# elun15/Graph-Convolutional-Network-for-Multi-Camera-Vehicle-Tracking

Measured on AMD Instinct MI355X. Metric: MPN forward edges/sec (+ achieved roofline fraction of the dominant kernel), higher is better.
Workload: dtype f32; 1 GPU; s02: AIC19-S02 ground-truth topology, cams 124/90/99/137: N=450 E=150454, L=3, Cs=1, eval forward; N=450, E=150454, parallelism=1 GPU

## Files before the change

### graph-convolutional-network-for-multi-camera-vehicle-tracking_amd/_lib.py

```python
from __future__ import annotations

import ctypes as C
import os

MAX_ENC_LAYERS = 8
NODE_DIM, EDGE_DIM, MAX_CLASSES = 32, 4, 4
AGG = {"sum": 0, "mean": 1, "max": 2}

(PH_BEGIN, PH_EDGE_ENC, PH_NODE_ENC, PH_NODE_H0, PH_ROUND_PROJ, PH_ROUND_A, PH_ROUND_B, PH_ROUND_STAT,
 PH_ROUND_C, PH_END, PH_NODE_COMBINE) = range(11)

E_ARG, E_WORKSPACE, E_HIP, E_ROWS = -1, -2, -3, -4

_f32p = C.c_void_p


class Layer(C.Structure):
    _fields_ = [("weight", _f32p), ("bias", _f32p), ("gamma", _f32p), ("beta", _f32p),
                ("in_dim", C.c_int32), ("out_dim", C.c_int32)]


class Model(C.Structure):
    _fields_ = [("struct_bytes", C.c_uint32), ("n_enc_layers", C.c_int32), ("enc_node", Layer * MAX_ENC_LAYERS), ("enc_edge", Layer * 2),
                ("upd_edge", Layer), ("upd_node", Layer), ("cls", Layer),
                ("agg", C.c_int32), ("num_enc_steps", C.c_int32), ("num_class_steps", C.c_int32),
                ("reattach_nodes", C.c_int32), ("reattach_edges", C.c_int32),
                ("dropout_enc", C.c_float), ("dropout_upd_edge", C.c_float), ("dropout_upd_node", C.c_float)]

    def __init__(self, *args, **kw):
        super().__init__(*args, **kw)
        self.struct_bytes = C.sizeof(type(self))


class Call(C.Structure):
    _fields_ = [("struct_bytes", C.c_uint32), ("x", C.c_void_p), ("x_row_stride", C.c_int64), ("row", C.c_void_p), ("col", C.c_void_p),
                ("idx_stride", C.c_int64), ("edge_attr", C.c_void_p), ("n_nodes", C.c_int64), ("n_edges", C.c_int64),
                ("n_edges_total", C.c_int64), ("node_lo", C.c_int64), ("node_hi", C.c_int64),
                ("logits", C.c_void_p), ("h_out", C.c_void_p), ("workspace", C.c_void_p),
                ("workspace_bytes", C.c_size_t), ("training", C.c_int32), ("flags", C.c_int32),
                ("seed", C.c_uint64), ("stream", C.c_void_p), ("row_lo", C.c_int64), ("row_hi", C.c_int64),
                ("weight_cache", C.c_void_p), ("weight_cache_bytes", C.c_size_t)]

    def __init__(self, *args, **kw):
        super().__init__(*args, **kw)
        self.struct_bytes = C.sizeof(type(self))


class WsLayout(C.Structure):
    _fields_ = [("total_bytes", C.c_size_t), ("zero_bytes", C.c_size_t), ("flags_off", C.c_size_t),
                ("stat_attr_off", C.c_size_t), ("stat_enc2_off", C.c_size_t), ("stat_enc_layer_off", C.c_size_t * MAX_ENC_LAYERS),
                ("stat_round_off", C.c_size_t), ("deg_off", C.c_size_t), ("seg_off", C.c_size_t),
                ("h0_off", C.c_size_t), ("h_acc_off", C.c_size_t * 2), ("deg_global_off", C.c_size_t),
                ("P_off", C.c_size_t)]


class Plan(C.Structure):
    _fields_ = [("enc_kernel", C.c_int32 * MAX_ENC_LAYERS), ("enc_split_k", C.c_int32 * MAX_ENC_LAYERS),
                ("edges_per_thread", C.c_int32), ("lazy_edges", C.c_int32), ("pass_c", C.c_int32),
                ("avg_degree", C.c_double), ("pass_a_col_blocks", C.c_int32), ("layer0_panels", C.c_int32),
                ("enc2_passenger", C.c_int32), ("node_stat_folded", C.c_int32)]


(GEMM_GENERIC, GEMM_INLOOP_64, GEMM_INLOOP_128, GEMM_PRESPLIT_256, GEMM_STAGED_128, GEMM_ROWS_16, GEMM_FEW_L0,
 GEMM_FEW_WAVE) = range(8)
PASS_C_WALK, PASS_C_MFMA_SORTED, PASS_C_MFMA_ANY = range(3)

STAT_REPLICAS, ATTR_STRIDE, ENC2_STRIDE, Z1_STRIDE, M_STRIDE, Z2_STRIDE = 16, 16, 16, 16, 16, 64
ROUND_BLOCK = STAT_REPLICAS * (Z1_STRIDE + M_STRIDE + Z2_STRIDE)
F_DETERMINISTIC, F_GLOBAL_DEG, F_FORK, F_SEED_ON_DEVICE = 1, 4, 2, 16
EDGE_W_ONE, EDGE_W_GIVEN, EDGE_W_BALANCED = range(3)
EDGE_LOSS_RECORD = 4
CLUSTER_SCORES, CLUSTER_COUNTS, EDGE_PRF = 9, 7, 5
CLUSTER_SCORES_MAX_N = 1048576
POOL_INFO = 4

LIB_PATH = os.environ.get("MTMC_MPN_LIB") or os.path.join(os.path.dirname(os.path.abspath(__file__)), "csrc", "libmtmc_mpn.so")
EXPORTS = ["mtmc_mpn_abi_version", "mtmc_mpn_last_error", "mtmc_mpn_workspace_bytes", "mtmc_mpn_workspace_layout",
           "mtmc_mpn_forward", "mtmc_mpn_run_phase", "mtmc_mpn_run_phases", "mtmc_mpn_plan_call", "mtmc_scatter_add", "mtmc_scatter_add_i64", "mtmc_scatter_mean", "mtmc_scatter_max",
           "mtmc_mlp_layer_forward", "mtmc_mpn_train_workspace_bytes", "mtmc_mpn_backward", "mtmc_graph_workspace_bytes",
           "mtmc_build_graph", "mtmc_postprocess_workspace_bytes", "mtmc_postprocess",
           "mtmc_cross_entropy_forward", "mtmc_cross_entropy_backward",
           "mtmc_cross_entropy_steps_forward", "mtmc_cross_entropy_steps_backward", "mtmc_mpn_backward_steps", "mtmc_mpn_backward_flat", "mtmc_mpn_grad_layout", "mtmc_linear_raw", "mtmc_edge_confusion",
           "mtmc_linear_presplit_raw", "mtmc_linear_staged_raw", "mtmc_linear_few_raw", "mtmc_mpn_weight_cache_bytes",
           "mtmc_graph_backward_workspace_bytes", "mtmc_build_graph_backward",
           "mtmc_edge_loss_scratch_bytes", "mtmc_edge_loss_forward", "mtmc_edge_loss_backward",
           "mtmc_cluster_scores_workspace_bytes", "mtmc_cluster_scores", "mtmc_edge_prf",
           "mtmc_pool_chunk_rows", "mtmc_pool_tracklets_workspace_bytes", "mtmc_pool_tracklets", "mtmc_pool_tracklets_backward"]

_lib = None


def load() -> C.CDLL:
    global _lib
    if _lib is not None:
        return _lib
    if not os.path.exists(LIB_PATH):
        raise RuntimeError(f"mtmc_mpn: HIP extension not built ({LIB_PATH} missing); run `python -m mtmc_mpn.build` "
                           "-- there is no fallback implementation")
    import torch
    lib = C.CDLL(LIB_PATH, mode=C.RTLD_GLOBAL)
    lib.mtmc_mpn_abi_version.restype = C.c_int32
    lib.mtmc_mpn_last_error.restype = C.c_char_p
    lib.mtmc_mpn_workspace_bytes.restype = C.c_size_t
    lib.mtmc_mpn_workspace_bytes.argtypes = [C.POINTER(Model), C.c_int64, C.c_int64]
    lib.mtmc_mpn_weight_cache_bytes.restype = C.c_size_t
    lib.mtmc_mpn_weight_cache_bytes.argtypes = [C.POINTER(Model)]
    lib.mtmc_linear_few_raw.restype = C.c_int32
    lib.mtmc_linear_few_raw.argtypes = [C.c_void_p, C.c_int64, C.c_void_p, C.c_void_p, C.c_void_p, C.c_double, C.c_void_p,
                                        C.c_void_p, C.c_void_p, C.c_int64, C.c_int32, C.c_int32, C.c_void_p, C.c_uint64,
                                        C.c_void_p, C.c_void_p]
    lib.mtmc_mpn_workspace_layout.restype = C.c_int32
    lib.mtmc_mpn_workspace_layout.argtypes = [C.POINTER(Model), C.c_int64, C.c_int64, C.POINTER(WsLayout)]
    lib.mtmc_mpn_forward.restype = C.c_int32
    lib.mtmc_mpn_forward.argtypes = [C.POINTER(Model), C.POINTER(Call)]
    lib.mtmc_mpn_train_workspace_bytes.restype = C.c_size_t
    lib.mtmc_mpn_train_workspace_bytes.argtypes = [C.POINTER(Model), C.c_int64, C.c_int64]
    lib.mtmc_mpn_backward.restype = C.c_int32
    lib.mtmc_mpn_backward.argtypes = [C.POINTER(Model), C.POINTER(Call), C.c_void_p, C.c_void_p, C.POINTER(Model),
                                      C.c_void_p, C.c_void_p]
    lib.mtmc_graph_workspace_bytes.restype = C.c_size_t
    lib.mtmc_graph_workspace_bytes.argtypes = [C.c_int64, C.c_int32]
    lib.mtmc_build_graph.restype = C.c_int32
    lib.mtmc_build_graph.argtypes = [C.c_void_p, C.c_int64, C.c_int64, C.c_int32, C.c_int32] + [C.c_void_p] * 5 + \
        [C.c_int32, C.c_int64] + [C.c_void_p] * 6 + [C.c_size_t, C.c_void_p]
    lib.mtmc_graph_backward_workspace_bytes.restype = C.c_size_t
    lib.mtmc_graph_backward_workspace_bytes.argtypes = [C.c_int64, C.c_int32]
    lib.mtmc_build_graph_backward.restype = C.c_int32
    lib.mtmc_build_graph_backward.argtypes = [C.c_void_p, C.c_int64, C.c_int64, C.c_int32, C.c_int32] + [C.c_void_p] * 5 + \
        [C.c_int32, C.c_int64] + [C.c_void_p] * 6 + [C.c_size_t, C.c_void_p]
    lib.mtmc_mpn_backward_steps.restype = C.c_int32
    lib.mtmc_mpn_backward_steps.argtypes = [C.POINTER(Model), C.POINTER(Call), C.POINTER(C.c_void_p), C.c_void_p,
                                            C.POINTER(Model), C.c_void_p, C.c_size_t, C.c_void_p, C.c_void_p]
    lib.mtmc_mpn_backward_flat.restype = C.c_int32
    lib.mtmc_mpn_backward_flat.argtypes = [C.POINTER(Model), C.POINTER(Call), C.POINTER(C.c_void_p), C.c_void_p, C.c_void_p,
                                           C.c_int64, C.c_void_p, C.c_void_p]
    lib.mtmc_mpn_grad_layout.restype = C.c_int64
    lib.mtmc_mpn_grad_layout.argtypes = [C.POINTER(Model), C.POINTER(C.c_int64), C.c_int32]
    lib.mtmc_edge_confusion.restype = C.c_int32
    lib.mtmc_edge_confusion.argtypes = [C.c_void_p, C.c_void_p, C.c_int64, C.c_int32, C.c_void_p, C.c_void_p]
    lib.mtmc_linear_presplit_raw.restype = C.c_int32
    lib.mtmc_linear_presplit_raw.argtypes = [C.c_void_p, C.c_int64, C.c_void_p, C.c_void_p, C.c_void_p, C.c_int64, C.c_int32,
                                             C.c_int32, C.c_void_p, C.c_uint64, C.c_void_p, C.c_void_p, C.c_int32, C.c_void_p]
    lib.mtmc_linear_staged_raw.restype = C.c_int32
    lib.mtmc_linear_staged_raw.argtypes = [C.c_void_p, C.c_int64, C.c_void_p, C.c_void_p, C.c_void_p, C.c_double, C.c_void_p,
                                           C.c_void_p, C.c_void_p, C.c_int64, C.c_int32, C.c_int32, C.c_void_p, C.c_uint64,
                                           C.c_void_p, C.c_void_p, C.c_void_p]
    lib.mtmc_linear_raw.restype = C.c_int32
    lib.mtmc_linear_raw.argtypes = [C.c_void_p, C.c_int64, C.c_void_p, C.c_void_p, C.c_void_p, C.c_int64, C.c_int32,
                                    C.c_int32, C.c_void_p, C.c_void_p, C.c_void_p]
    lib.mtmc_cross_entropy_forward.restype = C.c_int32
    lib.mtmc_cross_entropy_forward.argtypes = [C.c_void_p, C.c_void_p, C.c_void_p, C.c_int64, C.c_int32, C.c_int64,
                                               C.c_int32, C.c_void_p, C.c_void_p, C.c_void_p, C.c_void_p]
    lib.mtmc_cross_entropy_backward.restype = C.c_int32
    lib.mtmc_cross_entropy_backward.argtypes = [C.c_void_p, C.c_void_p, C.c_void_p, C.c_int64, C.c_int32, C.c_int64,
                                                C.c_int32, C.c_void_p, C.c_void_p, C.c_void_p, C.c_void_p]
    lib.mtmc_cross_entropy_steps_forward.restype = C.c_int32
    lib.mtmc_cross_entropy_steps_forward.argtypes = [C.c_void_p, C.c_void_p, C.c_void_p, C.c_int64, C.c_int32, C.c_int32,
                                                     C.c_int64, C.c_int32, C.c_void_p, C.c_void_p, C.c_void_p]
    lib.mtmc_cross_entropy_steps_backward.restype = C.c_int32
    lib.mtmc_cross_entropy_steps_backward.argtypes = [C.c_void_p, C.c_void_p, C.c_void_p, C.c_int64, C.c_int32, C.c_int32,
                                                      C.c_int64, C.c_int32, C.c_void_p, C.c_void_p, C.c_void_p, C.c_void_p]
    lib.mtmc_edge_loss_scratch_bytes.restype = C.c_size_t
    lib.mtmc_edge_loss_scratch_bytes.argtypes = [C.c_int32]
    lib.mtmc_edge_loss_forward.restype = C.c_int32
    lib.mtmc_edge_loss_forward.argtypes = [C.c_void_p, C.c_void_p, C.c_int64, C.c_int32, C.c_int32, C.c_int32, C.c_void_p,
                                           C.c_float, C.c_void_p, C.c_size_t, C.c_void_p, C.c_void_p, C.c_void_p, C.c_void_p]
    lib.mtmc_edge_loss_backward.restype = C.c_int32
    lib.mtmc_edge_loss_backward.argtypes = [C.c_void_p, C.c_void_p, C.c_int64, C.c_int32, C.c_int32, C.c_void_p, C.c_void_p,
                                            C.c_void_p, C.c_void_p]
    lib.mtmc_cluster_scores_workspace_bytes.restype = C.c_size_t
    lib.mtmc_cluster_scores_workspace_bytes.argtypes = [C.c_int64]
    lib.mtmc_cluster_scores.restype = C.c_int32
    lib.mtmc_cluster_scores.argtypes = [C.c_void_p, C.c_int64, C.c_void_p, C.c_int64, C.c_int64, C.c_void_p, C.c_void_p,
                                        C.c_void_p, C.c_size_t, C.c_void_p]
    lib.mtmc_edge_prf.restype = C.c_int32
    lib.mtmc_edge_prf.argtypes = [C.c_void_p, C.c_int64, C.c_void_p, C.c_int64, C.c_int64, C.c_void_p, C.c_void_p, C.c_void_p]
    lib.mtmc_pool_chunk_rows.restype = C.c_int32
    lib.mtmc_pool_chunk_rows.argtypes = []
    lib.mtmc_pool_tracklets_workspace_bytes.restype = C.c_size_t
    lib.mtmc_pool_tracklets_workspace_bytes.argtypes = [C.c_int64, C.c_int32]
    lib.mtmc_pool_tracklets.restype = C.c_int32
    lib.mtmc_pool_tracklets.argtypes = [C.c_void_p, C.c_int64, C.c_int64, C.c_int32, C.c_void_p, C.c_int64, C.c_void_p,
                                        C.c_void_p, C.c_void_p, C.c_size_t, C.c_void_p]
    lib.mtmc_pool_tracklets_backward.restype = C.c_int32
    lib.mtmc_pool_tracklets_backward.argtypes = [C.c_void_p, C.c_int64, C.c_int32, C.c_void_p, C.c_int64, C.c_void_p,
                                                 C.c_int64, C.c_void_p]
    lib.mtmc_postprocess_workspace_bytes.restype = C.c_size_t
    lib.mtmc_postprocess_workspace_bytes.argtypes = [C.c_int64, C.c_int64, C.c_int64]
    lib.mtmc_postprocess.restype = C.c_int32
    lib.mtmc_postprocess.argtypes = [C.c_void_p, C.c_void_p, C.c_void_p, C.c_int64, C.c_int64, C.c_int64, C.c_int32,
                                     C.c_int32, C.c_int64, C.c_void_p, C.c_void_p, C.c_void_p, C.c_void_p, C.c_void_p,
                                     C.c_size_t, C.c_void_p]
    lib.mtmc_mpn_plan_call.restype = C.c_int32
    lib.mtmc_mpn_plan_call.argtypes = [C.POINTER(Model), C.POINTER(Call), C.POINTER(Plan)]
    lib.mtmc_mpn_run_phase.restype = C.c_int32
    lib.mtmc_mpn_run_phase.argtypes = [C.POINTER(Model), C.POINTER(Call), C.c_int32, C.c_int32]
    lib.mtmc_mpn_run_phases.restype = C.c_int32
    lib.mtmc_mpn_run_phases.argtypes = [C.POINTER(Model), C.POINTER(Call), C.POINTER(C.c_int32), C.c_int32]
    for name in ("mtmc_scatter_add", "mtmc_scatter_add_i64"):
        getattr(lib, name).restype = C.c_int32
        getattr(lib, name).argtypes = [C.c_void_p, C.c_void_p, C.c_int64, C.c_int64, C.c_int64, C.c_void_p, C.c_void_p]
    lib.mtmc_scatter_mean.restype = C.c_int32
    lib.mtmc_scatter_mean.argtypes = [C.c_void_p, C.c_void_p, C.c_int64, C.c_int64, C.c_int64, C.c_void_p, C.c_void_p,
                                      C.c_void_p]
    lib.mtmc_scatter_max.restype = C.c_int32
    lib.mtmc_scatter_max.argtypes = [C.c_void_p, C.c_void_p, C.c_int64, C.c_int64, C.c_int64, C.c_void_p, C.c_void_p,
                                     C.c_void_p]
    lib.mtmc_mlp_layer_forward.restype = C.c_int32
    lib.mtmc_mlp_layer_forward.argtypes = [C.POINTER(Layer), C.c_void_p, C.c_int64, C.c_int64, C.c_void_p, C.c_void_p,
                                           C.c_void_p]
    if lib.mtmc_mpn_abi_version() != 6:
        raise RuntimeError("mtmc_mpn: ABI version mismatch between _lib.py and libmtmc_mpn.so")
    _lib = lib
    return lib


def check(rc: int):
    if rc == 0:
        return
    msg = load().mtmc_mpn_last_error().decode()
    if rc == E_ROWS:
        raise ValueError(msg)
    raise RuntimeError(f"mtmc_mpn: {msg} (code {rc})")
```

### graph-convolutional-network-for-multi-camera-vehicle-tracking_amd/csrc/api.hip

```cpp
#include "api_internal.h"

using namespace mtmc_api;

namespace {

struct Side { hipStream_t stream = nullptr; hipEvent_t fork = nullptr, join = nullptr; bool ok = false; };
Side* side_for_current_device() {
  static Side sides[64];
  static std::mutex mu;
  int dev = 0;
  if (hipGetDevice(&dev) != hipSuccess || dev < 0 || dev >= 64) return nullptr;
  std::lock_guard<std::mutex> lock(mu);
  Side& sd = sides[dev];
  if (!sd.ok) {
    if (hipStreamCreateWithFlags(&sd.stream, hipStreamNonBlocking) != hipSuccess) return nullptr;
    if (hipEventCreateWithFlags(&sd.fork, hipEventDisableTiming) != hipSuccess) return nullptr;
    if (hipEventCreateWithFlags(&sd.join, hipEventDisableTiming) != hipSuccess) return nullptr;
    sd.ok = true;
  }
  return &sd;
}

constexpr int kMaxPipes = 64;
struct PipeSlot { int dev; hipStream_t caller; SidePipe pipe; };
// ... 41 lines not shown
  Layout lo;
  make_layout(model, n_nodes, n_edges, &lo);
  return lo.pub.total_bytes;
}

size_t mtmc_mpn_weight_cache_bytes(const mtmc_mpn_model* model) {
  if (check_model(model) != MTMC_OK) return 0;
  CacheLayout cl;
  make_cache_layout(model, &cl);
  return cl.total > 0 ? cl.total : 256;
}

int32_t mtmc_mpn_workspace_layout(const mtmc_mpn_model* model, int64_t n_nodes, int64_t n_edges, mtmc_ws_layout* out) {
  if (int rc = check_model(model)) return rc;
  if (!out || n_nodes < 0 || n_edges < 0) return fail(MTMC_E_ARG, "bad layout arguments");
  Layout lo;
  make_layout(model, n_nodes, n_edges, &lo);
  *out = lo.pub;
  return MTMC_OK;
}

int32_t mtmc_dbg_panel_timing(int32_t enable) {
  PanelTiming& pt = panel_timing();
  if (enable && !pt.created) {
    for (int i = 0; i < 2 * kMaxPanels; ++i)
      if (hipEventCreate(&pt.ev[i]) != hipSuccess) return fail(MTMC_E_HIP, "hipEventCreate failed");
    pt.created = true;
  }
  pt.on = enable != 0;
  pt.n = 0;
  return MTMC_OK;
}
int32_t mtmc_dbg_panel_times(float* ms, int32_t max) {
  PanelTiming& pt = panel_timing();
  if (!ms || !pt.created) return 0;
  int n = 0;
  for (; n < pt.n && n < max; ++n) {
    if (hipEventSynchronize(pt.ev[2 * n + 1]) != hipSuccess) break;
    if (hipEventElapsedTime(&ms[n], pt.ev[2 * n], pt.ev[2 * n + 1]) != hipSuccess) break;
  }
  return n;
}

int32_t mtmc_mpn_run_phase(const mtmc_mpn_model* model, const mtmc_mpn_call* call, int32_t phase, int32_t arg) {
  Ctx x;
  if (int rc = make_ctx(model, call, &x)) return rc;
  return run_phase(x, phase, arg);
}

int32_t mtmc_mpn_run_phases(const mtmc_mpn_model* model, const mtmc_mpn_call* call, const int32_t* phase_args, int32_t n) {
  Ctx x;
  if (int rc = make_ctx(model, call, &x)) return rc;
  if (n < 0 || (n > 0 && !phase_args)) return fail(MTMC_E_ARG, "mtmc_mpn_run_phases: bad phase list");
  for (int i = 0; i < n; ++i)
    if (int rc = run_phase(x, phase_args[2 * i], phase_args[2 * i + 1])) return rc;
  return MTMC_OK;
}

int32_t mtmc_mpn_plan_call(const mtmc_mpn_model* model, const mtmc_mpn_call* call, mtmc_mpn_plan* out) {
  if (int rc = check_model(model)) return rc;
  if (!out) return fail(MTMC_E_ARG, "mtmc_mpn_plan_call: NULL result");
  if (int rc = check_call_size(call)) return rc;
  const mtmc_mpn_call* c = call;
  if (c->n_nodes < 0 || c->n_edges < 0 || c->n_edges > c->n_edges_total || c->node_lo < 0 || c->node_hi < c->node_lo ||
      c->node_hi > c->n_nodes || c->row_lo < 0 || c->row_hi < c->row_lo || c->row_hi > c->n_nodes)
    return fail(MTMC_E_ARG, "mtmc_mpn_plan_call: sizes / ranges out of order");
  Layout lo;
  CacheLayout cl;
  CallPlan p;
  make_layout(model, c->n_nodes, c->n_edges, &lo, c->training != 0);
  make_cache_layout(model, &cl);
  make_plan(model, c, lo, cl, &p);
  *out = mtmc_mpn_plan();
  for (int l = 0; l < model->n_enc_layers; ++l) { out->enc_kernel[l] = p.enc_kernel[l]; out->enc_split_k[l] = p.enc_split_k[l]; }
  out->edges_per_thread = p.edges_per_thread;
  out->lazy_edges = p.lazy_edges ? 1 : 0;
  out->avg_degree = p.avg_degree;
  out->pass_a_col_blocks = p.col_blocks;
  out->pass_c = p.pass_c_pub();
  out->node_stat_folded = p.fold_node_stat ? 1 : 0;
  out->layer0_panels = p.l0_panels;
  out->enc2_passenger = (p.enc2_may_ride && !(c->flags & MTMC_F_FORK)) ? 1 : 0;
  return MTMC_OK;
}

int32_t mtmc_mpn_forward(const mtmc_mpn_model* model, const mtmc_mpn_call* call) {
  Ctx x;
  if (int rc = make_ctx(model, call, &x)) return rc;
  int rc;
  if (x.plan.l0_panels >= 2) x.pipe = pipe_for(x.stream);
  Side* sd = (call->flags & MTMC_F_FORK) ? side_for_current_device() : nullptr;
  if (sd) {
    if ((rc = run_phase(x, MTMC_PH_BEGIN, 0))) return rc;
    if (hipEventRecord(sd->fork, x.stream) != hipSuccess || hipStreamWaitEvent(sd->stream, sd->fork, 0) != hipSuccess)
      return fail(MTMC_E_HIP, "fork onto the side stream failed");
    Ctx xs = x;
    xs.stream = sd->stream;
    if ((rc = run_phase(xs, MTMC_PH_EDGE_ENC, 0))) return rc;
    if (hipEventRecord(sd->join, sd->stream) != hipSuccess) return fail(MTMC_E_HIP, "hipEventRecord failed");
  } else {
    if ((rc = run_phase(x, MTMC_PH_BEGIN, 0))) return rc;
    x.enc2_rides = x.plan.enc2_may_ride;
    if (!x.enc2_rides && (rc = run_phase(x, MTMC_PH_EDGE_ENC, 0))) return rc;
  }
  for (int l = 0; l < model->n_enc_layers; ++l) {
    if ((rc = run_phase(x, MTMC_PH_NODE_ENC, l))) return rc;
    if ((rc = run_phase(x, MTMC_PH_NODE_COMBINE, l))) return rc;
  }
  if (sd && hipStreamWaitEvent(x.stream, sd->join, 0) != hipSuccess) return fail(MTMC_E_HIP, "join failed");
  const bool fused_h0 = model->num_enc_steps > 0 && call->node_lo == 0 && call->node_hi == call->n_nodes;
  if (!fused_h0 && (rc = run_phase(x, MTMC_PH_NODE_H0, 0))) return rc;
  for (int r = 0; r < model->num_enc_steps; ++r) {
    if ((rc = run_phase(x, MTMC_PH_ROUND_PROJ, r, fused_h0))) return rc;
    if ((rc = run_phase(x, MTMC_PH_ROUND_A, r))) return rc;
    if ((rc = run_phase(x, MTMC_PH_ROUND_B, r))) return rc;
    if ((rc = run_phase(x, MTMC_PH_ROUND_STAT, r))) return rc;
    if ((rc = run_phase(x, MTMC_PH_ROUND_C, r))) return rc;
  }
  return run_phase(x, MTMC_PH_END, 0);
}

static int scatter_common(const float* src, const int64_t* index, int64_t n_src, int64_t n_cols, int64_t dim_size,
                          float* out, float* count, int64_t* arg_out, int mode, void* stream) {
  if (n_src < 0 || n_cols < 1 || dim_size < 0 || !out || (n_src > 0 && (!src || !index)))
    return fail(MTMC_E_ARG, "bad scatter arguments");
  if (mode == 1 && !count) return fail(MTMC_E_ARG, "scatter_mean needs count_scratch[dim_size]");
  if (dim_size == 0) return MTMC_OK;
  mtmc::launch_scatter(src, index, n_src, n_cols, dim_size, out, count, arg_out, mode, static_cast<hipStream_t>(stream));
  const hipError_t e = hipGetLastError();
  return e == hipSuccess ? MTMC_OK : fail(MTMC_E_HIP, "scatter launch failed: %s", hipGetErrorString(e));
}
int32_t mtmc_scatter_add(const float* src, const int64_t* index, int64_t n_src, int64_t n_cols, int64_t dim_size,
                         float* out, void* stream) {
  return scatter_common(src, index, n_src, n_cols, dim_size, out, nullptr, nullptr, 0, stream);
}
int32_t mtmc_scatter_add_i64(const int64_t* src, const int64_t* index, int64_t n_src, int64_t n_cols, int64_t dim_size,
                             int64_t* out, void* stream) {
  if (n_src < 0 || n_cols < 1 || dim_size < 0 || !out || (n_src > 0 && (!src || !index)))
    return fail(MTMC_E_ARG, "bad scatter arguments");
  if (dim_size == 0) return MTMC_OK;
  mtmc::launch_scatter_add_i64(src, index, n_src, n_cols, dim_size, out, static_cast<hipStream_t>(stream));
  const hipError_t e = hipGetLastError();
  return e == hipSuccess ? MTMC_OK : fail(MTMC_E_HIP, "scatter launch failed: %s", hipGetErrorString(e));
}
int32_t mtmc_scatter_mean(const float* src, const int64_t* index, int64_t n_src, int64_t n_cols, int64_t dim_size,
                          float* out, float* count_scratch, void* stream) {
  return scatter_common(src, index, n_src, n_cols, dim_size, out, count_scratch, nullptr, 1, stream);
}
int32_t mtmc_scatter_max(const float* src, const int64_t* index, int64_t n_src, int64_t n_cols, int64_t dim_size,
                         float* out, int64_t* arg_out, void* stream) {
  return scatter_common(src, index, n_src, n_cols, dim_size, out, nullptr, arg_out, 2, stream);
}

int32_t mtmc_mlp_layer_forward(const mtmc_layer* layer, const float* x, int64_t x_row_stride, int64_t rows, float* y,
                               double* stats_scratch, void* stream) {
  if (!layer || !layer->weight || !layer->bias || !x || !y || rows < 1) return fail(MTMC_E_ARG, "bad mlp layer arguments");
  const bool bn = layer->gamma != nullptr;
  if (bn && (!layer->beta || !stats_scratch)) return fail(MTMC_E_ARG, "BatchNorm layer needs beta and stats_scratch[2*out]");
  if (bn && rows < 2) return fail(MTMC_E_ROWS, "Expected more than 1 value per channel when training");
  hipStream_t s = static_cast<hipStream_t>(stream);
  if (bn && hipMemsetAsync(stats_scratch, 0, 2 * (size_t)layer->out_dim * sizeof(double), s) != hipSuccess)
    return fail(MTMC_E_HIP, "hipMemsetAsync failed");
  mtmc::GemmParams g =
      mtmc::plain_gemm(x, x_row_stride, layer->weight, layer->bias, y, layer->out_dim, rows, layer->in_dim, layer->out_dim);
  if (bn) g.stats_out = stats_scratch;
  if (mtmc::launch_gemm_bn(g, s) != MTMC_OK) return fail(MTMC_E_ARG, "unsupported layer shape");
  if (bn)
    mtmc::launch_bn_relu_rows({y, layer->out_dim, rows, layer->out_dim, stats_scratch, layer->gamma, layer->beta, (double)rows, y,
                               mtmc::kNoDrop, 0}, s);
  const hipError_t e = hipGetLastError();
  return e == hipSuccess ? MTMC_OK : fail(MTMC_E_HIP, "mlp layer launch failed: %s", hipGetErrorString(e));
}

static int raw_begin(uint32_t* scratch, double* stats, int N, hipStream_t s) {
  return mtmc::clear_raw(scratch, stats, N, s) ? MTMC_OK : fail(MTMC_E_HIP, "hipMemsetAsync failed");
}
static int raw_end(int rc) {
  if (rc != 0) return fail(rc == MTMC_E_HIP ? MTMC_E_HIP : MTMC_E_ARG, "unsupported shape or launch refused");
  const hipError_t e = hipGetLastError();
  return e == hipSuccess ? MTMC_OK : fail(MTMC_E_HIP, "launch failed: %s", hipGetErrorString(e));
}
static void raw_amax(const float* A, int64_t lda, int64_t M, const float* W, int K, int N, uint32_t* scratch, hipStream_t s) {
  mtmc::PrepParams p = {};
  p.jobs[p.n_jobs++] = {A, M, K, lda, scratch, 0, 0};
  if (W) p.jobs[p.n_jobs++] = {W, N, K, K, scratch + mtmc::kAmaxRep, 0, 0};
  mtmc::launch_prep(p, s);
}

int32_t mtmc_linear_raw(const float* A, int64_t lda, const float* W, const float* bias, float* Y, int64_t M, int32_t K,
                        int32_t N, uint32_t* scratch, double* stats, void* stream) {
  if (!A || !W || !bias || !Y || !scratch || M < 1 || K < 32 || K % 32 || N < 1) return fail(MTMC_E_ARG, "bad arguments");
  hipStream_t s = static_cast<hipStream_t>(stream);
  if (int rc = raw_begin(scratch, stats, N, s)) return rc;
  raw_amax(A, lda, M, W, K, N, scratch, s);
  mtmc::GemmParams g = mtmc::plain_gemm(A, lda, W, bias, Y, N, M, K, N, scratch, scratch + mtmc::kAmaxRep, scratch + 2 * mtmc::kAmaxRep);
  g.stats_out = stats;
// ... 77 lines not shown
```

### graph-convolutional-network-for-multi-camera-vehicle-tracking_amd/csrc/api_internal.h

```cpp
#pragma once
#include "kernels.h"
#include "train_kernels.h"

#include <mutex>
#include <stdarg.h>
#include <stdio.h>
#include <stdlib.h>
#include <string.h>
#include <algorithm>
#include <vector>

namespace mtmc_api {


inline thread_local char g_err[512] = "";

inline int fail(int code, const char* fmt, ...) __attribute__((format(printf, 2, 3)));
inline int fail(int code, const char* fmt, ...) {
  va_list ap;
  va_start(ap, fmt);
  vsnprintf(g_err, sizeof(g_err), fmt, ap);
  va_end(ap);
  return code;
}

inline size_t align_up(size_t v, size_t a = 256) { return (v + a - 1) / a * a; }

struct Layout {
  mtmc_ws_layout pub;
  size_t row32, col32, e_buf[2], P, Q, slab, enc_aff, row_start, carry;
  size_t col_sub; int col_blocks;
  size_t amax;
  size_t amax_w;
  size_t Y[MTMC_MAX_ENC_LAYERS];
  size_t stat_enc_layer[MTMC_MAX_ENC_LAYERS];
  bool training;
  std::vector<size_t> z_tr, e_tr, h_tr;
  std::vector<size_t> P_tr, Q_tr;
  size_t xh, inv_a;
  bool few;
  size_t wh[MTMC_MAX_ENC_LAYERS], inv_w[MTMC_MAX_ENC_LAYERS]; bool w_ws[MTMC_MAX_ENC_LAYERS];
  size_t g_e[2], g_e0, g_h[2], g_h0, g_P, g_Q, g_de2, g_arg;
  size_t bst;
  size_t bwd_zero, bwd_zero_end;
  size_t gacc;
  size_t amax_bwd;
  size_t seed_word = 0;
  size_t gA, gB, tA, tB, tW, tX, zeros, bst_n;
};

struct CacheLayout { size_t planes[MTMC_MAX_ENC_LAYERS], inv[MTMC_MAX_ENC_LAYERS], fp[MTMC_MAX_ENC_LAYERS]; bool has[MTMC_MAX_ENC_LAYERS]; size_t total; };
inline void make_cache_layout(const mtmc_mpn_model* m, CacheLayout* cl) {
  size_t off = 0;
  auto take = [&](size_t bytes) { size_t o = off; off = align_up(off + bytes); return o; };
  for (int l = 0; l < MTMC_MAX_ENC_LAYERS; ++l) {
    cl->has[l] = l < m->n_enc_layers && m->enc_node[l].in_dim % 8 == 0 && m->enc_node[l].in_dim <= 2048;
    cl->planes[l] = cl->inv[l] = cl->fp[l] = 0;
    if (!cl->has[l]) continue;
    const size_t K = m->enc_node[l].in_dim, O = m->enc_node[l].out_dim;
    cl->planes[l] = take(4 * O * K);
    cl->inv[l] = take(4 * O);
    cl->fp[l] = take(8 * ((O + 7) / 8));
  }
  cl->total = off;
}
inline bool few_shape(const mtmc_mpn_model* m, int64_t rows) {
  int in_dim[MTMC_MAX_ENC_LAYERS], out_dim[MTMC_MAX_ENC_LAYERS];
  for (int l = 0; l < m->n_enc_layers; ++l) { in_dim[l] = m->enc_node[l].in_dim; out_dim[l] = m->enc_node[l].out_dim; }
  return mtmc::few_rows_path(rows, m->n_enc_layers, in_dim, out_dim);
}

inline int node_in_width(const mtmc_mpn_model* m) { return (m->reattach_nodes ? 2 : 1) * MTMC_NODE_DIM; }
inline int first_cls_step(const mtmc_mpn_model* m) { return std::max(1, m->num_enc_steps - m->num_class_steps + 1); }

inline int check_model(const mtmc_mpn_model* m) {
  if (!m) return fail(MTMC_E_ARG, "model is NULL");
  if (m->struct_bytes != sizeof(mtmc_mpn_model))
    return fail(MTMC_E_ARG, "mtmc_mpn_model.struct_bytes is %u, this library's struct has %zu bytes (ABI v%d): rebuild the caller against include/mtmc_mpn.h",
                m->struct_bytes, sizeof(mtmc_mpn_model), MTMC_MPN_ABI_VERSION);
  if (m->n_enc_layers < 1 || m->n_enc_layers > MTMC_MAX_ENC_LAYERS) return fail(MTMC_E_ARG, "n_enc_layers out of range");
  for (int l = 0; l < m->n_enc_layers; ++l) {
    const mtmc_layer& L = m->enc_node[l];
    if (!L.weight || !L.bias || !L.gamma || !L.beta) return fail(MTMC_E_ARG, "node encoder layer %d: NULL parameter", l);
    if (L.in_dim % 32 || L.in_dim < 32 || L.out_dim < 1) return fail(MTMC_E_ARG, "node encoder layer %d: in_dim must be a positive multiple of 32", l);
    if (l && L.in_dim != m->enc_node[l - 1].out_dim) return fail(MTMC_E_ARG, "node encoder layer %d: in_dim != previous out_dim", l);
  }
  if (m->enc_node[m->n_enc_layers - 1].out_dim != MTMC_NODE_DIM) return fail(MTMC_E_ARG, "node encoder must end at width %d", MTMC_NODE_DIM);
  if ((m->enc_edge[0].in_dim != 1 && m->enc_edge[0].in_dim != 2) || m->enc_edge[0].out_dim != 4 ||
      m->enc_edge[1].in_dim != 4 || m->enc_edge[1].out_dim != 4)
    return fail(MTMC_E_ARG, "edge encoder must be in(1|2)->4->4");
  const int hn = node_in_width(m), he = (m->reattach_edges ? 2 : 1) * MTMC_EDGE_DIM;
  if (m->upd_edge.in_dim != 2 * hn + he || m->upd_edge.out_dim != 4) return fail(MTMC_E_ARG, "edge update layer must be [4, %d]", 2 * hn + he);
  if (m->upd_node.in_dim != hn + 4 || m->upd_node.out_dim != MTMC_NODE_DIM) return fail(MTMC_E_ARG, "node update layer must be [32, %d]", hn + 4);
  if (m->cls.in_dim != 4 || m->cls.out_dim < 1 || m->cls.out_dim > MTMC_MAX_CLASSES) return fail(MTMC_E_ARG, "classifier must be [C<=4, 4]");
  const mtmc_layer* small[] = {&m->enc_edge[0], &m->enc_edge[1], &m->upd_edge, &m->upd_node};
  for (const mtmc_layer* L : small)
    if (!L->weight || !L->bias || !L->gamma || !L->beta) return fail(MTMC_E_ARG, "NULL parameter in an edge/update layer");
  if (!m->cls.weight || !m->cls.bias) return fail(MTMC_E_ARG, "NULL classifier parameter");
  if (m->agg < 0 || m->agg > 2) return fail(MTMC_E_ARG, "agg must be MTMC_AGG_SUM/MEAN/MAX");
  if (m->num_enc_steps < 0 || m->num_class_steps < 0) return fail(MTMC_E_ARG, "negative step count");
  return MTMC_OK;
}

inline void make_layout(const mtmc_mpn_model* m, int64_t N, int64_t E, Layout* lo, bool training = false) {
  *lo = Layout();
  lo->training = training;
  size_t off = 0;
  auto take = [&](size_t bytes) { size_t o = off; off = align_up(off + bytes); return o; };
  const int L = m->num_enc_steps;
  lo->pub.flags_off = take(8 * sizeof(int32_t));
  lo->pub.stat_attr_off = take((size_t)mtmc::kStatRep * mtmc::kAttrStride * sizeof(double));
  lo->stat_enc_layer[0] = take(2 * (size_t)m->enc_node[0].out_dim * sizeof(double));
  lo->pub.stat_enc2_off = take((size_t)mtmc::kStatRep * mtmc::kEnc2Stride * sizeof(double));
  for (int l = 1; l < m->n_enc_layers; ++l) lo->stat_enc_layer[l] = take(2 * (size_t)m->enc_node[l].out_dim * sizeof(double));
  for (int l = 0; l < m->n_enc_layers; ++l) lo->pub.stat_enc_layer_off[l] = lo->stat_enc_layer[l];
  lo->pub.stat_round_off = take((size_t)(L > 0 ? L : 1) * mtmc::kRoundBlock * sizeof(double));
  lo->pub.deg_off = take((size_t)N * sizeof(int32_t));
  lo->pub.seg_off = take(mtmc::fold_node_stat(E) ? 0 : (size_t)N * 4 * sizeof(double));
  lo->amax = take((size_t)(1 + 2 * MTMC_MAX_ENC_LAYERS) * mtmc::kAmaxRep * sizeof(uint32_t));
  lo->amax_w = take((size_t)MTMC_MAX_ENC_LAYERS * mtmc::kAmaxRep * sizeof(uint32_t));
  lo->pub.zero_bytes = off;
  lo->pub.deg_global_off = take((size_t)N * sizeof(int32_t));
  lo->pub.h0_off = take((size_t)N * 32 * sizeof(float));
  lo->pub.h_acc_off[0] = take((size_t)N * 32 * sizeof(float));
  lo->pub.h_acc_off[1] = take((size_t)N * 32 * sizeof(float));
  lo->enc_aff = take(16 * sizeof(float));
  lo->seed_word = take(sizeof(unsigned long long));
  lo->row_start = take((size_t)N * sizeof(int32_t));
  lo->carry = take((size_t)((E + 31) / 32) * 2 * 32 * sizeof(float));
  lo->col_blocks = mtmc::plan_col_blocks(N, E, 1e30, training);
  lo->col_sub = take(lo->col_blocks > 0 ? (size_t)N * (lo->col_blocks + 1) * sizeof(int32_t) : 0);
  lo->P = take((size_t)N * 8 * sizeof(float));
  lo->pub.P_off = lo->P;
  lo->Q = take((size_t)N * 32 * sizeof(float));
  lo->row32 = take((size_t)E * sizeof(int32_t));
  lo->col32 = take((size_t)E * sizeof(int32_t));
  lo->e_buf[0] = take((size_t)E * 4 * sizeof(float));
  lo->e_buf[1] = take((size_t)E * 4 * sizeof(float));
  for (int l = 0; l < m->n_enc_layers; ++l) lo->Y[l] = take((size_t)N * m->enc_node[l].out_dim * sizeof(float));
  size_t slab = 0;
  for (int l = 0; l < m->n_enc_layers; ++l) {
    int sk;
    mtmc::gemm_plan(N, m->enc_node[l].in_dim, m->enc_node[l].out_dim, &sk);
    const size_t need = sk > 1 ? (size_t)sk * N * m->enc_node[l].out_dim * sizeof(float) : 0;
    if (need > slab) slab = need;
  }
  lo->slab = take(slab);
  lo->few = few_shape(m, N);
  for (int l = 0; l < m->n_enc_layers; ++l) {
    const int K = m->enc_node[l].in_dim, O = m->enc_node[l].out_dim;
    lo->w_ws[l] = !training && (l == 0 ? mtmc::presplit_layer0(N, K, O) : mtmc::staged_layer(N, K, O));
  }
  if (lo->w_ws[0] || lo->few) {
    lo->xh = take((size_t)2 * N * m->enc_node[0].in_dim * sizeof(uint16_t));
    lo->inv_a = take((size_t)N * sizeof(float));
  }
  for (int l = 0; l < m->n_enc_layers; ++l)
    if (lo->w_ws[l]) {
      lo->wh[l] = take((size_t)2 * m->enc_node[l].out_dim * m->enc_node[l].in_dim * sizeof(uint16_t));
      lo->inv_w[l] = take((size_t)m->enc_node[l].out_dim * sizeof(float));
    }
  if (training) {
    for (int r = 0; r < L; ++r) {
      lo->z_tr.push_back(take((size_t)E * 4 * sizeof(float)));
      lo->e_tr.push_back(take((size_t)E * 4 * sizeof(float)));
      lo->h_tr.push_back(take((size_t)N * 32 * sizeof(float)));
      lo->P_tr.push_back(r == 0 ? lo->P : take((size_t)N * 8 * sizeof(float)));
      lo->Q_tr.push_back(r == 0 ? lo->Q : take((size_t)N * 32 * sizeof(float)));
    }
    size_t maxd = 0, bn_stats = 0;
    for (int l = 0; l < m->n_enc_layers; ++l) {
      maxd = std::max(maxd, (size_t)m->enc_node[l].in_dim);
      maxd = std::max(maxd, (size_t)m->enc_node[l].out_dim);
      bn_stats += 2 * (size_t)m->enc_node[l].out_dim;
    }
    lo->bwd_zero = off;
    lo->bst = take((size_t)(2 * L + 1) * mtmc::kStatRep * mtmc::kBwdStride * sizeof(double));
    lo->bst_n = take(bn_stats * sizeof(double));
    lo->gacc = take((size_t)mtmc::kGradRep * mtmc::kGaccN * sizeof(float));
    lo->amax_bwd = take((size_t)2 * MTMC_MAX_ENC_LAYERS * mtmc::kAmaxRep * sizeof(uint32_t));
    lo->g_P = take((size_t)(L > 0 ? L : 1) * mtmc::kGradRep * N * 8 * sizeof(float));
    lo->g_Q = take((size_t)(L > 0 ? L : 1) * N * 32 * sizeof(float));
    lo->zeros = take(maxd * sizeof(float));
    lo->g_h0 = take((size_t)N * 32 * sizeof(float));
    lo->g_e0 = take((size_t)E * 4 * sizeof(float));
    lo->g_e[0] = take((size_t)E * 4 * sizeof(float));
    lo->g_h[0] = take((size_t)N * 32 * sizeof(float));
    lo->bwd_zero_end = off;
    lo->g_e[1] = take((size_t)E * 4 * sizeof(float));
    lo->g_h[1] = take((size_t)N * 32 * sizeof(float));
    lo->g_de2 = take((size_t)E * 4 * sizeof(float));
    lo->g_arg = take((size_t)N * 32 * sizeof(int32_t));
    const size_t npad = (size_t)((N + 31) / 32 * 32);
    lo->gA = take((size_t)N * maxd * sizeof(float));
    lo->gB = take((size_t)N * maxd * sizeof(float));
    lo->tA = take(npad * maxd * sizeof(float));
    lo->tB = take(npad * maxd * sizeof(float));
    size_t wsum = 0;
    for (int l = 0; l < m->n_enc_layers; ++l) wsum += (size_t)m->enc_node[l].in_dim * m->enc_node[l].out_dim;
    lo->tW = take(wsum * sizeof(float));
    lo->tX = take(npad * (size_t)m->enc_node[0].in_dim * sizeof(float));
  }
  lo->pub.total_bytes = off;
}

constexpr int kMaxPanels = 16;
struct SidePipe { hipStream_t stream = nullptr; hipEvent_t fork = nullptr; hipEvent_t ready[kMaxPanels] = {}; };

struct PanelTiming { bool on = false, created = false; hipEvent_t ev[2 * kMaxPanels]; int n = 0; };
inline PanelTiming& panel_timing() { static PanelTiming t; return t; }

inline int l0_panels(int64_t rows, int Nout, int64_t* cuts, int* bm) {
  const int tiles_n = (Nout + 255) / 256;
  *bm = mtmc::presplit_tile_rows(rows, tiles_n);
  const int64_t per_round = (int64_t)(256 / tiles_n > 0 ? 256 / tiles_n : 1) * *bm;
  const int mode = mtmc::knobs().l0_pipeline;
  int np = 0;
  int64_t at = 0, k = 1;
  cuts[0] = 0;
  while (at < rows) {
    int64_t take = per_round * (mode == 3 ? 2 : mode == 2 ? 1 : k);
    if (np == kMaxPanels - 1 || at + take > rows) take = rows - at;
    at += take;
    cuts[++np] = at;
    if (k < 8) k *= 2;
  }
  return np;
}

struct CallPlan {
  int64_t rows;
  int enc_kernel[MTMC_MAX_ENC_LAYERS];
  int enc_split_k[MTMC_MAX_ENC_LAYERS];
  bool w_cached[MTMC_MAX_ENC_LAYERS];
  int l0_panels, l0_bm;
  int64_t l0_cuts[kMaxPanels + 1];
  bool enc2_may_ride;
  int edges_per_thread;
  bool lazy_edges;
  bool fold_node_stat;
  double avg_degree;
  int col_blocks;
  mtmc::PassC pass_c;
  int pass_c_pub() const {
    switch (pass_c) {
      case mtmc::kPassCSortedWalk: case mtmc::kPassCSortedDet: return MTMC_PASS_C_MFMA_SORTED;
      case mtmc::kPassCAnyWalk: case mtmc::kPassCAny: return MTMC_PASS_C_MFMA_ANY;
      default: return MTMC_PASS_C_WALK;
    }
  }
};

inline bool in_loop_kernel(int k) { return k == MTMC_GEMM_GENERIC || k == MTMC_GEMM_INLOOP_64 || k == MTMC_GEMM_INLOOP_128; }

inline void make_plan(const mtmc_mpn_model* m, const mtmc_mpn_call* c, const Layout& lo, const CacheLayout& cl, CallPlan* p) {
  *p = CallPlan();
  const int64_t N = c->n_nodes, E = c->n_edges, rows = c->node_hi - c->node_lo;
  const mtmc_layer& L0 = m->enc_node[0];
  p->rows = rows;
  const bool pre0 = lo.w_ws[0] && mtmc::presplit_layer0(rows, L0.in_dim, L0.out_dim);
  bool few = lo.few && c->weight_cache != nullptr && few_shape(m, rows);
  for (int l = 0; l < m->n_enc_layers; ++l) few = few && cl.has[l];
  for (int l = 0; l < m->n_enc_layers; ++l) {
    const mtmc_layer& Ll = m->enc_node[l];
    int k, sk = 1;
    if (few) k = l == 0 ? MTMC_GEMM_FEW_L0 : MTMC_GEMM_FEW_WAVE;
    else if (l == 0 && pre0) k = MTMC_GEMM_PRESPLIT_256;
    else if (l >= 1 && lo.w_ws[l] && mtmc::staged_layer(rows, Ll.in_dim, Ll.out_dim)) k = MTMC_GEMM_STAGED_128;
    else if (l >= 1 && !lo.training && mtmc::rows_layer(N, Ll.in_dim, Ll.out_dim) && mtmc::rows_layer(rows, Ll.in_dim, Ll.out_dim))
      k = MTMC_GEMM_ROWS_16;
    else {
      int sk_full = 1, sk_here = 1;
      mtmc::gemm_plan(N, Ll.in_dim, Ll.out_dim, &sk_full);
      const int cfg = rows > 0 ? mtmc::gemm_plan(rows, Ll.in_dim, Ll.out_dim, &sk_here) : 0;
      k = cfg == 2 ? MTMC_GEMM_INLOOP_128 : cfg == 1 ? MTMC_GEMM_INLOOP_64 : MTMC_GEMM_GENERIC;
      if (sk_here > 1 && (size_t)sk_here * rows <= (size_t)(sk_full > 1 ? sk_full : 0) * N) sk = sk_here;
    }
    p->enc_kernel[l] = k;
    p->enc_split_k[l] = sk;
    p->w_cached[l] = c->weight_cache != nullptr && cl.has[l] && !in_loop_kernel(k) && k != MTMC_GEMM_ROWS_16;
  }
  p->l0_panels = 1;
  if (p->enc_kernel[0] == MTMC_GEMM_PRESPLIT_256 && mtmc::knobs().l0_pipeline > 0)
    p->l0_panels = l0_panels(rows, L0.out_dim, p->l0_cuts, &p->l0_bm);
  const int last = m->n_enc_layers - 1, kl = p->enc_kernel[last];
  p->enc2_may_ride = E > 0 && E <= mtmc::kSmallEdges &&
                     (kl == MTMC_GEMM_INLOOP_64 || (kl == MTMC_GEMM_FEW_WAVE && mtmc::few_wave_threads(m->enc_node[last].in_dim) == 256));
  p->edges_per_thread = mtmc::plan_edges_per_thread(E);
  p->lazy_edges = !lo.training && E > mtmc::kSmallEdges;
  p->fold_node_stat = mtmc::fold_node_stat(E);
  if (c->row_hi > 0) p->avg_degree = c->row_hi > c->row_lo ? (double)E / (double)(c->row_hi - c->row_lo) : 0.0;
  else p->avg_degree = N > 0 ? (double)c->n_edges_total / (double)N : 0.0;
  p->col_blocks = (m->num_enc_steps > 0 && lo.col_blocks > 0 &&
                   mtmc::plan_col_blocks(N, E, p->avg_degree, lo.training) == lo.col_blocks) ? lo.col_blocks : 0;
  const bool drop_n = lo.training && m->dropout_upd_node > 0.f;
  p->pass_c = mtmc::plan_pass_c(m->agg, (c->flags & MTMC_F_DETERMINISTIC) != 0, drop_n, E, N, p->avg_degree);
}

struct Ctx {
  const mtmc_mpn_model* m;
  const mtmc_mpn_call* c;
  Layout lo;
  char* ws;
  hipStream_t stream;
  char* wc = nullptr;
  CacheLayout cl;
  CallPlan plan;
  template <typename T> T* wc_at(size_t off) const { return reinterpret_cast<T*>(wc + off); }
  const SidePipe* pipe = nullptr;
  bool enc2_rides = false;
  template <typename T> T* at(size_t off) const { return reinterpret_cast<T*>(ws + off); }
};

inline int check_call_size(const mtmc_mpn_call* c) {
  if (!c) return fail(MTMC_E_ARG, "call is NULL");
  if (c->struct_bytes != sizeof(mtmc_mpn_call))
    return fail(MTMC_E_ARG, "mtmc_mpn_call.struct_bytes is %u, this library's struct has %zu bytes (ABI v%d): rebuild the caller against include/mtmc_mpn.h",
                c->struct_bytes, sizeof(mtmc_mpn_call), MTMC_MPN_ABI_VERSION);
  return MTMC_OK;
}

inline int make_ctx(const mtmc_mpn_model* m, const mtmc_mpn_call* c, Ctx* ctx) {
  if (int rc = check_model(m)) return rc;
  if (int rc = check_call_size(c)) return rc;
  if (c->training && (c->node_lo != 0 || c->node_hi != c->n_nodes || c->n_edges_total != c->n_edges))
    return fail(MTMC_E_ARG, "training mode is single-shard only");
  if (c->training && (c->flags & MTMC_F_SEED_ON_DEVICE) && (c->seed == 0 || (c->seed & 7)))
    return fail(MTMC_E_ARG, "MTMC_F_SEED_ON_DEVICE: seed must hold the 8-byte aligned device address of a uint64 counter");
  if (c->n_nodes < 2) return fail(MTMC_E_ROWS, "BatchNorm over %lld node rows: Expected more than 1 value per channel", (long long)c->n_nodes);
  if (c->n_edges_total < 2) return fail(MTMC_E_ROWS, "BatchNorm over %lld edge rows: Expected more than 1 value per channel", (long long)c->n_edges_total);
  if (c->n_edges < 0 || c->n_edges > c->n_edges_total || c->n_edges >= (1ll << 31) || c->n_nodes >= (1ll << 31))
    return fail(MTMC_E_ARG, "edge/node counts out of range");
  if (c->node_lo < 0 || c->node_hi < c->node_lo || c->node_hi > c->n_nodes) return fail(MTMC_E_ARG, "bad node range");
  if (c->row_lo < 0 || c->row_hi < c->row_lo || c->row_hi > c->n_nodes) return fail(MTMC_E_ARG, "bad row range");
  if (c->training && (c->row_lo != 0 || (c->row_hi != 0 && c->row_hi != c->n_nodes)))
    return fail(MTMC_E_ARG, "training calls project every node row (row_lo = row_hi = 0)");
  if (!c->x || !c->edge_attr || !c->logits || !c->h_out || !c->workspace) return fail(MTMC_E_ARG, "NULL tensor pointer");
  if (c->n_edges > 0 && (!c->row || !c->col)) return fail(MTMC_E_ARG, "NULL edge_index pointer");
  if (c->idx_stride < 1) return fail(MTMC_E_ARG, "idx_stride must be >= 1");
  if (((uintptr_t)c->x & 15) || (c->x_row_stride & 3) || c->x_row_stride < m->enc_node[0].in_dim)
    return fail(MTMC_E_ARG, "x must be 16-byte aligned with a row stride that is a multiple of 4 and >= in_dim");
  if (((uintptr_t)c->edge_attr & 7) || ((uintptr_t)c->logits & 7) || ((uintptr_t)c->h_out & 15))
    return fail(MTMC_E_ARG, "edge_attr/logits must be 8-byte and h_out 16-byte aligned");
  if ((uintptr_t)c->workspace & 255) return fail(MTMC_E_WORKSPACE, "workspace must be 256-byte aligned");
  ctx->m = m; ctx->c = c;
  make_layout(m, c->n_nodes, c->n_edges, &ctx->lo, c->training != 0);
  if (c->workspace_bytes < ctx->lo.pub.total_bytes)
    return fail(MTMC_E_WORKSPACE, "workspace has %zu bytes, %zu needed", c->workspace_bytes, ctx->lo.pub.total_bytes);
  ctx->ws = static_cast<char*>(c->workspace);
  ctx->stream = static_cast<hipStream_t>(c->stream);
  make_cache_layout(m, &ctx->cl);
  if (c->weight_cache) {
    if ((uintptr_t)c->weight_cache & 255) return fail(MTMC_E_WORKSPACE, "weight_cache must be 256-byte aligned");
    if (c->weight_cache_bytes < ctx->cl.total)
      return fail(MTMC_E_WORKSPACE, "weight_cache has %zu bytes, %zu needed (mtmc_mpn_weight_cache_bytes)", c->weight_cache_bytes, ctx->cl.total);
    ctx->wc = static_cast<char*>(c->weight_cache);
  }
  make_plan(m, c, ctx->lo, ctx->cl, &ctx->plan);
  return MTMC_OK;
}

inline mtmc::Drop make_drop(const Ctx& x, float p) {
  mtmc::Drop d;
  d.on = (x.c->training && p > 0.f) ? 1 : 0;
  d.seed = x.c->seed;
  if (d.on && (x.c->flags & MTMC_F_SEED_ON_DEVICE)) {
    d.on = 2;
    d.seed = (unsigned long long)(uintptr_t)(x.ws + x.lo.seed_word);
  }
  const double t = (double)p * 65536.0;
  d.thresh = t >= 65535.0 ? 65535u : (unsigned)t;
  d.inv_keep = p < 1.f ? 1.f / (1.f - p) : 0.f;
  return d;
}

inline mtmc::EdgeEncParams enc_params(const Ctx& x) {
  mtmc::EdgeEncParams e;
  const mtmc_layer& a = x.m->enc_edge[0];
  const mtmc_layer& b = x.m->enc_edge[1];
  e.w1 = a.weight; e.b1 = a.bias; e.g1 = a.gamma; e.bt1 = a.beta;
  e.w2 = b.weight; e.b2 = b.bias; e.g2 = b.gamma; e.bt2 = b.beta;
  e.stat_attr = x.at<double>(x.lo.pub.stat_attr_off);
  e.stat_enc2 = x.at<double>(x.lo.pub.stat_enc2_off);
  e.aff = x.at<float>(x.lo.enc_aff);
  e.fe = a.in_dim;
  e.drop = make_drop(x, x.m->dropout_enc);
  return e;
}

inline float* agg_target(const Ctx& x, int r) {
  if (x.lo.training) return x.at<float>(x.lo.h_tr[r]);
  if (r == x.m->num_enc_steps - 1 && x.m->agg != MTMC_AGG_MEAN) return x.c->h_out;
  return x.at<float>(x.lo.pub.h_acc_off[r & 1]);
}
inline int64_t proj_lo(const mtmc_mpn_call* c) { return c->row_hi > 0 ? c->row_lo : 0; }
inline int64_t proj_hi(const mtmc_mpn_call* c) { return c->row_hi > 0 ? c->row_hi : c->n_nodes; }
inline float* round_h_src(const Ctx& x, int r) {
  if (r == 0) return x.at<float>(x.lo.pub.h0_off);
  return x.lo.training ? x.at<float>(x.lo.h_tr[r - 1]) : x.at<float>(x.lo.pub.h_acc_off[(r - 1) & 1]);
}
inline float* round_P(const Ctx& x, int r) { return x.at<float>(x.lo.training ? x.lo.P_tr[r] : x.lo.P); }
inline float* round_Q(const Ctx& x, int r) { return x.at<float>(x.lo.training ? x.lo.Q_tr[r] : x.lo.Q); }
inline float* round_z(const Ctx& x, int r) { return x.at<float>(x.lo.training ? x.lo.z_tr[r] : x.lo.e_buf[r & 1]); }
inline float* round_e(const Ctx& x, int r) { return x.at<float>(x.lo.training ? x.lo.e_tr[r] : x.lo.e_buf[r & 1]); }

inline mtmc::RoundParams round_params(const Ctx& x, int r) {
  const mtmc_mpn_model* m = x.m;
  const int hn = node_in_width(m);
  mtmc::RoundParams p;
  p.row32 = x.at<int>(x.lo.row32); p.col32 = x.at<int>(x.lo.col32);
  p.attr = x.c->edge_attr;
  p.e_buf = round_z(x, r); p.e_out = round_e(x, r); p.e_prev = r > 0 ? round_e(x, r - 1) : nullptr;
  p.drop_e = make_drop(x, m->dropout_upd_edge); p.drop_n = make_drop(x, m->dropout_upd_node);
  p.drop_stream = mtmc::kDropRound + 2 * r;
  p.P = round_P(x, r); p.Q = round_Q(x, r);
  p.seg = x.at<double>(x.lo.pub.seg_off); p.fold_z2 = x.plan.fold_node_stat ? 1 : 0;
  p.ue_w = m->upd_edge.weight; p.ue_b = m->upd_edge.bias; p.ue_g = m->upd_edge.gamma; p.ue_bt = m->upd_edge.beta;
  p.ue_ld = m->upd_edge.in_dim; p.ue_eoff = 2 * hn;
  p.un_w = m->upd_node.weight; p.un_b = m->upd_node.bias; p.un_g = m->upd_node.gamma; p.un_bt = m->upd_node.beta;
  p.un_ld = m->upd_node.in_dim; p.un_eoff = hn;
  p.cls_w = m->cls.weight; p.cls_b = m->cls.bias; p.n_classes = m->cls.out_dim;
  p.stats = x.at<double>(x.lo.pub.stat_round_off) + (size_t)r * mtmc::kRoundBlock;
  p.lazy_e = x.plan.lazy_edges ? 1 : 0;
  p.prev_stats = r > 0 ? p.stats - mtmc::kRoundBlock : nullptr;
  p.h_acc = agg_target(x, r);
  const int step = r + 1, first_cls = first_cls_step(m);
  p.logits = step >= first_cls ? x.c->logits + (size_t)(step - first_cls) * x.c->n_edges * m->cls.out_dim : nullptr;
  p.n_edges = x.c->n_edges; p.e_total = (double)x.c->n_edges_total;
  p.first_round = r == 0; p.reattach_edges = m->reattach_edges; p.agg = m->agg;
  p.det = (x.c->flags & MTMC_F_DETERMINISTIC) ? 1 : 0; p.flags = x.at<int>(x.lo.pub.flags_off);
  p.deg = x.at<int>(x.lo.pub.deg_off); p.row_start = x.at<int>(x.lo.row_start); p.carry = x.at<float>(x.lo.carry);
  p.n_nodes = x.c->n_nodes;
  p.avg_degree = x.plan.avg_degree;
  p.pass_c = x.plan.pass_c;
  p.col_blocks = x.plan.col_blocks;
  p.col_sub = x.at<int>(x.lo.col_sub); p.cb_row_lo = proj_lo(x.c); p.cb_row_hi = proj_hi(x.c);
  p.enc = enc_params(x);
  return p;
}

inline _Float16* w_planes(const Ctx& x, int l) {
  if (x.plan.w_cached[l]) return x.wc_at<_Float16>(x.cl.planes[l]);
  return x.at<_Float16>(x.lo.wh[l]);
}
inline float* w_inv(const Ctx& x, int l) {
  if (x.plan.w_cached[l]) return x.wc_at<float>(x.cl.inv[l]);
  return x.at<float>(x.lo.inv_w[l]);
}

enum { kPhMemset = -1, kPhPrep = -2 };

inline void fill_prep_edge(const Ctx& x, mtmc::PrepEdge* p) {
  const mtmc_mpn_call* c = x.c;
  p->row = c->row; p->col = c->col; p->idx_stride = c->idx_stride; p->attr = c->edge_attr; p->fe = x.m->enc_edge[0].in_dim;
  p->n_edges = c->n_edges; p->n_nodes = c->n_nodes;
  p->row32 = x.at<int>(x.lo.row32); p->col32 = x.at<int>(x.lo.col32); p->deg = x.at<int>(x.lo.pub.deg_off);
  p->flags = x.at<int>(x.lo.pub.flags_off); p->stat_attr = x.at<double>(x.lo.pub.stat_attr_off);
  p->row_start = x.at<int>(x.lo.row_start);
}

inline const int* scale_deg(const Ctx& x) {
  return x.at<int>((x.c->flags & MTMC_F_GLOBAL_DEG) ? x.lo.pub.deg_global_off : x.lo.pub.deg_off);
}

inline unsigned* amax_x(const Ctx& x) { return x.at<unsigned>(x.lo.amax); }
inline unsigned* amax_y(const Ctx& x, int l) { return amax_x(x) + (1 + MTMC_MAX_ENC_LAYERS + l) * mtmc::kAmaxRep; }
inline unsigned* amax_w(const Ctx& x, int l) { return x.at<unsigned>(x.lo.amax_w) + l * mtmc::kAmaxRep; }
inline unsigned* amax_in(const Ctx& x, int l) { return l == 0 ? amax_x(x) : amax_y(x, l - 1); }

inline void fill_in(const Ctx& x, int l, mtmc::ActIn* q) {
  if (l == 0) {
    q->A = x.c->x; q->lda = x.c->x_row_stride;
  } else {
    const mtmc_layer& Pv = x.m->enc_node[l - 1];
    q->A = x.at<float>(x.lo.Y[l - 1]); q->lda = Pv.out_dim;
    q->stats_in = x.at<double>(x.lo.stat_enc_layer[l - 1]); q->gamma_in = Pv.gamma; q->beta_in = Pv.beta;
  }
  q->count = (double)x.c->n_nodes;
  q->drop_in = make_drop(x, x.m->dropout_enc); q->drop_stream = mtmc::kDropEncNode + l - 1;
}
inline void fill_out(const Ctx& x, int l, mtmc::LayerOut* q) {
  const mtmc_layer& Lr = x.m->enc_node[l];
  q->bias = Lr.bias; q->Y = x.at<float>(x.lo.Y[l]); q->ldy = Lr.out_dim;
  q->stats_out = x.at<double>(x.lo.stat_enc_layer[l]); q->amax_y = amax_y(x, l);
  q->M = x.plan.rows; q->K = Lr.in_dim; q->Nout = Lr.out_dim;
}
inline void fill_w(const Ctx& x, int l, mtmc::PlanesW* q) { q->Wh = w_planes(x, l); q->inv_w = w_inv(x, l); }
inline void fill_x(const Ctx& x, mtmc::PlanesA* q) { q->Ah = x.at<_Float16>(x.lo.xh); q->inv_a = x.at<float>(x.lo.inv_a); }
inline void ride_enc2(const Ctx& x, mtmc::Enc2Ride* q) {
  const int64_t blocks = (x.c->n_edges + 255) / 256;
  q->pass_blocks = (int)(blocks > 2048 ? 2048 : blocks);
  q->pass_enc = enc_params(x); q->pass_attr = x.c->edge_attr; q->pass_edges = x.c->n_edges;
  q->pass_e_total = (double)x.c->n_edges_total; q->pass_stat = x.at<double>(x.lo.pub.stat_enc2_off);
}

inline int launch_enc_few(const Ctx& x, int l) {
  int rc;
  if (l == 0) {
    mtmc::FewL0Params q;
    fill_x(x, &q); fill_w(x, 0, &q); fill_out(x, 0, &q);
    rc = mtmc::launch_few_l0(q, x.stream);
  } else {
    mtmc::FewWaveParams q;
    fill_in(x, l, &q); fill_w(x, l, &q); fill_out(x, l, &q);
    if (x.enc2_rides && l == x.m->n_enc_layers - 1) ride_enc2(x, &q);
    rc = mtmc::launch_few_wave(q, x.stream);
  }
  if (rc != 0) return fail(rc == MTMC_E_HIP ? MTMC_E_HIP : MTMC_E_ARG, "encoder layer %d: few-row kernel refused the shape or the launch", l);
  return MTMC_OK;
}

inline int launch_enc_presplit0(const Ctx& x) {
  const mtmc_mpn_call* c = x.c;
  const mtmc_layer& Lr = x.m->enc_node[0];
  const int64_t rows = x.plan.rows;
  hipStream_t s = x.stream;
  mtmc::SplitGemmParams q;
  fill_x(x, &q); fill_w(x, 0, &q); fill_out(x, 0, &q);
  PanelTiming& pt = panel_timing();
  if (x.pipe) {
// ... 71 lines not shown
        const CallPlan& pl = x.plan;
        const int64_t rows = pl.rows;
        mtmc::PrepParams p;
        fill_prep_edge(x, &p);
        p.n_jobs = 0;
        if (rows > 0) {
          if (pl.enc_kernel[0] == MTMC_GEMM_FEW_L0)
            p.jobs[p.n_jobs++] = {c->x, rows, m->enc_node[0].in_dim, c->x_row_stride, c->training ? amax_x(x) : nullptr, 0, 0, mtmc::kJobSplit,
                                  x.at<_Float16>(x.lo.xh), x.at<float>(x.lo.inv_a), nullptr};
          else if (pl.enc_kernel[0] != MTMC_GEMM_PRESPLIT_256)
            p.jobs[p.n_jobs++] = {c->x, rows, m->enc_node[0].in_dim, c->x_row_stride, amax_x(x), 0, 0, mtmc::kJobAmax, nullptr, nullptr, nullptr};
          for (int l = 0; l < m->n_enc_layers; ++l) {
            const mtmc_layer& Ll = m->enc_node[l];
            if (pl.w_cached[l])
              p.jobs[p.n_jobs++] = {Ll.weight, Ll.out_dim, Ll.in_dim, Ll.in_dim, c->training ? amax_w(x, l) : nullptr, 0, 0,
                                    mtmc::kJobSplit, x.wc_at<_Float16>(x.cl.planes[l]), x.wc_at<float>(x.cl.inv[l]),
                                    x.wc_at<unsigned long long>(x.cl.fp[l])};
            else if (in_loop_kernel(pl.enc_kernel[l]))
              p.jobs[p.n_jobs++] = {Ll.weight, Ll.out_dim, Ll.in_dim, Ll.in_dim, amax_w(x, l), 0, 0, mtmc::kJobAmax,
                                    nullptr, nullptr, nullptr};
          }
        }
        mtmc::launch_prep(p, s);
        if (pl.col_blocks > 0) {
          const mtmc::RoundParams rp = round_params(x, 0);
          mtmc::launch_colblock_index(rp, x.at<int>(x.lo.col_sub), rp.col_blocks, rp.cb_row_lo, rp.cb_row_hi, s);
        }
        if (pl.enc_kernel[0] == MTMC_GEMM_PRESPLIT_256 && !x.pipe)
          mtmc::launch_split_rows(c->x, c->x_row_stride, rows, m->enc_node[0].in_dim, x.at<void>(x.lo.xh),
                                  x.at<float>(x.lo.inv_a), s);
        for (int l = 0; l < m->n_enc_layers; ++l) {
          const mtmc_layer& Ll = m->enc_node[l];
          if ((pl.enc_kernel[l] == MTMC_GEMM_PRESPLIT_256 || pl.enc_kernel[l] == MTMC_GEMM_STAGED_128) && !pl.w_cached[l])
            mtmc::launch_split_rows(Ll.weight, Ll.in_dim, Ll.out_dim, Ll.in_dim, w_planes(x, l), w_inv(x, l), s);
        }
      }
      break;
    }
    case MTMC_PH_EDGE_ENC:
      if (c->n_edges > 0)
        mtmc::launch_enc2(enc_params(x), c->edge_attr, c->n_edges, (double)c->n_edges_total, x.at<double>(x.lo.pub.stat_enc2_off), s);
      break;
    case MTMC_PH_NODE_ENC:
    case MTMC_PH_NODE_COMBINE: {
      if (arg < 0 || arg >= m->n_enc_layers) return fail(MTMC_E_ARG, "encoder layer %d out of range", arg);
      if (x.plan.rows == 0) break;
      const int k = x.plan.enc_kernel[arg];
      if (phase == MTMC_PH_NODE_COMBINE && !in_loop_kernel(k)) break;
      int rc;
      if (k == MTMC_GEMM_FEW_L0 || k == MTMC_GEMM_FEW_WAVE) rc = launch_enc_few(x, arg);
      else if (k == MTMC_GEMM_PRESPLIT_256) rc = launch_enc_presplit0(x);
      else if (k == MTMC_GEMM_STAGED_128) rc = launch_enc_staged(x, arg);
      else rc = launch_enc_gemm(x, arg, phase);
      if (rc) return rc;
      break;
    }
    case MTMC_PH_NODE_H0: {
      const int last = m->n_enc_layers - 1;
      const int64_t rows = c->node_hi - c->node_lo;
      if (rows > 0)
        mtmc::launch_bn_relu_rows({x.at<float>(x.lo.Y[last]), MTMC_NODE_DIM, rows, MTMC_NODE_DIM,
                                   x.at<double>(x.lo.stat_enc_layer[last]), m->enc_node[last].gamma, m->enc_node[last].beta,
                                   (double)c->n_nodes, x.at<float>(x.lo.pub.h0_off) + (size_t)c->node_lo * MTMC_NODE_DIM,
                                   make_drop(x, m->dropout_enc), mtmc::kDropEncNode + last, c->node_lo}, s);
      break;
    }
    case MTMC_PH_ROUND_PROJ: {
      if (arg < 0 || arg >= L) return fail(MTMC_E_ARG, "round %d out of range", arg);
      mtmc::NodeProjParams p;
      const int last = m->n_enc_layers - 1;
      p.y_last = (arg == 0 && fused_h0) ? x.at<float>(x.lo.Y[last]) : nullptr;
      p.y_stats = x.at<double>(x.lo.stat_enc_layer[last]); p.y_gamma = m->enc_node[last].gamma;
      p.y_beta = m->enc_node[last].beta; p.y_count = (double)c->n_nodes; p.h0_out = x.at<float>(x.lo.pub.h0_off);
      p.finalize_enc = arg == 0; p.enc = enc_params(x); p.e_total = (double)c->n_edges_total;
      p.h_src = round_h_src(x, arg);
      p.drop = make_drop(x, m->dropout_enc); p.drop_stream = mtmc::kDropEncNode + last;
      p.h0 = m->reattach_nodes ? x.at<float>(x.lo.pub.h0_off) : nullptr;
      p.deg = (m->agg == MTMC_AGG_MEAN && arg > 0) ? scale_deg(x) : nullptr;
      p.ue_w = m->upd_edge.weight; p.ue_ld = m->upd_edge.in_dim;
      p.un_w = m->upd_node.weight; p.un_ld = m->upd_node.in_dim;
      p.hn = node_in_width(m);
      p.P = round_P(x, arg); p.Q = round_Q(x, arg);
      p.zero_buf = agg_target(x, arg);
      p.n_nodes = c->n_nodes;
      p.node_begin = proj_lo(c); p.node_end = proj_hi(c);
      p.edge_deg = x.at<int>(x.lo.pub.deg_off); p.un_b = m->upd_node.bias;
      p.z2_stats = x.plan.fold_node_stat
                       ? x.at<double>(x.lo.pub.stat_round_off) + (size_t)arg * mtmc::kRoundBlock + mtmc::kRoundZ2Off : nullptr;
      mtmc::launch_node_proj(p, s);
      break;
    }
    case MTMC_PH_ROUND_A:
    case MTMC_PH_ROUND_B:
    case MTMC_PH_ROUND_C: {
      if (arg < 0 || arg >= L) return fail(MTMC_E_ARG, "round %d out of range", arg);
      if (c->n_edges == 0) break;
      const mtmc::RoundParams p = round_params(x, arg);
      if (phase == MTMC_PH_ROUND_A) mtmc::launch_pass_a(p, s);
      else if (phase == MTMC_PH_ROUND_B) mtmc::launch_pass_b(p, s);
      else mtmc::launch_pass_c(p, s);
      break;
    }
    case MTMC_PH_ROUND_STAT: {
      if (arg < 0 || arg >= L) return fail(MTMC_E_ARG, "round %d out of range", arg);
      if (x.plan.fold_node_stat) break;
      mtmc::NodeStatParams p;
      p.Q = round_Q(x, arg); p.deg = x.at<int>(x.lo.pub.deg_off); p.seg = x.at<double>(x.lo.pub.seg_off);
      p.un_w = m->upd_node.weight; p.un_b = m->upd_node.bias; p.un_ld = m->upd_node.in_dim;
      p.un_eoff = node_in_width(m);
      p.stats = x.at<double>(x.lo.pub.stat_round_off) + (size_t)arg * mtmc::kRoundBlock;
      p.n_nodes = c->n_nodes;
      p.node_begin = proj_lo(c); p.node_end = proj_hi(c);
      mtmc::launch_node_stat(p, s);
      break;
    }
    case MTMC_PH_END: {
      const float* src = round_h_src(x, L);
      if (L == 0 || m->agg == MTMC_AGG_MEAN || x.lo.training)
        mtmc::launch_h_final(src, scale_deg(x), (m->agg == MTMC_AGG_MEAN && L > 0) ? 1 : 0, c->n_nodes, c->h_out, s);
      if (L == 0 && c->n_edges > 0)
        mtmc::launch_classify_e0(enc_params(x), c->edge_attr, c->n_edges, (double)c->n_edges_total, m->cls.weight,
                                 m->cls.bias, m->cls.out_dim, c->logits, s);
      break;
    }
    default:
      return fail(MTMC_E_ARG, "unknown phase %d", phase);
  }
  const hipError_t e = hipGetLastError();
  if (e != hipSuccess) return fail(MTMC_E_HIP, "kernel launch failed in phase %d: %s", phase, hipGetErrorString(e));
  return MTMC_OK;
}

}
```

### graph-convolutional-network-for-multi-camera-vehicle-tracking_amd/csrc/edge_pass_b.hip

```cpp
#include "edge_common.h"

namespace mtmc {

template <int kEPT>
__global__ __launch_bounds__(256) void pass_b_kernel(RoundParams p) {
  drop_resolve(p.drop_e);
  __shared__ float s1[4], t1[4];
  __shared__ double red[14 * 4 + 4 * 128 + 4];
  const int lane = threadIdx.x & 63;
  constexpr bool kFold = kEPT == 1;
  const int k32 = lane & 31, hh = lane >> 5;
  const float ub = p.un_b[k32];
  double c0 = 0, c1 = 0;
  const int64_t stride = (int64_t)gridDim.x * blockDim.x * kEPT;
  const int64_t e_end = ((p.n_edges + 63) / 64) * 64;
  int64_t base = (int64_t)blockIdx.x * blockDim.x * kEPT + threadIdx.x;
  int rr[kEPT];
  float4 zz[kEPT];
  auto whole = [&](int64_t b) { return b - threadIdx.x + 256 * kEPT <= p.n_edges; };
  auto fetch = [&](int64_t b) {
    if (whole(b)) {
      const int64_t t0 = b - threadIdx.x;
#pragma unroll
      for (int i = 0; i < kEPT; ++i) {
#if PB_NT
        typedef float f4v __attribute__((ext_vector_type(4)));
        rr[i] = __builtin_nontemporal_load(p.row32 + t0 + i * 256 + threadIdx.x);
        const f4v v = __builtin_nontemporal_load(reinterpret_cast<const f4v*>(p.e_buf + (t0 + i * 256) * 4) + threadIdx.x);
        zz[i] = make_float4(v[0], v[1], v[2], v[3]);
#else
        rr[i] = (p.row32 + t0 + i * 256)[threadIdx.x];
        zz[i] = reinterpret_cast<const float4*>(p.e_buf + (t0 + i * 256) * 4)[threadIdx.x];
#endif
      }
      return;
    }
#pragma unroll
    for (int i = 0; i < kEPT; ++i) {
      const int64_t e = b + i * 256;
      rr[i] = -1;
      zz[i] = make_float4(0.f, 0.f, 0.f, 0.f);
      if (e < p.n_edges) {
        rr[i] = p.row32[e];
        zz[i] = reinterpret_cast<const float4*>(p.e_buf)[e];
      }
    }
  };
  float qf[kEPT], ql[kEPT];
  auto prefetch_q = [&]() {
#pragma unroll
    for (int i = 0; i < kEPT; ++i) {
      qf[i] = ql[i] = 0.f;
      if (kFold) {
        const int rf = __builtin_amdgcn_readfirstlane(rr[i]), rl = __builtin_amdgcn_readlane(rr[i], 63);
        qf[i] = p.Q[(int64_t)(rf < 0 ? 0 : rf) * kH + k32];
        ql[i] = p.Q[(int64_t)(rl < 0 ? 0 : rl) * kH + k32];
      }
    }
  };
  EK_T(3, 0);
  if (base < e_end) fetch(base);
  stat_gather(p.stats + kRoundZ1Off, 8, kZ1Stride, red);
  if (base < e_end) prefetch_q();
  __syncthreads();
  EK_T(3, 1);
  if (threadIdx.x < 4) {
    const int k = threadIdx.x;
    bn_affine(red[k], red[4 + k], p.e_total, p.ue_g[k], p.ue_bt[k], s1[k], t1[k]);
  }
  __syncthreads();
  EK_T(3, 2);
  double acc[14];
#pragma unroll
  for (int i = 0; i < 14; ++i) acc[i] = 0;
  bool first_trip = true;
  while (base < e_end) {
    const bool full = whole(base);
    float vv[kEPT][4];
#pragma unroll
    for (int i = 0; i < kEPT; ++i) {
      const int64_t e = base + i * 256;
#pragma unroll
      for (int k = 0; k < 4; ++k) vv[i][k] = 0.f;
      if (full || e < p.n_edges) {
        const float z4[4] = {zz[i].x, zz[i].y, zz[i].z, zz[i].w};
#pragma unroll
        for (int k = 0; k < 4; ++k) vv[i][k] = fmaxf(fmaf(z4[k], s1[k], t1[k]), 0.f);
        drop_apply4(p.drop_e, p.drop_stream, (unsigned long long)e * 4, vv[i]);
        if (!p.lazy_e) reinterpret_cast<float4*>(p.e_out)[e] = make_float4(vv[i][0], vv[i][1], vv[i][2], vv[i][3]);
      }
    }
    if (!first_trip) prefetch_q();
    first_trip = false;
    auto rl_f32 = [](float x, int l) { return __int_as_float(__builtin_amdgcn_readlane(__float_as_int(x), l)); };
    auto add_run = [&](float S0, float S1, float S2, float S3, float qrow) {
      const double qb = (double)(qrow + ub);
      c0 = fma((double)(hh ? S2 : S0), qb, c0);
      c1 = fma((double)(hh ? S3 : S1), qb, c1);
    };
#pragma unroll
    for (int i = 0; i < kEPT; ++i) {
      const int64_t e = base + i * 256;
      if (!full && e - lane >= p.n_edges) continue;
      const bool active = full || e < p.n_edges;
      float* v = vv[i];
      const int r = rr[i];
#pragma unroll
      for (int a = 0; a < 4; ++a) {
        acc[a] += v[a];
#pragma unroll
        for (int b = a; b < 4; ++b) acc[4 + tri(4, a, b)] += (double)v[a] * v[b];
      }
      const int r0 = __builtin_amdgcn_readfirstlane(r);
      const unsigned long long in_first = __ballot(r == r0);
      if (in_first == ~0ull && r0 >= 0) {
        const float t = wave_sum4_f32(v[0], v[1], v[2], v[3]);
        if (kFold) add_run(rl_f32(t, 15), rl_f32(t, 47), rl_f32(t, 31), rl_f32(t, 63), qf[i]);
        else if ((lane & 15) == 15) unsafeAtomicAdd(p.seg + (int64_t)r0 * 4 + wave_sum4_slot(lane), (double)t);
        continue;
      }
      const int r1 = __builtin_amdgcn_readlane(r, 63);
      if (r0 >= 0 && r1 >= 0 && (in_first | __ballot(r == r1)) == ~0ull) {
        const bool first = r == r0;
        const float tot = wave_sum4_f32(v[0], v[1], v[2], v[3]);
        const float fst = wave_sum4_f32(first ? v[0] : 0.f, first ? v[1] : 0.f, first ? v[2] : 0.f, first ? v[3] : 0.f);
        if (kFold) {
          const float f0 = rl_f32(fst, 15), f1 = rl_f32(fst, 47);
          const float f2 = rl_f32(fst, 31), f3 = rl_f32(fst, 63);
          add_run(f0, f1, f2, f3, qf[i]);
          add_run(rl_f32(tot, 15) - f0, rl_f32(tot, 47) - f1, rl_f32(tot, 31) - f2, rl_f32(tot, 63) - f3, ql[i]);
        } else if ((lane & 15) == 15) {
          const int k = wave_sum4_slot(lane);
          unsafeAtomicAdd(p.seg + (int64_t)r0 * 4 + k, (double)fst);
          unsafeAtomicAdd(p.seg + (int64_t)r1 * 4 + k, (double)(tot - fst));
        }
        continue;
      }
      const int prev = __shfl_up(r, 1, 64);
      int flag = (lane == 0 || prev != r) ? 1 : 0;
      const int next_head = __shfl_down(flag, 1, 64);
      const bool tail = active && (lane == 63 || next_head != 0 || e + 1 >= p.n_edges);
#pragma unroll
      for (int off = 1; off < 64; off <<= 1) {
        const int f_up = __shfl_up(flag, off, 64);
        float u[4];
#pragma unroll
        for (int k = 0; k < 4; ++k) u[k] = __shfl_up(v[k], off, 64);
        if (lane >= off && !flag) {
#pragma unroll
          for (int k = 0; k < 4; ++k) v[k] += u[k];
          flag = f_up;
        }
      }
      if (!kFold) {
        if (tail) {
#pragma unroll
          for (int k = 0; k < 4; ++k) unsafeAtomicAdd(p.seg + (int64_t)r * 4 + k, (double)v[k]);
        }
        continue;
      }
      unsigned long long tails = __ballot(tail);
      while (tails) {
        const int tl = __builtin_amdgcn_readfirstlane(__ffsll((long long)tails) - 1);
        tails &= tails - 1;
        const int rt = __builtin_amdgcn_readlane(r, tl);
        add_run(rl_f32(v[0], tl), rl_f32(v[1], tl), rl_f32(v[2], tl),
                rl_f32(v[3], tl), p.Q[(int64_t)rt * kH + k32]);
      }
    }
    base += stride;
    if (base < e_end) fetch(base);
  }
  EK_T(3, 3);
  {
    const int wid = threadIdx.x >> 6;
    double* sm_m = red;
    double* sm_c = red + 14 * 4;
    double* sm_m1 = sm_c + 4 * 128;
    wave_sums_f64<14>(acc, sm_m + wid * 14);
    sm_c[wid * 128 + (2 * hh) * 32 + k32] = c0;
    sm_c[wid * 128 + (2 * hh + 1) * 32 + k32] = c1;
    __syncthreads();
    double* m_dst = p.stats + kRoundMOff + (blockIdx.x % kStatRep) * kMStride;
    if (threadIdx.x < 14) {
      const double t = sm_m[threadIdx.x] + sm_m[14 + threadIdx.x] + sm_m[28 + threadIdx.x] + sm_m[42 + threadIdx.x];
      unsafeAtomicAdd(m_dst + threadIdx.x, t);
      if (threadIdx.x < 4) sm_m1[threadIdx.x] = t;
    }
    if (threadIdx.x >= 64 && threadIdx.x < 64 + 128) {
      const int i = threadIdx.x - 64;
      sm_c[i] = sm_c[i] + sm_c[128 + i] + sm_c[256 + i] + sm_c[384 + i];
    }
    __syncthreads();
    if (kFold && threadIdx.x < 32) {
      const int k = threadIdx.x;
      const float* a = p.un_w + k * p.un_ld + p.un_eoff;
      double lin = 0, cross = 0;
#pragma unroll
      for (int j = 0; j < 4; ++j) {
        lin += (double)a[j] * sm_m1[j];
        cross += (double)a[j] * sm_c[j * 32 + k];
      }
      double* z_dst = p.stats + kRoundZ2Off + (blockIdx.x % kStatRep) * kZ2Stride;
      unsafeAtomicAdd(z_dst + k, lin);
      unsafeAtomicAdd(z_dst + 32 + k, 2.0 * cross);
    }
  }
  EK_T(3, 4);
}

void launch_pass_b(const RoundParams& p, hipStream_t s) {
  switch (pick_ept(p.n_edges)) {
    case 1: hipLaunchKernelGGL(pass_b_kernel<1>, dim3(edge_grid(p.n_edges, 256)), dim3(256), 0, s, p); break;
    default: hipLaunchKernelGGL(pass_b_kernel<4>, dim3(edge_grid(p.n_edges, 1024)), dim3(256), 0, s, p);
  }
}
bool fold_node_stat(int64_t n_edges) { return pick_ept(n_edges) == 1; }

#if EK_STAMP
int ek_stamps_pass_b(unsigned long long* out) { return (int)hipMemcpyFromSymbol(out, HIP_SYMBOL(g_ek), sizeof(g_ek)); }
#endif

}
```

### graph-convolutional-network-for-multi-camera-vehicle-tracking_amd/csrc/edge_pass_c.hip

```cpp
#include "edge_common.h"

namespace mtmc {


__device__ __forceinline__ void flush_run(const RoundParams& p, bool det, int64_t chunk, int slot, int node, int k,
                                          float acc);

__device__ __forceinline__ void flush_node(const RoundParams& p, int node, int k, float acc) {
  float* dst = p.h_acc + (int64_t)node * kH + k;
  if (p.agg == 2) {
    atomicMax(reinterpret_cast<int*>(dst), __float_as_int(acc));
  } else {
    unsafeAtomicAdd(dst, acc);
  }
}

__device__ __forceinline__ void flush_run(const RoundParams& p, bool det, int64_t chunk, int slot, int node, int k,
                                          float acc) {
  if (!det) { flush_node(p, node, k, acc); return; }
  if (slot < 0) p.h_acc[(int64_t)node * kH + k] = acc;
  else p.carry[(chunk * 2 + slot) * kH + k] = acc;
}

__global__ __launch_bounds__(256) void agg_fixup_kernel(RoundParams p) {
// ... 45 lines not shown
constexpr int kTileC = 256;
__global__ __launch_bounds__(kTileC) void pass_c_kernel(RoundParams p) {
  drop_resolve(p.drop_n);
  __shared__ float4 tile_e[kTileC];
  __shared__ int tile_row[kTileC];
  __shared__ double st[10 + 64];
  __shared__ Z1AffineShared z1s;
  const int k = threadIdx.x & 31;
  const int hw = threadIdx.x >> 5;
  int64_t e_first = 0;
  if ((p.pass_c == kPassCAnyWalk || p.pass_c == kPassCSortedDet) && p.flags[0] == 0) return;
  if (p.pass_c == kPassCSortedWalk && p.flags[0] == 0) {
    e_first = p.n_edges & ~(int64_t)63;
    if (e_first == p.n_edges) return;
  }
  const int64_t n_tiles = (p.n_edges + kTileC - 1) / kTileC;
  int64_t tile = e_first / kTileC + blockIdx.x;
  if (tile >= n_tiles) return;
  float4 ev;
  int rw;
  auto fetch = [&](int64_t t) {
    const int64_t e = t * kTileC + threadIdx.x;
    ev = make_float4(0, 0, 0, 0);
    rw = 0;
    if (e < p.n_edges) {
      ev = reinterpret_cast<const float4*>(p.e_out)[e];
      rw = p.row32[e];
    }
  };
  if (tile < n_tiles) fetch(tile);
  const NodeUpdAffine af = node_upd_affine(p, p.lazy_e, k, 0, st, z1s);
  const float sk = af.sk, cb = af.cb;
  float a4[4];
#pragma unroll
  for (int j = 0; j < 4; ++j) a4[j] = sk * p.un_w[k * p.un_ld + p.un_eoff + j];
  const bool det = p.det && p.agg != 2 && p.flags[0] == 0;

  while (tile < n_tiles) {
    const int64_t base = tile * kTileC;
    const int64_t e = base + threadIdx.x;
    if (p.lazy_e) lazy_relu4(ev, z1s.s1, z1s.t1);
    if (e < p.n_edges) {
      tile_row[threadIdx.x] = rw;
      if (p.logits && e >= e_first) {
        float lg[MTMC_MAX_CLASSES];
        classify_edge(p.cls_w, p.cls_b, p.n_classes, ev, lg);
        if (p.n_classes == 2) {
          reinterpret_cast<float2*>(p.logits)[e] = make_float2(lg[0], lg[1]);
        } else {
          for (int c = 0; c < p.n_classes; ++c) p.logits[e * p.n_classes + c] = lg[c];
        }
      }
    }
    tile_e[threadIdx.x] = ev;
    __syncthreads();
    const int n_here = base + hw * 32 < e_first ? 0 : (int)min((int64_t)32, p.n_edges - (base + hw * 32));
    const int64_t chunk = (base >> 5) + hw;
    int cur = -1;
    bool first = true;
    float acc = 0.f, c0 = 0.f;
    unsigned long long zd = 0;
    for (int j = 0; j < n_here; ++j) {
      const int r = tile_row[hw * 32 + j];
      const float4 v = tile_e[hw * 32 + j];
      if (p.drop_n.on && (j & 3) == 0)
        zd = drop_hash4(p.drop_n.seed, p.drop_stream + 1, drop_msg_index(base + hw * 32 + j, k, p.n_edges) >> 2);
      if (r != cur) {
        if (cur >= 0) { flush_run(p, det, chunk, first ? 0 : -1, cur, k, acc); first = false; }
        cur = r;
        acc = 0.f;
        c0 = fmaf(sk, p.Q[(int64_t)r * kH + k], cb);
      }
      float m = fmaxf(fmaf(a4[3], v.w, fmaf(a4[2], v.z, fmaf(a4[1], v.y, fmaf(a4[0], v.x, c0)))), 0.f);
      if (p.drop_n.on) m = drop_field(p.drop_n, zd, j & 3) ? m * p.drop_n.inv_keep : 0.f;
      acc = (p.agg == 2) ? fmaxf(acc, m) : acc + m;
    }
    if (cur >= 0) flush_run(p, det, chunk, first ? 0 : 1, cur, k, acc);
    tile += gridDim.x;
    if (tile < n_tiles) fetch(tile);
    __syncthreads();
  }
}

template <bool DROP, bool DET, typename C0Of, typename Account>
__device__ __forceinline__ void several_rows_group(const RoundParams& p, const NodeUpdAffine& af, const f32x16c& acc, int rw,
                                                   int g, unsigned gm, int k, int hi, unsigned keep, float ikn, C0Of c0_of,
                                                   Account account) {
  auto relu_c0 = [&](int i, float c0) -> float {
    const float t = fmaxf(acc[i] + c0, 0.f);
    return DROP ? t * (((keep >> i) & 1u) ? ikn : 0.f) : t;
  };
  int n_rows = 0;
  if (!DET) {
    unsigned left = gm;
    while (left != 0 && n_rows <= 4) {
      const int r = __builtin_amdgcn_readfirstlane(__shfl(rw, 32 * g + __ffs(left) - 1, 64));
      left &= ~((unsigned)(__ballot(rw == r) >> (32 * g)));
      ++n_rows;
    }
  }
  if (!DET && n_rows > 4) {
#pragma unroll
    for (int i = 0; i < 16; ++i) {
      const int off = (i & 3) + 8 * (i >> 2) + 4 * hi;
      const int r = __shfl(rw, 32 * g + off, 64);
      if ((gm >> off) & 1u)
        unsafeAtomicAdd(p.h_acc + (int64_t)r * kH + k, relu_c0(i, fmaf(af.sk, p.Q[(int64_t)r * kH + k], af.cb)));
    }
    return;
  }
  unsigned done = 0;
  while (done != gm) {
    const int pos = __ffs(gm & ~done) - 1;
    const int r = __builtin_amdgcn_readfirstlane(__shfl(rw, 32 * g + pos, 64));
    const unsigned same = (unsigned)(__ballot(rw == r) >> (32 * g)) & gm & ~done;
    done |= same;
    const float c0 = c0_of(r);
    const unsigned mine = same >> (4 * hi);
    float sacc = 0.f;
#pragma unroll
    for (int i = 0; i < 16; ++i) sacc += ((mine >> ((i & 3) + 8 * (i >> 2))) & 1u) ? relu_c0(i, c0) : 0.f;
    account(r, sacc);
  }
}


template <bool DROP>
__global__ __launch_bounds__(256, (DROP ? 3 : 1)) void pass_c_mfma_kernel(RoundParams p, int span_c) {
  if (DROP) drop_resolve(p.drop_n);
  __shared__ double st[10 + 64];
  __shared__ Z1AffineShared z1s;
  const int lane = threadIdx.x & 63;
  const int wid = __builtin_amdgcn_readfirstlane(threadIdx.x >> 6);
  const int k = lane & 31, hi = lane >> 5;
  if (p.pass_c == kPassCAnyWalk && p.flags[0] != 0) return;
  EK_T(4, 0);
  const NodeUpdAffine af = node_upd_affine(p, p.lazy_e, k, 4, st, z1s);
  const float sk = af.sk, cb = af.cb;
  const float b0 = sk * p.un_w[k * p.un_ld + p.un_eoff + hi];
  const float b1 = sk * p.un_w[k * p.un_ld + p.un_eoff + 2 + hi];
  const bool want_logits = p.logits != nullptr;
  const Cls2 cls = cls2_load(p.cls_w, p.cls_b, want_logits && p.n_classes == 2);

  EK_T(4, 2);
  const int64_t n_chunks = (p.n_edges + 63) / 64;
  const int64_t n_spans = (n_chunks + span_c - 1) / span_c;
  const int64_t wave_stride = (int64_t)gridDim.x * 4;
  for (int64_t span = (int64_t)blockIdx.x * 4 + wid; span < n_spans; span += wave_stride) {
    int cur = -1;
    float run = 0.f;
    auto flush = [&]() {
      if (cur >= 0) {
        const float tot = run + __shfl_xor(run, 32, 64);
        if (hi == 0) unsafeAtomicAdd(p.h_acc + (int64_t)cur * kH + k, tot);
      }
    };
    const int64_t c_end = min(n_chunks, (span + 1) * span_c);
    auto fetch = [&](int64_t chunk, float4& ev_o, int& rw_o) {
      const int64_t e = min(chunk * 64 + lane, p.n_edges - 1);
      ev_o = reinterpret_cast<const float4*>(p.e_out)[e];
      rw_o = p.row32[e];
    };
    auto rows_of = [&](int rw_raw, int64_t chunk, int& first, int& last) {
      const int nv = (int)min((int64_t)64, p.n_edges - chunk * 64);
      first = __builtin_amdgcn_readfirstlane(rw_raw);
      last = __builtin_amdgcn_readfirstlane(__shfl(rw_raw, (nv > 0 ? nv : 1) - 1, 64));
    };
    int qa_row = -1, qb_row = -1;
    float qa = 0.f, qb = 0.f;
    auto c0_of = [&](int r) -> float {
      const float q = r == qa_row ? qa : (r == qb_row ? qb : p.Q[(int64_t)r * kH + k]);
      return fmaf(sk, q, cb);
    };
    auto account = [&](int r, float part) {
      if (r != cur) {
        flush();
        cur = r;
        run = 0.f;
      }
      run += part;
    };
    unsigned keepbits[2] = {0u, 0u};
    const float ikn = DROP ? p.drop_n.inv_keep : 1.f;
    auto keepf = [&](int g, int i) -> float { return ((keepbits[g] >> i) & 1u) ? ikn : 0.f; };
    auto relu_sum = [&](const f32x16c& acc, int g) -> float {
      float s0 = 0.f, s1 = 0.f;
#pragma unroll
      for (int i = 0; i < 16; i += 2) {
        const float t0 = __int_as_float(max(__float_as_int(acc[i]), 0)), t1 = __int_as_float(max(__float_as_int(acc[i + 1]), 0));
        s0 += DROP ? t0 * keepf(g, i) : t0;
        s1 += DROP ? t1 * keepf(g, i + 1) : t1;
      }
      return s0 + s1;
    };
    const int64_t c0_chunk = span * span_c;
    float4 ev_1, ev_2;
    int rw_1, rw_2;
    fetch(c0_chunk, ev_1, rw_1);
    rows_of(rw_1, c0_chunk, qa_row, qb_row);
    qa = p.Q[(int64_t)qa_row * kH + k];
    qb = p.Q[(int64_t)qb_row * kH + k];
    ev_2 = ev_1; rw_2 = rw_1;
    if (c0_chunk + 1 < c_end) fetch(c0_chunk + 1, ev_2, rw_2);
    for (int64_t chunk = c0_chunk; chunk < c_end; ++chunk) {
      int qa_row_2 = qa_row, qb_row_2 = qb_row;
      float qa_2 = qa, qb_2 = qb;
      if (chunk + 1 < c_end) {
        rows_of(rw_2, chunk + 1, qa_row_2, qb_row_2);
        qa_2 = p.Q[(int64_t)qa_row_2 * kH + k];
        qb_2 = p.Q[(int64_t)qb_row_2 * kH + k];
      }
      float4 ev_3 = ev_2;
      int rw_3 = rw_2;
      if (chunk + 2 < c_end) fetch(chunk + 2, ev_3, rw_3);
      const int64_t e = chunk * 64 + lane;
      const bool valid = e < p.n_edges;
      float4 ev = make_float4(0.f, 0.f, 0.f, 0.f);
      if (valid) {
        ev = ev_1;
        if (p.lazy_e) lazy_relu4(ev, af.s1, af.t1);
      }
      const int rw = valid ? rw_1 : -1;
      const int n_valid = (int)min((int64_t)64, p.n_edges - chunk * 64);
      if (DROP) {
        keepbits[0] = keepbits[1] = 0u;
#pragma unroll
        for (int g = 0; g < 2; ++g)
#pragma unroll
          for (int q = 0; q < 4; ++q) {
            const unsigned long long zd =
                drop_hash4(p.drop_n.seed, p.drop_stream + 1, drop_msg_index(chunk * 64 + 32 * g + 8 * q + 4 * hi, k, p.n_edges) >> 2);
#pragma unroll
            for (int j = 0; j < 4; ++j) keepbits[g] |= drop_field(p.drop_n, zd, j) ? (1u << (4 * q + j)) : 0u;
          }
      }
      float2 lg = make_float2(0.f, 0.f);
      if (want_logits && p.n_classes == 2) lg = classify_edge(cls, ev);
      const auto xy = __builtin_amdgcn_permlane32_swap(__float_as_uint(ev.x), __float_as_uint(ev.y), false, false);
      const auto zw = __builtin_amdgcn_permlane32_swap(__float_as_uint(ev.z), __float_as_uint(ev.w), false, false);
      const unsigned long long row_first_mask = __ballot(rw == qa_row), row_last_mask = __ballot(rw == qb_row);
      const int nv1 = n_valid - 32;
      const unsigned gmv[2] = {n_valid >= 32 ? 0xffffffffu : ((1u << n_valid) - 1u),
                               nv1 >= 32 ? 0xffffffffu : (nv1 > 0 ? ((1u << nv1) - 1u) : 0u)};
      int ra[2], rb[2];
      unsigned ma[2], mb[2];
      bool two_rows_max[2];
#pragma unroll
      for (int g = 0; g < 2; ++g) {
        ra[g] = rb[g] = -1;
        ma[g] = mb[g] = 0;
        two_rows_max[g] = true;
        if (gmv[g] == 0) continue;
        ra[g] = g == 0 ? qa_row : __builtin_amdgcn_readlane(rw, 32);
        const unsigned long long fa = g == 0 ? row_first_mask : (ra[g] == qb_row ? row_last_mask : __ballot(rw == ra[g]));
        ma[g] = (unsigned)(fa >> (32 * g)) & gmv[g];
        const unsigned rest = gmv[g] & ~ma[g];
        if (rest != 0) {
          rb[g] = __builtin_amdgcn_readfirstlane(__shfl(rw, 32 * g + __ffs(rest) - 1, 64));
          const unsigned long long fb = rb[g] == qb_row ? row_last_mask : __ballot(rw == rb[g]);
          mb[g] = (unsigned)(fb >> (32 * g)) & gmv[g];
          two_rows_max[g] = (ma[g] | mb[g]) == gmv[g];
        }
      }
      if (want_logits && valid) {
        if (p.n_classes == 2) reinterpret_cast<float2*>(p.logits)[e] = lg;
        else classify_edge(p.cls_w, p.cls_b, p.n_classes, ev, p.logits + e * p.n_classes);
      }
      if (two_rows_max[0] && two_rows_max[1]) {
        f32x16c acc[2];
#pragma unroll
        for (int g = 0; g < 2; ++g) {
          const unsigned long long member = (unsigned long long)ma[g] | ((unsigned long long)mb[g] << 32);
          const float a_c = __builtin_amdgcn_inverse_ballot_w64(member) ? 1.0f : 0.0f;
          const float c_a = ra[g] >= 0 ? c0_of(ra[g]) : 0.f, c_b = rb[g] >= 0 ? c0_of(rb[g]) : 0.f;
          f32x16c z = {};
          acc[g] = __builtin_amdgcn_mfma_f32_32x32x2f32(a_c, hi == 0 ? c_a : c_b, z, 0, 0, 0);
        }
#pragma unroll
        for (int g = 0; g < 2; ++g) acc[g] = __builtin_amdgcn_mfma_f32_32x32x2f32(__uint_as_float(xy[g]), b0, acc[g], 0, 0, 0);
#pragma unroll
        for (int g = 0; g < 2; ++g) acc[g] = __builtin_amdgcn_mfma_f32_32x32x2f32(__uint_as_float(zw[g]), b1, acc[g], 0, 0, 0);
#pragma unroll
        for (int g = 0; g < 2; ++g) {
          if (ra[g] < 0) break;
          const float total = relu_sum(acc[g], g);
          if (rb[g] < 0) {
            account(ra[g], total);
          } else {
            float sa0 = 0.f, sa1 = 0.f;
#pragma unroll
            for (int i = 0; i < 16; ++i) {
              const int c = (i & 3) + 8 * (i >> 2);
              const unsigned long long in_a = (((ma[g] >> c) & 1u) ? 0xffffffffull : 0ull) |
                                              (((ma[g] >> (c + 4)) & 1u) ? 0xffffffff00000000ull : 0ull);
              const float t0 = __int_as_float(max(__float_as_int(acc[g][i]), 0));
              const float t = DROP ? t0 * keepf(g, i) : t0;
              const float v = __builtin_amdgcn_inverse_ballot_w64(in_a) ? t : 0.f;
              if (i & 1) sa1 += v; else sa0 += v;
            }
            const float sa = sa0 + sa1;
            account(ra[g], sa);
            account(rb[g], total - sa);
          }
        }
      } else {
#pragma unroll
        for (int g = 0; g < 2; ++g) {
          const unsigned gm = gmv[g];
          if (gm == 0) break;
          f32x16c acc = {};
          acc = __builtin_amdgcn_mfma_f32_32x32x2f32(__uint_as_float(xy[g]), b0, acc, 0, 0, 0);
          acc = __builtin_amdgcn_mfma_f32_32x32x2f32(__uint_as_float(zw[g]), b1, acc, 0, 0, 0);
          several_rows_group<DROP, false>(p, af, acc, rw, g, gm, k, hi, keepbits[g], ikn, c0_of, account);
        }
      }
      ev_1 = ev_2; rw_1 = rw_2;
      ev_2 = ev_3; rw_2 = rw_3;
      qa_row = qa_row_2; qb_row = qb_row_2;
      qa = qa_2; qb = qb_2;
    }
    flush();
  }
  EK_T(4, 3);
}

template <bool LAZY, bool DET>
__global__ __launch_bounds__(256) void pass_c_sorted_kernel(RoundParams p, int span_c) {
  __shared__ double st[10 + 64];
  __shared__ Z1AffineShared z1s;
  const int lane = threadIdx.x & 63;
  const int wid = __builtin_amdgcn_readfirstlane(threadIdx.x >> 6);
  const int k = lane & 31, hi = lane >> 5;
  if (p.flags[0] != 0) return;
  const NodeUpdAffine af = node_upd_affine(p, LAZY, k, 0, st, z1s);
  const float sk = af.sk, cb = af.cb;
  const float b0 = sk * p.un_w[k * p.un_ld + p.un_eoff + hi];
  const float b1 = sk * p.un_w[k * p.un_ld + p.un_eoff + 2 + hi];
  const bool two_class = p.logits != nullptr && p.n_classes == 2;
  const Cls2 cls = cls2_load(p.cls_w, p.cls_b, two_class);
  const int lim_hi = 4 * hi;
  const unsigned koff = (unsigned)k * 4u;

  const int n_full = (int)(p.n_edges >> 6);
  const int n_tail = (int)(p.n_edges & 63);
  const int n_spans = ((DET && n_tail ? n_full + 1 : n_full) + span_c - 1) / span_c;
  const int wave_stride = (int)gridDim.x * 4;
  for (int span = (int)blockIdx.x * 4 + wid; span < n_spans; span += wave_stride) {
    int cur = -1;
    float run = 0.f;
    bool first_run = true;
    auto flush = [&](bool last) {
      if (cur >= 0) {
        const auto sw = __builtin_amdgcn_permlane32_swap(__float_as_uint(run), __float_as_uint(run), false, false);
        const float tot = run + __uint_as_float(hi == 0 ? sw[1] : sw[0]);
        if (!DET) {
          if (hi == 0) unsafeAtomicAdd(p.h_acc + (int64_t)cur * kH + k, tot);
        } else if (hi == 0) {
          if (first_run) p.carry[((int64_t)span * 2 + 0) * kH + k] = tot;
          else if (last) p.carry[((int64_t)span * 2 + 1) * kH + k] = tot;
          else p.h_acc[(int64_t)cur * kH + k] = tot;
        }
        first_run = false;
      }
    };
    auto account = [&](int r, float part) {
      if (r != cur) {
        flush(false);
        cur = r;
        run = 0.f;
      }
      run += part;
    };
    auto c0_of = [&](int r) -> float { return fmaf(sk, p.Q[(int64_t)r * kH + k], cb); };
    auto slow_group = [&](const f32x16c& acc, int rwc, int g, unsigned gm) {
      several_rows_group<false, DET>(p, af, acc, rwc, g, gm, k, hi, 0u, 1.f, c0_of, account);
    };
    const int c_beg = span * span_c, c_end = min(n_full, c_beg + span_c);
    float4 ev[3];
    int rw[3];
    float qv[3][2];
    int rows[3][4];
    auto fetch = [&](int c, int slot) {
      const int cc = min(c, n_full - 1);
      const int64_t e0 = (int64_t)cc * 64;
#if PC_NT
      {
        typedef float f4v __attribute__((ext_vector_type(4)));
        const f4v v = __builtin_nontemporal_load(reinterpret_cast<const f4v*>(p.e_out + e0 * 4) + lane);
        ev[slot] = make_float4(v[0], v[1], v[2], v[3]);
        rw[slot] = __builtin_nontemporal_load(p.row32 + e0 + lane);
      }
#else
      ev[slot] = reinterpret_cast<const float4*>(p.e_out + e0 * 4)[lane];
      rw[slot] = (p.row32 + e0)[lane];
#endif
    };
// ... 70 lines not shown
        }
      } else {
#pragma unroll
        for (int g = 0; g < 2; ++g) {
          f32x16c acc = {};
          acc = __builtin_amdgcn_mfma_f32_32x32x2f32(__uint_as_float(xy[g]), b0, acc, 0, 0, 0);
          acc = __builtin_amdgcn_mfma_f32_32x32x2f32(__uint_as_float(zw[g]), b1, acc, 0, 0, 0);
          slow_group(acc, rwc, g, 0xffffffffu);
        }
      }
    };
    fetch(c_beg, 0);
    fetch(c_beg + 1, 1);
    lookup(0);
    for (int c = c_beg; c < c_end; c += 3) {
      step(c, 0, 1, 2);
      if (c + 1 < c_end) step(c + 1, 1, 2, 0);
      if (c + 2 < c_end) step(c + 2, 2, 0, 1);
    }
    if (DET && n_tail && span == n_spans - 1) {
      const int64_t e = (int64_t)n_full * 64 + lane;
      const bool valid = lane < n_tail;
      const int64_t ec = valid ? e : p.n_edges - 1;
      float4 e4 = reinterpret_cast<const float4*>(p.e_out)[ec];
      const int rwc = valid ? p.row32[ec] : -1;
      if (LAZY) lazy_relu4(e4, af.s1, af.t1);
      if (p.logits != nullptr && valid) classify_edge(p.cls_w, p.cls_b, p.n_classes, e4, p.logits + e * p.n_classes);
      const auto xy = __builtin_amdgcn_permlane32_swap(__float_as_uint(e4.x), __float_as_uint(e4.y), false, false);
      const auto zw = __builtin_amdgcn_permlane32_swap(__float_as_uint(e4.z), __float_as_uint(e4.w), false, false);
#pragma unroll
      for (int g = 0; g < 2; ++g) {
        const int nv = n_tail - 32 * g;
        const unsigned gm = nv >= 32 ? 0xffffffffu : (nv > 0 ? ((1u << nv) - 1u) : 0u);
        if (gm == 0) break;
        f32x16c acc = {};
        acc = __builtin_amdgcn_mfma_f32_32x32x2f32(__uint_as_float(xy[g]), b0, acc, 0, 0, 0);
        acc = __builtin_amdgcn_mfma_f32_32x32x2f32(__uint_as_float(zw[g]), b1, acc, 0, 0, 0);
        slow_group(acc, rwc, g, gm);
      }
    }
    flush(true);
  }
}

constexpr int64_t kSortedMaxNodes = 1ll << 24;
static bool pass_c_sorted_taken(int64_t n_nodes) { return !knobs().pass_c_general && n_nodes < kSortedMaxNodes; }

PassC plan_pass_c(int agg, bool deterministic, bool dropout, int64_t n_edges, int64_t n_nodes, double avg_degree) {
  const Knobs& kn = knobs();
  if (kn.pass_c_walk || agg == 2 || avg_degree < 24.0) return kPassCWalk;
  if (dropout && (n_edges > kSmallEdges || deterministic)) return kPassCWalk;
  const bool sorted = pass_c_sorted_taken(n_nodes);
  if (n_edges > kSmallEdges) {
    if (deterministic) return sorted ? kPassCSortedDet : kPassCWalk;
    return sorted ? kPassCSortedWalk : kPassCAnyWalk;
  }
  if (deterministic) return (sorted && n_edges > kDetSortedEdges) ? kPassCSortedDet : kPassCWalk;
  return n_edges >= kn.pass_c_small_min ? kPassCAny : kPassCWalk;
}

void launch_pass_c(const RoundParams& p0, hipStream_t s) {
  RoundParams p = p0;
  p.det_len = 32;
  const int span_env = knobs().pass_c_span, max_blocks = knobs().pass_c_blocks;
  if (p.pass_c == kPassCSortedWalk || p.pass_c == kPassCSortedDet) {
    const bool det = p.pass_c == kPassCSortedDet;
    const int64_t n_full = p.n_edges >> 6;
    int64_t blocks = (n_full + 3) / 4;
    if (blocks > max_blocks) blocks = max_blocks;
    if (blocks < 1) blocks = 1;
    const int64_t per_wave = (n_full + blocks * 4 - 1) / (blocks * 4), m = (per_wave + 47) / 48;
    const int span_c = span_env > 0 ? span_env : (int)((per_wave + (m > 0 ? m : 1) - 1) / (m > 0 ? m : 1));
    const int sc = span_c > 0 ? span_c : 1;
    p.det_len = det ? sc * 64 : 32;
    const dim3 grid((int)blocks);
    if (det) {
      if (p.lazy_e) hipLaunchKernelGGL((pass_c_sorted_kernel<true, true>), grid, dim3(256), 0, s, p, sc);
      else hipLaunchKernelGGL((pass_c_sorted_kernel<false, true>), grid, dim3(256), 0, s, p, sc);
    } else {
      if (p.lazy_e) hipLaunchKernelGGL((pass_c_sorted_kernel<true, false>), grid, dim3(256), 0, s, p, sc);
      else hipLaunchKernelGGL((pass_c_sorted_kernel<false, false>), grid, dim3(256), 0, s, p, sc);
    }
  } else if (p.pass_c != kPassCWalk) {
    const int span_c = span_env > 0 ? span_env : (p.pass_c == kPassCAny ? 1 : 8);
    const int64_t spans = ((p.n_edges + 63) / 64 + span_c - 1) / span_c, blocks = (spans + 3) / 4;
    const int cap = max_blocks < 256 * 3 ? max_blocks : 256 * 3;
    if (p.drop_n.on) hipLaunchKernelGGL(pass_c_mfma_kernel<true>, dim3((int)(blocks > cap ? cap : blocks)), dim3(256), 0, s, p, span_c);
    else hipLaunchKernelGGL(pass_c_mfma_kernel<false>, dim3((int)(blocks > cap ? cap : blocks)), dim3(256), 0, s, p, span_c);
  }
#ifdef MTMC_WALK_TAIL_GRID
  if (p.pass_c == kPassCSortedWalk || p.pass_c == kPassCSortedDet) {
    hipLaunchKernelGGL(pass_c_kernel, dim3(MTMC_WALK_TAIL_GRID), dim3(kTileC), 0, s, p);
  } else
#endif
  if (p.pass_c != kPassCAny) hipLaunchKernelGGL(pass_c_kernel, dim3(edge_grid(p.n_edges, kTileC)), dim3(kTileC), 0, s, p);
  if (p.det && p.agg != 2) {
    const int64_t blocks = (p.n_nodes + 7) / 8;
    hipLaunchKernelGGL(agg_fixup_kernel, dim3((int)(blocks < 1 ? 1 : (blocks > 2048 ? 2048 : blocks))), dim3(256), 0, s, p);
  }
}

#if EK_STAMP
static int ek_stamps_pass_c(unsigned long long* out) { return (int)hipMemcpyFromSymbol(out, HIP_SYMBOL(g_ek), sizeof(g_ek)); }
#endif

}

#if EK_STAMP
extern "C" int mtmc_dbg_ek_stamps_edge(unsigned long long* out) {
  constexpr int n = mtmc::kEkKernels * 2 * mtmc::kEkPoints;
  unsigned long long a[n], b[n];
  const int err = mtmc::ek_stamps_pass_a(a) | mtmc::ek_stamps_pass_b(b) | mtmc::ek_stamps_pass_c(out);
  for (int i = 0; i < n; ++i) out[i] += a[i] + b[i];
  return err;
}
#endif
```

### graph-convolutional-network-for-multi-camera-vehicle-tracking_amd/csrc/kernels.h

```cpp
#pragma once
#include "../../include/mtmc_mpn.h"
#include "common.h"
#include <type_traits>

namespace mtmc {

struct Knobs {
  bool pass_c_walk;
  int64_t pass_c_small_min;
  int staged_xr;
  int presplit_rows;
  bool pass_c_general;
  int pass_c_span;
  int pass_c_blocks;
  bool gemm_fp32;
  bool gemm_no_f16;
  bool gemm_no_presplit;
  bool gemm_no_staged;
  bool no_col_blocks;
  int col_blocks;
  int l0_pipeline;
  bool gemm_no_few;
  int few_rows_max;
  int few_l0_map;
  int few_wave_rb;
};
const Knobs& knobs();

constexpr int kAmaxRep = 16;
enum { kJobAmax = 0, kJobSplit = 1 };
struct AmaxJob { const float* ptr; int64_t rows; int cols; int64_t ld; unsigned* out; int block0, n_blocks;
                 int kind; _Float16* planes; float* inv; unsigned long long* fp; };

struct PrepEdge {
  int n_edge_blocks = 0;
  const int64_t* row; const int64_t* col; int64_t idx_stride;
  const float* attr; int fe;
  int64_t n_edges; int64_t n_nodes;
  int* row32; int* col32; int* deg; int* flags; int* row_start;
  double* stat_attr;
};
struct PrepParams : PrepEdge {
  int n_jobs;
  int n_pass_blocks;
  AmaxJob jobs[2 * MTMC_MAX_ENC_LAYERS + 2];
};

enum PassC : int {
  kPassCWalk = 0,
  kPassCAnyWalk = 1,
  kPassCAny = 2,
  kPassCSortedWalk = 3,
  kPassCSortedDet = 4,
};

struct RoundParams {
  const int* row32; const int* col32; const float* attr;
  const float* e_prev;
  float* e_buf;
  float* e_out;
  Drop drop_e, drop_n; unsigned drop_stream;
  const float* P;
  const float* Q;
  double* seg;
  int fold_z2;
  const float* ue_w; const float* ue_b; const float* ue_g; const float* ue_bt; int ue_ld; int ue_eoff;
  const float* un_w; const float* un_b; const float* un_g; const float* un_bt; int un_ld; int un_eoff;
  const float* cls_w; const float* cls_b; int n_classes;
  double* stats;
  float* h_acc;
  float* logits;
  int64_t n_edges; double e_total;
  int first_round; int reattach_edges; int agg;
  int lazy_e; const double* prev_stats;
  PassC pass_c;
  int stream_z1;
  int det_len;
  int det; const int* flags; const int* deg; const int* row_start; float* carry; int64_t n_nodes;
  double avg_degree;
  int col_blocks = 0; const int* col_sub = nullptr; int64_t cb_row_lo = 0, cb_row_hi = 0;
  EdgeEncParams enc;
};

struct NodeProjParams {
  const float* y_last; const double* y_stats; const float* y_gamma; const float* y_beta; double y_count; float* h0_out;
  int finalize_enc; EdgeEncParams enc; double e_total;
  Drop drop; unsigned drop_stream;
  const float* h_src;
  const float* h0;
  const int* deg;
  const float* ue_w; int ue_ld;
  const float* un_w; int un_ld;
  int hn;
  float* P; float* Q;
  float* zero_buf;
  int64_t n_nodes;
  int64_t node_begin, node_end;
  const int* edge_deg; const float* un_b; double* z2_stats;
};

struct NodeStatParams {
  const float* Q; const int* deg; double* seg;
  const float* un_w; const float* un_b; int un_ld; int un_eoff;
  double* stats;
  int64_t n_nodes;
  int64_t node_begin, node_end;
};

struct ActIn {
  const float* A = nullptr; int64_t lda = 0;
  const double* stats_in = nullptr;
  const float* gamma_in = nullptr; const float* beta_in = nullptr;
  double count = 0;
  Drop drop_in = kNoDrop; unsigned drop_stream = 0;
};
struct PlanesA { const _Float16* Ah = nullptr; const float* inv_a = nullptr; };
struct PlanesW { const _Float16* Wh = nullptr; const float* inv_w = nullptr; };
struct LayerOut {
  const float* bias = nullptr;
  float* Y = nullptr; int64_t ldy = 0;
  double* stats_out = nullptr;
  unsigned* amax_y = nullptr;
  int64_t M = 0; int K = 0; int Nout = 0;
};
struct Enc2Ride {
  int pass_blocks = 0; EdgeEncParams pass_enc = {}; const float* pass_attr = nullptr; int64_t pass_edges = 0;
  double pass_e_total = 0; double* pass_stat = nullptr;
};

struct GemmParams : ActIn, LayerOut, Enc2Ride {
  const float* W = nullptr;
  float* slab = nullptr;
  int split_k = 1;
  const unsigned* amax_a = nullptr;
  const unsigned* amax_w = nullptr;
};
inline void set_in(ActIn* q, const float* A, int64_t lda, const double* stats_in = nullptr, const float* gamma_in = nullptr,
                   const float* beta_in = nullptr, double count = 0) {
  q->A = A; q->lda = lda; q->stats_in = stats_in; q->gamma_in = gamma_in; q->beta_in = beta_in; q->count = count;
}
inline void set_out(LayerOut* q, const float* bias, float* Y, int64_t ldy, int64_t M, int K, int Nout, double* stats_out = nullptr,
                    unsigned* amax_y = nullptr) {
  q->bias = bias; q->Y = Y; q->ldy = ldy; q->M = M; q->K = K; q->Nout = Nout; q->stats_out = stats_out; q->amax_y = amax_y;
}
inline GemmParams plain_gemm(const float* A, int64_t lda, const float* W, const float* bias, float* Y, int64_t ldy, int64_t M,
                             int K, int Nout, const unsigned* amax_a = nullptr, const unsigned* amax_w = nullptr,
                             unsigned* amax_y = nullptr) {
  GemmParams g;
  g.W = W; g.amax_a = amax_a; g.amax_w = amax_w;
  set_in(&g, A, lda);
  set_out(&g, bias, Y, ldy, M, K, Nout, nullptr, amax_y);
  return g;
}

struct FewL0Params : PlanesA, PlanesW, LayerOut {};
struct FewWaveParams : ActIn, PlanesW, LayerOut, Enc2Ride {
  int tiles = 0;
};
bool few_l0_shape(int K, int Nout);
bool few_wave_shape(int K, int Nout);
int few_wave_threads(int K);
bool few_rows_path(int64_t rows, int n_layers, const int* in_dim, const int* out_dim);
int launch_few_l0(const FewL0Params& p, hipStream_t s);
int launch_few_wave(const FewWaveParams& p, hipStream_t s);

struct SplitGemmParams : PlanesA, PlanesW, LayerOut {
  int64_t m_lo = 0; int64_t M_rows = 0; int bm = 0;
};
struct StagedGemmParams : ActIn, PlanesW, LayerOut {
  const unsigned* amax_a = nullptr;
};
static_assert(std::is_trivially_copyable<GemmParams>::value && std::is_trivially_copyable<FewL0Params>::value &&
              std::is_trivially_copyable<FewWaveParams>::value && std::is_trivially_copyable<SplitGemmParams>::value &&
              std::is_trivially_copyable<StagedGemmParams>::value, "the blocks are passed to kernels by value");
bool staged_layer(int64_t rows, int K, int Nout);
int launch_gemm_staged(const StagedGemmParams& p, hipStream_t s);
int staged_tile_rows(int64_t M, int tiles_n, int wm);
bool rows_layer(int64_t rows, int K, int Nout);
// ... 77 lines not shown
```

### graph-convolutional-network-for-multi-camera-vehicle-tracking_amd/csrc/node_kernels.hip

```cpp
#include "kernels.h"
#include "rows_body.h"

namespace mtmc {

#ifndef MTMC_PROJ_MFMA_MIN
#define MTMC_PROJ_MFMA_MIN 1
#endif
constexpr int64_t kProjMfmaMinRows = MTMC_PROJ_MFMA_MIN;
constexpr int kProjNodes = 16;
constexpr int kProjOut = 40;

__global__ __launch_bounds__(256) void node_proj_kernel(NodeProjParams p) {
  drop_resolve(p.drop);
  __shared__ float wt[64 * kProjOut];
  __shared__ float hs[kProjNodes * 66];
  __shared__ float ys[kH], yt[kH];
  __shared__ EdgeEncAffine enc_af;
  __shared__ double scratch[kStatAttr + kStatEnc2];
  __shared__ double zred[4][2 * kH];
  double zs1[4] = {0, 0, 0, 0}, zs2[4] = {0, 0, 0, 0};
  const int hn = p.hn, ldh = hn + 2;
  EK_T(0, 0);
  for (int i = threadIdx.x; i < hn * kProjOut; i += blockDim.x) {
    const int kk = i / kProjOut, j = i % kProjOut;
    float w;
    if (j < 4) w = p.ue_w[j * p.ue_ld + kk];
    else if (j < 8) w = p.ue_w[(j - 4) * p.ue_ld + hn + kk];
    else w = p.un_w[(j - 8) * p.un_ld + kk];
    wt[i] = w;
  }
  if (p.y_last && threadIdx.x < kH)
    bn_affine(p.y_stats[threadIdx.x], p.y_stats[kH + threadIdx.x], p.y_count, p.y_gamma[threadIdx.x],
              p.y_beta[threadIdx.x], ys[threadIdx.x], yt[threadIdx.x]);
  const int nl = threadIdx.x >> 4, part = (threadIdx.x >> 1) & 7, kh = threadIdx.x & 1;
  float ubv[4] = {0.f, 0.f, 0.f, 0.f};
  if (p.z2_stats) {
#pragma unroll
    for (int i = 0; i < 4; ++i) ubv[i] = p.un_b[part + 8 * i];
  }
  const int64_t n_groups = (p.node_end - p.node_begin + kProjNodes - 1) / kProjNodes;
  for (int64_t g = blockIdx.x; g < n_groups; g += gridDim.x) {
    const int64_t node0 = p.node_begin + g * kProjNodes;
    const double dnode = (p.z2_stats && node0 + nl < p.node_end) ? (double)p.edge_deg[node0 + nl] : 0.0;
    __syncthreads();
    EK_T(0, 1);
    for (int i = threadIdx.x; i < kProjNodes * kH; i += blockDim.x) {
      const int n = i >> 5, kk = i & 31;
      const int64_t node = node0 + n;
      float v = 0.f;
      if (node < p.node_end) {
        if (p.y_last) {
          v = drop_apply(p.drop, p.drop_stream, (unsigned long long)node * kH + kk,
                         fmaxf(fmaf(p.y_last[node * kH + kk], ys[kk], yt[kk]), 0.f));
          p.h0_out[node * kH + kk] = v;
        } else {
          v = p.h_src[node * kH + kk];
          if (p.deg) { const int d = p.deg[node]; v = v / (float)(d > 1 ? d : 1); }
        }
      }
      hs[n * ldh + (hn - kH) + kk] = v;
      if (hn == 2 * kH) hs[n * ldh + kk] = (p.y_last || node >= p.node_end) ? v : p.h0[node * kH + kk];
    }
    if (p.zero_buf && threadIdx.x < kProjNodes * 8) {
      const int64_t node = node0 + (threadIdx.x >> 3);
      if (node < p.node_end)
        reinterpret_cast<float4*>(p.zero_buf + node * kH)[threadIdx.x & 7] = make_float4(0.f, 0.f, 0.f, 0.f);
    }
    __syncthreads();
    EK_T(0, 2);
    float acc[5] = {0.f, 0.f, 0.f, 0.f, 0.f};
    for (int kk = kh; kk < hn; kk += 2) {
      const float hv = hs[nl * ldh + kk];
#pragma unroll
      for (int i = 0; i < 5; ++i) acc[i] = fmaf(hv, wt[kk * kProjOut + part + 8 * i], acc[i]);
    }
#pragma unroll
    for (int i = 0; i < 5; ++i) acc[i] += __shfl_xor(acc[i], 1, 64);
    const int64_t node = node0 + nl;
    if (kh == 0 && node < p.node_end) {
      p.P[(part < 4 ? node : p.n_nodes + node) * 4 + (part & 3)] = acc[0];
#pragma unroll
      for (int i = 1; i < 5; ++i) p.Q[node * kH + part + 8 * (i - 1)] = acc[i];
      if (p.z2_stats) {
#pragma unroll
        for (int i = 1; i < 5; ++i) {
          const double qb = (double)(acc[i] + ubv[i - 1]);
          zs1[i - 1] += dnode * qb;
          zs2[i - 1] += dnode * qb * qb;
        }
      }
    }
  }
  EK_T(0, 3);
  if (p.z2_stats) {
#pragma unroll
    for (int i = 0; i < 4; ++i) {
      zs1[i] += __shfl_xor(zs1[i], 16, 64); zs2[i] += __shfl_xor(zs2[i], 16, 64);
      zs1[i] += __shfl_xor(zs1[i], 32, 64); zs2[i] += __shfl_xor(zs2[i], 32, 64);
    }
    __syncthreads();
    if ((threadIdx.x & 63) < 16 && kh == 0) {
#pragma unroll
      for (int i = 0; i < 4; ++i) {
        zred[threadIdx.x >> 6][part + 8 * i] = zs1[i];
        zred[threadIdx.x >> 6][kH + part + 8 * i] = zs2[i];
      }
    }
    __syncthreads();
    if (threadIdx.x < 2 * kH)
      unsafeAtomicAdd(p.z2_stats + (blockIdx.x % kStatRep) * kZ2Stride + threadIdx.x,
                      zred[0][threadIdx.x] + zred[1][threadIdx.x] + zred[2][threadIdx.x] + zred[3][threadIdx.x]);
  }
  EK_T(0, 4);
  if (p.finalize_enc && blockIdx.x == 0) {
    edge_enc_affine_to_smem(p.enc, p.e_total, 2, &enc_af, scratch);
    if (threadIdx.x < 16) p.enc.aff[threadIdx.x] = reinterpret_cast<const float*>(&enc_af)[threadIdx.x];
  }
  EK_T(0, 5);
}

typedef float f32x4p __attribute__((ext_vector_type(4)));

template <int HALVES>
__global__ __launch_bounds__(256) void node_proj_mfma_kernel(NodeProjParams p) {
  drop_resolve(p.drop);
  __shared__ float ys[kH], yt[kH];
  __shared__ EdgeEncAffine enc_af;
  __shared__ double scratch[kStatAttr + kStatEnc2];
  __shared__ double zred[4][2 * kH];
  double zs1[2] = {0, 0}, zs2[2] = {0, 0};
  const int lane = threadIdx.x & 63, wid = threadIdx.x >> 6;
  const int i16 = lane & 15, g = lane >> 4;
  const float ub0 = p.z2_stats ? p.un_b[i16] : 0.f, ub1 = p.z2_stats ? p.un_b[16 + i16] : 0.f;
  EK_T(5, 0);
  float bw[3][HALVES][8];
#pragma unroll
  for (int nb = 0; nb < 3; ++nb)
#pragma unroll
    for (int hf = 0; hf < HALVES; ++hf)
#pragma unroll
      for (int s8 = 0; s8 < 8; ++s8) {
        const int kk = 32 * hf + 8 * g + s8;
        float w = 0.f;
        if (nb < 2) w = p.un_w[(16 * nb + i16) * p.un_ld + kk];
        else if (i16 < 4) w = p.ue_w[i16 * p.ue_ld + kk];
        else if (i16 < 8) w = p.ue_w[(i16 - 4) * p.ue_ld + p.hn + kk];
        bw[nb][hf][s8] = w;
      }
  if (p.y_last) {
    if (threadIdx.x < kH)
      bn_affine(p.y_stats[threadIdx.x], p.y_stats[kH + threadIdx.x], p.y_count, p.y_gamma[threadIdx.x],
                p.y_beta[threadIdx.x], ys[threadIdx.x], yt[threadIdx.x]);
    __syncthreads();
  }
  float ysv[8], ytv[8];
  if (p.y_last) {
#pragma unroll
    for (int s8 = 0; s8 < 8; ++s8) { ysv[s8] = ys[8 * g + s8]; ytv[s8] = yt[8 * g + s8]; }
  }
  EK_T(5, 1);
  const int64_t n_groups = (p.node_end - p.node_begin + 15) / 16;
  for (int64_t grp = (int64_t)blockIdx.x * 4 + wid; grp < n_groups; grp += (int64_t)gridDim.x * 4) {
    const int64_t node = p.node_begin + grp * 16 + i16;
    const bool live = node < p.node_end;
    const int64_t nd = live ? node : p.node_end - 1;
    double dg[4] = {0, 0, 0, 0};
    if (p.z2_stats) {
#pragma unroll
      for (int r = 0; r < 4; ++r) {
        const int64_t on = p.node_begin + grp * 16 + 4 * g + r;
        dg[r] = (double)p.edge_deg[on < p.node_end ? on : p.node_end - 1];
      }
    }
    float a[HALVES][8];
    {
      const float* src = (p.y_last ? p.y_last : p.h_src) + nd * kH + 8 * g;
      const float4 v0 = *reinterpret_cast<const float4*>(src), v1 = *reinterpret_cast<const float4*>(src + 4);
      float v[8] = {v0.x, v0.y, v0.z, v0.w, v1.x, v1.y, v1.z, v1.w};
      if (p.y_last) {
#pragma unroll
        for (int s8 = 0; s8 < 8; ++s8)
          v[s8] = drop_apply(p.drop, p.drop_stream, (unsigned long long)nd * kH + 8 * g + s8,
                             fmaxf(fmaf(v[s8], ysv[s8], ytv[s8]), 0.f));
        if (live) {
          *reinterpret_cast<float4*>(p.h0_out + node * kH + 8 * g) = make_float4(v[0], v[1], v[2], v[3]);
          *reinterpret_cast<float4*>(p.h0_out + node * kH + 8 * g + 4) = make_float4(v[4], v[5], v[6], v[7]);
        }
      } else if (p.deg) {
        const int d = p.deg[nd];
        const float sc = (float)(d > 1 ? d : 1);
#pragma unroll
        for (int s8 = 0; s8 < 8; ++s8) v[s8] = v[s8] / sc;
      }
#pragma unroll
      for (int s8 = 0; s8 < 8; ++s8) a[HALVES - 1][s8] = v[s8];
      if (HALVES == 2) {
        if (p.y_last) {
#pragma unroll
          for (int s8 = 0; s8 < 8; ++s8) a[0][s8] = v[s8];
        } else {
          const float* s0 = p.h0 + nd * kH + 8 * g;
          const float4 u0 = *reinterpret_cast<const float4*>(s0), u1 = *reinterpret_cast<const float4*>(s0 + 4);
          a[0][0] = u0.x; a[0][1] = u0.y; a[0][2] = u0.z; a[0][3] = u0.w;
          a[0][4] = u1.x; a[0][5] = u1.y; a[0][6] = u1.z; a[0][7] = u1.w;
        }
      }
    }
    if (p.zero_buf && live) {
      *reinterpret_cast<float4*>(p.zero_buf + node * kH + 8 * g) = make_float4(0.f, 0.f, 0.f, 0.f);
      *reinterpret_cast<float4*>(p.zero_buf + node * kH + 8 * g + 4) = make_float4(0.f, 0.f, 0.f, 0.f);
    }
    f32x4p acc[3];
#pragma unroll
    for (int nb = 0; nb < 3; ++nb) {
      acc[nb] = f32x4p{0.f, 0.f, 0.f, 0.f};
#pragma unroll
      for (int hf = 0; hf < HALVES; ++hf)
#pragma unroll
        for (int s8 = 0; s8 < 8; ++s8) acc[nb] = __builtin_amdgcn_mfma_f32_16x16x4f32(a[hf][s8], bw[nb][hf][s8], acc[nb], 0, 0, 0);
    }
#pragma unroll
    for (int r = 0; r < 4; ++r) {
      const int64_t on = p.node_begin + grp * 16 + 4 * g + r;
      if (on < p.node_end) {
        p.Q[on * kH + i16] = acc[0][r];
        p.Q[on * kH + 16 + i16] = acc[1][r];
        if (i16 < 8) p.P[(i16 < 4 ? on : p.n_nodes + on) * 4 + (i16 & 3)] = acc[2][r];
        if (p.z2_stats) {
          const double d = dg[r];
          const double q0 = (double)(acc[0][r] + ub0), q1 = (double)(acc[1][r] + ub1);
          zs1[0] += d * q0; zs2[0] += d * q0 * q0;
          zs1[1] += d * q1; zs2[1] += d * q1 * q1;
        }
      }
    }
  }
  EK_T(5, 2);
  if (p.z2_stats) {
#pragma unroll
    for (int c = 0; c < 2; ++c) {
      zs1[c] += __shfl_xor(zs1[c], 16, 64); zs2[c] += __shfl_xor(zs2[c], 16, 64);
      zs1[c] += __shfl_xor(zs1[c], 32, 64); zs2[c] += __shfl_xor(zs2[c], 32, 64);
    }
    if (lane < 16) {
#pragma unroll
      for (int c = 0; c < 2; ++c) {
        zred[wid][16 * c + i16] = zs1[c];
        zred[wid][kH + 16 * c + i16] = zs2[c];
      }
    }
    __syncthreads();
    if (threadIdx.x < 2 * kH)
      unsafeAtomicAdd(p.z2_stats + (blockIdx.x % kStatRep) * kZ2Stride + threadIdx.x,
                      zred[0][threadIdx.x] + zred[1][threadIdx.x] + zred[2][threadIdx.x] + zred[3][threadIdx.x]);
  }
  EK_T(5, 3);
  if (p.finalize_enc && blockIdx.x == 0) {
    __syncthreads();
    edge_enc_affine_to_smem(p.enc, p.e_total, 2, &enc_af, scratch);
    if (threadIdx.x < 16) p.enc.aff[threadIdx.x] = reinterpret_cast<const float*>(&enc_af)[threadIdx.x];
  }
  EK_T(5, 4);
}

__global__ __launch_bounds__(256) void node_stat_kernel(NodeStatParams p) {
  __shared__ double red[2 * 8 * 32];
  const int k = threadIdx.x & 31, slot = threadIdx.x >> 5;
  float a[4];
#pragma unroll
  for (int j = 0; j < 4; ++j) a[j] = p.un_w[k * p.un_ld + p.un_eoff + j];
  const float b = p.un_b[k];
  double s1 = 0, s2 = 0;
  const int64_t n_groups = (p.node_end - p.node_begin + 7) / 8;
  for (int64_t g = blockIdx.x; g < n_groups; g += gridDim.x) {
    const int64_t node = p.node_begin + g * 8 + slot;
    if (node < p.node_end) {
      const double d = (double)p.deg[node];
      const double qb = (double)(p.Q[node * kH + k] + b);
      double proj = 0;
#pragma unroll
      for (int j = 0; j < 4; ++j) proj += (double)a[j] * p.seg[node * 4 + j];
      s1 += d * qb + proj;
      s2 += d * qb * qb + 2.0 * qb * proj;
    }
    __syncthreads();
    if (node < p.node_end && k < 4) p.seg[node * 4 + k] = 0.0;
  }
  red[slot * 32 + k] = s1;
  red[256 + slot * 32 + k] = s2;
  __syncthreads();
  if (threadIdx.x < 64) {
    const int kk = threadIdx.x & 31, which = threadIdx.x >> 5;
    double s = 0;
// ... 91 lines not shown
```

### graph-convolutional-network-for-multi-camera-vehicle-tracking_amd/engine.py

```python
from __future__ import annotations

import ctypes as C
import types
from typing import List

import torch

from . import _lib
from .config import MpnSpec


def _check_param(p: torch.Tensor, dev) -> int:
    if p.device != dev or p.dtype != torch.float32 or not p.is_contiguous():
        raise RuntimeError("mtmc_mpn: parameters must be contiguous float32 tensors on the input's device "
                           f"(got {p.dtype} on {p.device})")
    if p.data_ptr() % 16:
        raise RuntimeError("mtmc_mpn: parameters must be 16-byte aligned (a view at an odd storage offset? use .clone())")
    return p.data_ptr()


def layer_slots(spec: MpnSpec):
    out = [("enc_node", i, l) for i, l in enumerate(spec.enc_node)]
    out += [("enc_edge", i, l) for i, l in enumerate(spec.enc_edge)]
    out += [("upd_edge", None, spec.upd_edge[0]), ("upd_node", None, spec.upd_node[0]), ("cls", None, spec.cls_edge[0])]
# ... 79 lines not shown
                "upd_node": m.MPNet.node_model.node_mlp, "cls": m.classifier.edge_mlp}
        return [((slot, idx), mlps[slot].fc_layers[l.lin_slot],
                 mlps[slot].fc_layers[l.bn_slot] if l.bn_slot is not None else None, l) for slot, idx, l in self._slots]

    def params(self) -> List[torch.Tensor]:
        if self.module is None:
            raise RuntimeError("mtmc_mpn: no parameters given")
        return ordered_params(self.module)

    def model_struct(self, dev, params=None, dropout=True) -> _lib.Model:
        params = self.params() if params is None else params
        key = (dev,) + tuple((t.data_ptr(), t.dtype, t.shape, t.stride()) for t in params)
        if key != self._ms_key:
            it = iter(params)

            def pointers(slot, idx, layer):
                w, b = next(it), next(it)
                if tuple(w.shape) != (layer.out_dim, layer.in_dim) or tuple(b.shape) != (layer.out_dim,):
                    raise RuntimeError(f"mtmc_mpn: parameter shapes of {slot}[{idx}] do not match the configuration")
                ptrs = _check_param(w, dev), _check_param(b, dev)
                if layer.bn_slot is None:
                    return ptrs + (None, None)
                return ptrs + (_check_param(next(it), dev), _check_param(next(it), dev))
            try:
                out = _fill_model(_lib.Model(), self.spec, self._slots, pointers, dropout=True)
            except StopIteration:
                raise RuntimeError("mtmc_mpn: parameter list shorter than the configuration needs") from None
            self._ms_key, self._ms = key, out
        out = _lib.Model.from_buffer_copy(self._ms)
        if not dropout:
            out.dropout_enc = out.dropout_upd_edge = out.dropout_upd_node = 0.0
        return out

    def shape_model(self, dropout=False) -> _lib.Model:
        return _fill_model(_lib.Model(), self.spec, self._slots, _placeholder_pointers, dropout)

    def workspace(self, model, n, e, dev, stream_ptr) -> torch.Tensor:
        need = self.lib.mtmc_mpn_workspace_bytes(C.byref(model), n, e)
        if need == 0:
            _lib.check(_lib.E_ARG)
        key = (dev, stream_ptr)
        ws = self._ws.get(key)
        if ws is None or ws.numel() < need:
            ws = torch.empty(int(need * 1.25) + 256, dtype=torch.uint8, device=dev)
            self._ws[key] = ws
        return ws

    def weight_plane_cache(self, model, dev, stream_ptr) -> torch.Tensor:
        key = (dev, stream_ptr)
        buf = self._wc.get(key)
        if buf is None:
            need = self.lib.mtmc_mpn_weight_cache_bytes(C.byref(model))
            if need == 0:
                _lib.check(_lib.E_ARG)
            buf = self._wc[key] = torch.zeros(need + 256, dtype=torch.uint8, device=dev)
        return buf

    def take_stream_buffers(self, dev, stream_ptr) -> list:
        key = (dev, stream_ptr)
        return [buf for buf in (self._ws.pop(key, None), self._wc.pop(key, None)) if buf is not None]

    def check_inputs(self, x, edge_index, edge_attr):
        if not (isinstance(x, torch.Tensor) and x.is_cuda and edge_index.is_cuda and edge_attr.is_cuda):
            raise RuntimeError("mtmc_mpn: data.x / edge_index / edge_attr must be on a ROCm GPU -- "
                               "this module has no CPU or PyTorch fallback path")
        if not (x.device == edge_index.device == edge_attr.device):
            raise RuntimeError("mtmc_mpn: all inputs must be on the same device")
        s = self.spec
        if x.dim() != 2 or x.shape[1] != s.enc_node[0].in_dim:
            raise RuntimeError(f"mtmc_mpn: data.x must be [N, {s.enc_node[0].in_dim}], got {tuple(x.shape)}")
        if edge_index.dim() != 2 or edge_index.shape[0] != 2:
            raise RuntimeError(f"mtmc_mpn: data.edge_index must be [2, E], got {tuple(edge_index.shape)}")
        e = edge_index.shape[1]
        if edge_attr.dim() != 2 or tuple(edge_attr.shape) != (e, s.enc_edge[0].in_dim):
            raise RuntimeError(f"mtmc_mpn: data.edge_attr must be [{e}, {s.enc_edge[0].in_dim}], got {tuple(edge_attr.shape)}")
        if x.dtype != torch.float32 or edge_attr.dtype != torch.float32:
            raise RuntimeError("mtmc_mpn: x and edge_attr must be float32")
        if edge_index.dtype != torch.int64:
            raise RuntimeError("mtmc_mpn: edge_index must be int64")

    def call_struct(self, n_nodes, n_edges, n_edges_total=None, node_lo=0, node_hi=None, row_range=None, training=False,
                    flags=None, weight_cache=None) -> _lib.Call:
        if flags is None:
            flags = _lib.F_DETERMINISTIC if getattr(self.module, "deterministic", False) else 0
        if weight_cache is None:
            weight_cache = getattr(self.module, "cache_weight_planes", True)
        call = _lib.Call()
        call.n_nodes, call.n_edges = int(n_nodes), int(n_edges)
        call.n_edges_total = int(n_edges if n_edges_total is None else n_edges_total)
        call.node_lo, call.node_hi = int(node_lo), int(n_nodes if node_hi is None else node_hi)
        call.row_lo, call.row_hi = _row_range(row_range)
        call.training, call.flags = int(bool(training)), int(flags)
        if weight_cache:
            call.weight_cache, call.weight_cache_bytes = 256, 1 << 62
        return call

    def prepare(self, x, edge_index, edge_attr, training=False, n_edges_total=None, node_range=None, tape=False,
                seed=0, row_range=None, params=None, tape_ws=None, flags=None, weight_cache=None):
        self.check_inputs(x, edge_index, edge_attr)
        s, dev = self.spec, x.device
        e = edge_index.shape[1]
        node_lo, node_hi = (0, x.shape[0]) if node_range is None else node_range[:2]
        n = x.shape[0] if node_range is None else node_range[2]
        if not (0 <= node_lo <= node_hi <= n) or x.shape[0] != node_hi - node_lo:
            raise RuntimeError(f"mtmc_mpn: node_range {(node_lo, node_hi, n)} does not describe the {x.shape[0]} rows of x")
        if row_range is not None and not (0 <= int(row_range[0]) <= int(row_range[1]) <= n):
            raise RuntimeError(f"mtmc_mpn: row_range {tuple(row_range)} is not inside [0, {n}]")
        if x.stride(1) != 1 or x.stride(0) % 4 != 0:
            x = x.contiguous()
        if not edge_attr.is_contiguous():
            edge_attr = edge_attr.contiguous()
        if e > 0 and edge_index.stride(1) < 1:
            edge_index = edge_index.contiguous()
        n_out = n_classified_steps(s)
        n_cls = s.cls_edge[0].out_dim
        logits = torch.empty((n_out, e, n_cls), dtype=torch.float32, device=dev)
        h = torch.empty((n, s.node_dim), dtype=torch.float32, device=dev)
        with torch.cuda.device(dev):
            stream = torch.cuda.current_stream(dev).cuda_stream
        model = self.model_struct(dev, params, dropout=training or not tape)
        if tape_ws is not None:
            ws = tape_ws
        elif tape:
            need = self.lib.mtmc_mpn_train_workspace_bytes(C.byref(model), n, e)
            if need == 0:
                _lib.check(_lib.E_ARG)
            ws = torch.empty(need + 256, dtype=torch.uint8, device=dev)
        else:
            ws = self.workspace(model, n, e, dev, stream)
        call = self.call_struct(n, e, n_edges_total, node_lo, node_hi, row_range, tape, flags,
                                False if tape_ws is not None else weight_cache)
        call.x, call.x_row_stride = x.data_ptr(), x.stride(0)
        call.row = edge_index[0].data_ptr() if e > 0 else None
        call.col = edge_index[1].data_ptr() if e > 0 else None
        call.idx_stride = edge_index.stride(1) if e > 0 else 1
        call.edge_attr = edge_attr.data_ptr() if e > 0 else ws.data_ptr()
        call.logits = logits.data_ptr() if logits.numel() else ws.data_ptr()
        call.h_out = h.data_ptr()
        call.workspace, call.workspace_bytes = ws.data_ptr(), ws.numel()
        call.seed = int(seed) & 0xFFFFFFFFFFFFFFFF
        keep = (x, edge_index, edge_attr)
        if call.weight_cache:
            wc = self.weight_plane_cache(model, dev, stream)
            call.weight_cache, call.weight_cache_bytes = wc.data_ptr(), wc.numel()
            keep = keep + (wc,)
        call.stream = stream
        return types.SimpleNamespace(model=model, call=call, ws=ws, logits=logits, h=h, n_out=n_out, n=n, e=e,
                                     dev=dev, keep=keep)

    def plan(self, n_nodes, n_edges, n_edges_total=None, node_range=None, row_range=None, training=False, flags=0,
             params=None, device=None, weight_cache=True) -> types.SimpleNamespace:
        model = self.shape_model(dropout=True)
        node_lo, node_hi = (0, None) if node_range is None else node_range[:2]
        call = self.call_struct(n_nodes, n_edges, n_edges_total, node_lo, node_hi, row_range, training, flags, weight_cache)
        out = _lib.Plan()
        _lib.check(self.lib.mtmc_mpn_plan_call(C.byref(model), C.byref(call), C.byref(out)))
        n_layers = len(self.spec.enc_node)
        return types.SimpleNamespace(enc_kernel=list(out.enc_kernel)[:n_layers], enc_split_k=list(out.enc_split_k)[:n_layers],
                                     edges_per_thread=out.edges_per_thread, lazy_edges=bool(out.lazy_edges),
                                     pass_c=out.pass_c, avg_degree=out.avg_degree, pass_a_col_blocks=out.pass_a_col_blocks,
                                     layer0_panels=out.layer0_panels, enc2_passenger=bool(out.enc2_passenger),
                                     node_stat_folded=bool(out.node_stat_folded))

    def phase_list(self):
        s = self.spec
        seq = [(_lib.PH_BEGIN, 0), (_lib.PH_EDGE_ENC, 0)]
        for l in range(len(s.enc_node)):
            seq += [(_lib.PH_NODE_ENC, l), (_lib.PH_NODE_COMBINE, l)]
        seq += [(_lib.PH_NODE_H0, 0)]
        for r in range(s.num_enc_steps):
            seq += [(_lib.PH_ROUND_PROJ, r), (_lib.PH_ROUND_A, r), (_lib.PH_ROUND_B, r), (_lib.PH_ROUND_STAT, r),
                    (_lib.PH_ROUND_C, r)]
        return seq + [(_lib.PH_END, 0)]

    def run_phase(self, prep, ph, arg):
        with torch.cuda.device(prep.dev):
            _lib.check(self.lib.mtmc_mpn_run_phase(C.byref(prep.model), C.byref(prep.call), ph, arg))

    def run_phase_list(self, prep, pairs):
        flat = (C.c_int32 * (2 * len(pairs)))(*[v for pair in pairs for v in pair])
        with torch.cuda.device(prep.dev):
            _lib.check(self.lib.mtmc_mpn_run_phases(C.byref(prep.model), C.byref(prep.call), flat, len(pairs)))

    def set_flags(self, prep, flags):
        prep.call.flags = int(flags)

    def region(self, prep, name, idx=0) -> torch.Tensor:
        lay = getattr(prep, "_layout", None)
        if lay is None:
            lay = prep._layout = self.layout(prep)
        ws, n, s = prep.ws, prep.n, self.spec
        R = _lib.STAT_REPLICAS

        def f64(off, count):
            return ws[off:off + 8 * count].view(torch.float64)

        if name == "stat_attr":
            return f64(lay.stat_attr_off, R * _lib.ATTR_STRIDE)
        if name == "stat_enc2":
            return f64(lay.stat_enc2_off, R * _lib.ENC2_STRIDE)
        if name == "stat_enc_node":
            return f64(lay.stat_enc_layer_off[idx], 2 * s.enc_node[idx].out_dim)
        if name == "enc_merged":
            head = lay.stat_attr_off if idx == 0 else lay.stat_enc2_off
            end = lay.stat_enc_layer_off[idx] + 16 * s.enc_node[idx].out_dim
            return (f64(head, (end - head) // 8),)
        if name == "round_m_z2":
            base = lay.stat_round_off + 8 * idx * _lib.ROUND_BLOCK + 8 * R * _lib.Z1_STRIDE
            return (f64(base, R * (_lib.M_STRIDE + _lib.Z2_STRIDE)),)
        if name in ("round_z1", "round_m", "round_z2"):
            base = lay.stat_round_off + 8 * idx * _lib.ROUND_BLOCK
            if name == "round_z1":
                return f64(base, R * _lib.Z1_STRIDE)
            if name == "round_m":
                return f64(base + 8 * R * _lib.Z1_STRIDE, R * _lib.M_STRIDE)
            return f64(base + 8 * R * (_lib.Z1_STRIDE + _lib.M_STRIDE), R * _lib.Z2_STRIDE)
        if name == "deg":
            return ws[lay.deg_off:lay.deg_off + 4 * n].view(torch.int32)
        if name == "deg_global":
            return ws[lay.deg_global_off:lay.deg_global_off + 4 * n].view(torch.int32)
        if name == "h0":
            return ws[lay.h0_off:lay.h0_off + 128 * n].view(torch.float32).view(n, 32)
        if name == "Pc":
            off = lay.P_off + 16 * n
            return ws[off:off + 16 * n].view(torch.float32).view(n, 4)
        if name == "agg":
            if idx == s.num_enc_steps - 1 and s.agg != "mean":
                return prep.h
            off = lay.h_acc_off[idx & 1]
            return ws[off:off + 128 * n].view(torch.float32).view(n, 32)
        raise KeyError(name)

    def outputs(self, prep):
        return [prep.logits[i] for i in range(prep.n_out)], prep.h

    def layout(self, prep) -> _lib.WsLayout:
        lay = _lib.WsLayout()
        _lib.check(self.lib.mtmc_mpn_workspace_layout(C.byref(prep.model), prep.n, prep.e, C.byref(lay)))
        return lay

    def run_phases(self, prep, after_phase=None, before_phase=None):
        with torch.cuda.device(prep.dev):
            for ph, arg in self.phase_list():
                if before_phase is not None:
                    before_phase(ph, arg)
                self.run_phase(prep, ph, arg)
# ... 4 lines not shown
```

### graph-convolutional-network-for-multi-camera-vehicle-tracking_amd/modules.py

```python
from __future__ import annotations

from typing import Dict, List, Optional

import torch
from torch import nn

from . import _lib as _lib_flags
from . import config as _config
from .config import LayerSpec, MpnSpec


class MLP(nn.Module):

    def __init__(self, input_dim, fc_dims, dropout_p=0.4, use_batchnorm=False, is_classifier=False):
        super().__init__()
        self.layers: List[LayerSpec] = _config.plan_mlp(input_dim, fc_dims, dropout_p, use_batchnorm, is_classifier)
        seq: List[nn.Module] = []
        for spec in self.layers:
            seq.append(nn.Linear(spec.in_dim, spec.out_dim))
            if spec.bn_slot is not None:
                seq.append(nn.BatchNorm1d(spec.out_dim, track_running_stats=False))
            if spec.relu:
                seq.append(nn.ReLU(inplace=True))
            if spec.dropout_p is not None:
                seq.append(nn.Dropout(p=spec.dropout_p))
        self.fc_layers = nn.Sequential(*seq)

    def forward(self, input):
        from . import ops
        return ops.mlp_forward(self, input)


class MLPGraphIndependent(nn.Module):

    def __init__(self, edge_in_dim=None, node_in_dim=None, edge_out_dim=None, node_out_dim=None,
                 node_fc_dims=None, edge_fc_dims=None, dropout_p=None, use_batchnorm=None, is_classifier=False):
        super().__init__()
        self.node_mlp = None if node_in_dim is None else MLP(
            node_in_dim, list(node_fc_dims) + [node_out_dim], dropout_p, use_batchnorm, is_classifier)
        self.edge_mlp = None if edge_in_dim is None else MLP(
            edge_in_dim, list(edge_fc_dims) + [edge_out_dim], dropout_p, use_batchnorm, is_classifier)

    def forward(self, edge_feats=None, nodes_feats=None):
        out_nodes = self.node_mlp(nodes_feats) if (self.node_mlp is not None and nodes_feats is not None) else nodes_feats
        out_edges = self.edge_mlp(edge_feats) if (self.edge_mlp is not None and edge_feats is not None) else edge_feats
        return out_edges, out_nodes


class EdgeModel(nn.Module):

    def __init__(self, edge_mlp):
        super().__init__()
        self.edge_mlp = edge_mlp


class NodeModel(nn.Module):

    def __init__(self, node_mlp, node_agg_fn: str):
        super().__init__()
        self.node_mlp = node_mlp
        self.node_agg_fn = node_agg_fn


class MetaLayer(nn.Module):

    def __init__(self, edge_model=None, node_model=None):
        super().__init__()
        self.edge_model = edge_model
        self.node_model = node_model

    def __repr__(self):
        return "{}(edge_model={}, node_model={})".format(self.__class__.__name__, self.edge_model, self.node_model)


class MOTMPNet(nn.Module):

    def __init__(self, model_params: Dict, bb_encoder=None, arch: Optional[str] = None):
        super().__init__()
        self.node_cnn = bb_encoder
        self.model_params = model_params
        self.arch = arch
        self.spec: MpnSpec = _config.resolve(model_params, arch)
        ok, why = _config.check_supported(self.spec)
        if not ok:
            raise NotImplementedError("mtmc_mpn HIP path does not cover this GRAPH_NET_PARAMS: " + why)

        enc_e = model_params["encoder_feats_dict"]["edges"]
        enc_n = model_params["encoder_feats_dict"]["nodes"][arch]
        enc_e.update(enc_n)
        self.encoder = MLPGraphIndependent(**enc_e)
        self.classifier = MLPGraphIndependent(**model_params["classifier_feats_dict"])
        em, nm = model_params["edge_model_feats_dict"], model_params["node_model_feats_dict"]
        s = self.spec
        self.MPNet = MetaLayer(
            edge_model=EdgeModel(MLP(s.upd_edge[0].in_dim, em["fc_dims"], em["dropout_p"], em["use_batchnorm"])),
            node_model=NodeModel(MLP(s.upd_node[0].in_dim, nm["fc_dims"], nm["dropout_p"], nm["use_batchnorm"]),
                                 s.agg))
        self.reattach_initial_nodes = s.reattach_nodes
        self.reattach_initial_edges = s.reattach_edges
        self.num_enc_steps = s.num_enc_steps
        self.num_class_steps = s.num_class_steps
        self.check_indices = False
        self.deterministic = False
        self.cache_weight_planes = True
        self.device_seed = None
        self._engine = None

    def capture(self, data):
        if self.training:
            raise RuntimeError("mtmc_mpn: capture() is for eval-mode inference")
        from . import torch_ops
        dev = data.x.device
        with torch.no_grad():
            self.forward(data)
            op_engine = torch_ops.engine_for(self._config_key)
            side = torch.cuda.Stream(device=dev)
            side.wait_stream(torch.cuda.current_stream(dev))
            with torch.cuda.stream(side):
                self.forward(data)
            side.synchronize()
            graph = torch.cuda.CUDAGraph()
            with torch.cuda.graph(graph, stream=side):
                out = self.forward(data)
            torch.cuda.current_stream(dev).wait_stream(side)
            held = op_engine.take_stream_buffers(dev, side.cuda_stream) + [side]

        def replay():
            graph.replay()
            return out
        replay.graph, replay.workspaces = graph, held
        return replay

    def capture_training_step(self, data, loss_fn, optimizer, warmup=3):
        if not self.training:
            raise RuntimeError("mtmc_mpn: capture_training_step() is for .train() mode")
        dev = data.x.device
        if self.device_seed is None:
            self.device_seed = torch.randint(0, 2 ** 62, (1,), dtype=torch.int64).to(dev)
        side = torch.cuda.Stream(device=dev)
        side.wait_stream(torch.cuda.current_stream(dev))

        def step():
            outputs, h = self(data)
            loss = loss_fn(outputs, h)
            loss.backward()
            optimizer.step()
            return loss
        import gc
        import warnings
        gc.collect()
        warn_always = torch.is_warn_always_enabled()
        torch.set_warn_always(True)
        try:
            with torch.cuda.stream(side), warnings.catch_warnings(record=True) as caught:
                warnings.simplefilter("always")
                for _ in range(max(int(warmup), 1)):
                    optimizer.zero_grad(set_to_none=True)
                    step()
            side.synchronize()
        finally:
            torch.set_warn_always(warn_always)
        for w in caught:
            if "AccumulateGrad node's stream does not match" in str(w.message):
                raise RuntimeError("mtmc_mpn.capture_training_step: an earlier step's autograd graph is still alive (its loss or "
                                   "outputs are referenced somewhere): delete those references (`del loss, outputs`) and call again")
            warnings.warn_explicit(w.message, w.category, w.filename, w.lineno)
        optimizer.zero_grad(set_to_none=True)
        graph = torch.cuda.CUDAGraph()
        with torch.cuda.graph(graph, stream=side):
            loss = step()
        torch.cuda.current_stream(dev).wait_stream(side)
        from . import torch_ops
        held = torch_ops.engine_for(self._config_key).take_stream_buffers(dev, side.cuda_stream) + [side]

        def replay():
            graph.replay()
            return loss
        replay.graph, replay.workspaces = graph, held
        return replay

    def forward(self, data):
        from . import engine, torch_ops
        if self._engine is None:
            self._engine = engine.ForwardEngine(self)
            self._config_key = torch_ops.config_key(self.model_params, self.arch)
        x, edge_index, edge_attr = data.x, data.edge_index, data.edge_attr
        if not (isinstance(x, torch.Tensor) and x.is_cuda):
            raise RuntimeError("mtmc_mpn: data.x / edge_index / edge_attr must be on a ROCm GPU -- "
                               "this module has no CPU or PyTorch fallback path")
        params = engine.ordered_params(self)
        needs_grad = torch.is_grad_enabled() and (
            x.requires_grad or edge_attr.requires_grad or any(p.requires_grad for p in params))
        tape = bool(needs_grad or self.training)
        flags = (_lib_flags.F_DETERMINISTIC if self.deterministic else 0) | \
            (torch_ops.CHECK_INDICES if self.check_indices else 0) | \
            (0 if self.cache_weight_planes else torch_ops.NO_WEIGHT_CACHE)
        if self.training and self.device_seed is not None:
            ds = self.device_seed
            if not (isinstance(ds, torch.Tensor) and ds.dtype == torch.int64 and ds.numel() == 1 and ds.device == x.device):
                raise RuntimeError("mtmc_mpn: device_seed must be an int64 tensor of one element on the device of data.x")
            seed, flags = ds.data_ptr(), flags | _lib_flags.F_SEED_ON_DEVICE
        else:
            seed = int(torch.randint(0, 2 ** 62, (1,)).item()) if self.training else 0
        if tape and edge_index.is_cuda and edge_attr.is_cuda and not torch.compiler.is_compiling():
            steps, h = torch_ops.mp_forward_lean(x, edge_index, edge_attr, params, self._config_key, self.training, seed, flags)
            return {"classified_edges": steps}, h
        else:
            logits, h, _ = torch.ops.mtmc_mpn.mp_forward(x, edge_index, edge_attr, params, self._config_key,
                                                         self.training, seed, flags, tape)
        return {"classified_edges": list(logits.unbind(0))}, h
```

### include/mtmc_mpn.h

```cpp
#ifndef MTMC_MPN_H
#define MTMC_MPN_H

#include <stddef.h>
#include <stdint.h>

#ifdef __cplusplus
extern "C" {
#endif

#define MTMC_MPN_ABI_VERSION 6

#define MTMC_MAX_ENC_LAYERS 8
#define MTMC_NODE_DIM 32
#define MTMC_EDGE_DIM 4
#define MTMC_MAX_CLASSES 4

enum { MTMC_AGG_SUM = 0, MTMC_AGG_MEAN = 1, MTMC_AGG_MAX = 2 };

enum {
  MTMC_OK = 0,
  MTMC_E_ARG = -1,
  MTMC_E_WORKSPACE = -2,
  MTMC_E_HIP = -3,
  MTMC_E_ROWS = -4
};

typedef struct mtmc_layer {
  const float* weight;
  const float* bias;
  const float* gamma;
  const float* beta;
  int32_t in_dim;
  int32_t out_dim;
} mtmc_layer;

typedef struct mtmc_mpn_model {
  uint32_t struct_bytes;
  int32_t n_enc_layers;
  mtmc_layer enc_node[MTMC_MAX_ENC_LAYERS];
  mtmc_layer enc_edge[2];
  mtmc_layer upd_edge;
  mtmc_layer upd_node;
  mtmc_layer cls;
  int32_t agg;
  int32_t num_enc_steps;
  int32_t num_class_steps;
  int32_t reattach_nodes;
  int32_t reattach_edges;
  float dropout_enc;
  float dropout_upd_edge;
  float dropout_upd_node;
} mtmc_mpn_model;

typedef struct mtmc_mpn_call {
  uint32_t struct_bytes;
  const float* x;
  int64_t x_row_stride;
  const int64_t* row;
  const int64_t* col;
  int64_t idx_stride;
  const float* edge_attr;
  int64_t n_nodes;
  int64_t n_edges;
  int64_t n_edges_total;
  int64_t node_lo, node_hi;
  float* logits;
  float* h_out;
  void* workspace;
  size_t workspace_bytes;
  int32_t training;
  int32_t flags;
  uint64_t seed;
  void* stream;
  int64_t row_lo, row_hi;
  void* weight_cache;
  size_t weight_cache_bytes;
} mtmc_mpn_call;

#define MTMC_F_DETERMINISTIC 1
#define MTMC_F_GLOBAL_DEG 4
#define MTMC_F_FORK 2
#define MTMC_F_SEED_ON_DEVICE 16

#define MTMC_STAT_REPLICAS 16
#define MTMC_ATTR_STRIDE 16
#define MTMC_ENC2_STRIDE 16
#define MTMC_Z1_STRIDE 16
#define MTMC_M_STRIDE 16
#define MTMC_Z2_STRIDE 64
#define MTMC_ROUND_BLOCK (MTMC_STAT_REPLICAS * (MTMC_Z1_STRIDE + MTMC_M_STRIDE + MTMC_Z2_STRIDE))
typedef struct mtmc_ws_layout {
  size_t total_bytes;
  size_t zero_bytes;
  size_t flags_off;
  size_t stat_attr_off;
  size_t stat_enc2_off;
  size_t stat_enc_layer_off[MTMC_MAX_ENC_LAYERS];
  size_t stat_round_off;
  size_t deg_off;
  size_t seg_off;
  size_t h0_off;
  size_t h_acc_off[2];
  size_t deg_global_off;
  size_t P_off;
} mtmc_ws_layout;

enum {
  MTMC_PH_BEGIN = 0,
  MTMC_PH_EDGE_ENC = 1,
  MTMC_PH_NODE_ENC = 2,
  MTMC_PH_NODE_H0 = 3,
  MTMC_PH_ROUND_PROJ = 4,
  MTMC_PH_ROUND_A = 5,
  MTMC_PH_ROUND_B = 6,
  MTMC_PH_ROUND_STAT = 7,
  MTMC_PH_ROUND_C = 8,
  MTMC_PH_END = 9,
  MTMC_PH_NODE_COMBINE = 10
};

int32_t mtmc_mpn_abi_version(void);
const char* mtmc_mpn_last_error(void);
size_t mtmc_mpn_workspace_bytes(const mtmc_mpn_model* model, int64_t n_nodes, int64_t n_edges);
size_t mtmc_mpn_weight_cache_bytes(const mtmc_mpn_model* model);
int32_t mtmc_mpn_workspace_layout(const mtmc_mpn_model* model, int64_t n_nodes, int64_t n_edges,
                                  mtmc_ws_layout* out);
int32_t mtmc_mpn_forward(const mtmc_mpn_model* model, const mtmc_mpn_call* call);

size_t mtmc_mpn_train_workspace_bytes(const mtmc_mpn_model* model, int64_t n_nodes, int64_t n_edges);
int32_t mtmc_mpn_backward(const mtmc_mpn_model* model, const mtmc_mpn_call* call, const float* d_logits,
                          const float* d_h, const mtmc_mpn_model* grads, float* d_x, float* d_edge_attr);
int32_t mtmc_mpn_backward_steps(const mtmc_mpn_model* model, const mtmc_mpn_call* call,
                                const float* const* d_logits_steps, const float* d_h, const mtmc_mpn_model* grads,
                                void* grads_flat, size_t grads_flat_bytes, float* d_x, float* d_edge_attr);
int64_t mtmc_mpn_grad_layout(const mtmc_mpn_model* model, int64_t* offsets, int32_t max_offsets);
int32_t mtmc_mpn_backward_flat(const mtmc_mpn_model* model, const mtmc_mpn_call* call,
                               const float* const* d_logits_steps, const float* d_h, float* flat, int64_t flat_floats,
                               float* d_x, float* d_edge_attr);
int32_t mtmc_mpn_run_phase(const mtmc_mpn_model* model, const mtmc_mpn_call* call, int32_t phase, int32_t arg);
int32_t mtmc_mpn_run_phases(const mtmc_mpn_model* model, const mtmc_mpn_call* call, const int32_t* phase_args, int32_t n);

enum { MTMC_GEMM_GENERIC = 0, MTMC_GEMM_INLOOP_64 = 1, MTMC_GEMM_INLOOP_128 = 2, MTMC_GEMM_PRESPLIT_256 = 3,
       MTMC_GEMM_STAGED_128 = 4, MTMC_GEMM_ROWS_16 = 5, MTMC_GEMM_FEW_L0 = 6, MTMC_GEMM_FEW_WAVE = 7 };
enum { MTMC_PASS_C_WALK = 0, MTMC_PASS_C_MFMA_SORTED = 1, MTMC_PASS_C_MFMA_ANY = 2 };
typedef struct mtmc_mpn_plan {
  int32_t enc_kernel[MTMC_MAX_ENC_LAYERS];
  int32_t enc_split_k[MTMC_MAX_ENC_LAYERS];
  int32_t edges_per_thread;
  int32_t lazy_edges;
  int32_t pass_c;
  double avg_degree;
  int32_t pass_a_col_blocks;
  int32_t layer0_panels;
  int32_t enc2_passenger;
  int32_t node_stat_folded;
} mtmc_mpn_plan;
int32_t mtmc_mpn_plan_call(const mtmc_mpn_model* model, const mtmc_mpn_call* call, mtmc_mpn_plan* out);

int32_t mtmc_scatter_add(const float* src, const int64_t* index, int64_t n_src, int64_t n_cols,
                         int64_t dim_size, float* out, void* stream);
int32_t mtmc_scatter_add_i64(const int64_t* src, const int64_t* index, int64_t n_src, int64_t n_cols,
                             int64_t dim_size, int64_t* out, void* stream);
int32_t mtmc_scatter_mean(const float* src, const int64_t* index, int64_t n_src, int64_t n_cols,
                          int64_t dim_size, float* out, float* count_scratch, void* stream);
int32_t mtmc_scatter_max(const float* src, const int64_t* index, int64_t n_src, int64_t n_cols,
                         int64_t dim_size, float* out, int64_t* arg_out, void* stream);

int32_t mtmc_mlp_layer_forward(const mtmc_layer* layer, const float* x, int64_t x_row_stride, int64_t rows,
                               float* y, double* stats_scratch, void* stream);

int32_t mtmc_linear_raw(const float* A, int64_t lda, const float* W, const float* bias, float* Y, int64_t M, int32_t K,
                        int32_t N, uint32_t* scratch, double* stats, void* stream);

int32_t mtmc_linear_few_raw(const float* A, int64_t lda, const double* stats_in, const float* gamma_in, const float* beta_in,
                            double count, const float* W, const float* bias, float* Y, int64_t M, int32_t K, int32_t N,
                            void* work, uint64_t work_bytes, double* stats, void* stream);

int32_t mtmc_linear_staged_raw(const float* A, int64_t lda, const double* stats_in, const float* gamma_in,
                               const float* beta_in, double count, const float* W, const float* bias, float* Y, int64_t M,
                               int32_t K, int32_t N, void* work, uint64_t work_bytes, uint32_t* scratch, double* stats,
                               void* stream);

int32_t mtmc_linear_presplit_raw(const float* A, int64_t lda, const float* W, const float* bias, float* Y, int64_t M,
                                 int32_t K, int32_t N, void* work, uint64_t work_bytes, uint32_t* scratch,
                                 double* stats, int32_t reuse_planes, void* stream);

size_t mtmc_graph_workspace_bytes(int64_t n_nodes, int32_t feat_dim);
int32_t mtmc_build_graph(const float* feats, int64_t feat_row_stride, int64_t n_nodes, int32_t feat_dim, int32_t l2norm,
                         const int32_t* in_list, const int32_t* in_off, const int32_t* out_list, const int64_t* out_off,
                         const int64_t* block_off, int32_t n_cams, int64_t n_edges, const int64_t* node_labels,
                         float* x_out, int64_t* edge_index_out, float* edge_attr_out, float* edge_labels_out,
                         void* workspace, size_t workspace_bytes, void* stream);

size_t mtmc_graph_backward_workspace_bytes(int64_t n_nodes, int32_t feat_dim);
int32_t mtmc_build_graph_backward(const float* feats, int64_t feat_row_stride, int64_t n_nodes, int32_t feat_dim, int32_t l2norm,
                                  const int32_t* in_list, const int32_t* in_off, const int32_t* out_list,
                                  const int64_t* out_off, const int64_t* block_off, int32_t n_cams, int64_t n_edges,
                                  const float* x, const float* edge_attr, const float* d_x, const float* d_edge_attr,
                                  float* d_feats_out, void* workspace, size_t workspace_bytes, void* stream);

int32_t mtmc_cross_entropy_forward(const float* logits, const int64_t* labels, const float* weight, int64_t n,
                                   int32_t n_classes, int64_t ignore_index, int32_t mode, float* per_sample,
                                   double* sums, float* loss_out, void* stream);
int32_t mtmc_cross_entropy_backward(const float* logits, const int64_t* labels, const float* weight, int64_t n,
                                    int32_t n_classes, int64_t ignore_index, int32_t mode, const float* grad,
                                    const double* sums, float* d_logits, void* stream);

int32_t mtmc_cross_entropy_steps_forward(const float* logits, const int64_t* labels, const float* weight, int64_t n,
                                         int32_t n_classes, int32_t n_steps, int64_t ignore_index, int32_t mode,
                                         double* sums, float* loss_out, void* stream);
int32_t mtmc_cross_entropy_steps_backward(const float* logits, const int64_t* labels, const float* weight, int64_t n,
                                          int32_t n_classes, int32_t n_steps, int64_t ignore_index, int32_t mode,
                                          const float* grad, const double* sums, float* d_logits, void* stream);

int32_t mtmc_edge_confusion(const float* logits, const int64_t* labels, int64_t n, int32_t n_classes, int64_t* counts,
                            void* stream);

enum { MTMC_EDGE_W_ONE = 0, MTMC_EDGE_W_GIVEN = 1, MTMC_EDGE_W_BALANCED = 2 };
#define MTMC_EDGE_LOSS_RECORD 4
size_t mtmc_edge_loss_scratch_bytes(int32_t n_steps);
int32_t mtmc_edge_loss_forward(const float* logits, const int64_t* labels, int64_t n, int32_t n_classes, int32_t n_steps,
                               int32_t weight_mode, const float* weight, float fpr_alpha, void* scratch,
                               size_t scratch_bytes, double* record, float* out, int64_t* confusion, void* stream);
int32_t mtmc_edge_loss_backward(const float* logits, const int64_t* labels, int64_t n, int32_t n_classes, int32_t n_steps,
                                const float* grad, const double* record, float* d_logits, void* stream);

enum { MTMC_PP_CUTTING = 1, MTMC_PP_PRUNING = 2, MTMC_PP_SPLITTING = 4 };
size_t mtmc_postprocess_workspace_bytes(int64_t n_nodes, int64_t n_edges, int64_t max_active);
int32_t mtmc_postprocess(const float* logits, const int64_t* row, const int64_t* col, int64_t idx_stride,
                         int64_t n_nodes, int64_t n_edges, int32_t num_cameras, int32_t flags, int64_t max_active,
                         float* prob1, int64_t* predictions, int64_t* id_pred, int32_t* info,
                         void* workspace, size_t workspace_bytes, void* stream);

#define MTMC_CLUSTER_SCORES 9
#define MTMC_CLUSTER_COUNTS 7
#define MTMC_EDGE_PRF 5
size_t mtmc_cluster_scores_workspace_bytes(int64_t n);
int32_t mtmc_cluster_scores(const int64_t* labels_true, int64_t stride_true, const int64_t* labels_pred, int64_t stride_pred,
                            int64_t n, double* scores, int64_t* counts, void* workspace, size_t workspace_bytes,
                            void* stream);
// ... 17 lines not shown
```

Baseline: 1.264 billion edges/s.

## Fold next-round node projections into pass C via linearity of sum aggregation

In eval mode with sum aggregation, pass C now also scatters its per-edge updates through the concatenated node/edge update weights into the next round's P/Q buffers. This lets the per-round projection phase be skipped for rounds after the first. Pass B gains per-node run-length sums so the node-stat moments stay correct without the separate projection. P/Q are double-buffered and zeroed in earlier kernels. The cost is more atomics and register pressure in pass C (launch bounds raised to 3 waves/SIMD, larger span), plus float reassociation in the projections.

```diff
diff --git a/graph-convolutional-network-for-multi-camera-vehicle-tracking_amd/_lib.py b/graph-convolutional-network-for-multi-camera-vehicle-tracking_amd/_lib.py
--- a/graph-convolutional-network-for-multi-camera-vehicle-tracking_amd/_lib.py
+++ b/graph-convolutional-network-for-multi-camera-vehicle-tracking_amd/_lib.py
@@ -67,7 +67,7 @@
 
 STAT_REPLICAS, ATTR_STRIDE, ENC2_STRIDE, Z1_STRIDE, M_STRIDE, Z2_STRIDE = 16, 16, 16, 16, 16, 64
 ROUND_BLOCK = STAT_REPLICAS * (Z1_STRIDE + M_STRIDE + Z2_STRIDE)
-F_DETERMINISTIC, F_GLOBAL_DEG, F_FORK, F_SEED_ON_DEVICE = 1, 4, 2, 16
+F_DETERMINISTIC, F_GLOBAL_DEG, F_FORK, F_SEED_ON_DEVICE, F_NO_PROJ_FOLD = 1, 4, 2, 16, 32
 EDGE_W_ONE, EDGE_W_GIVEN, EDGE_W_BALANCED = range(3)
 EDGE_LOSS_RECORD = 4
 CLUSTER_SCORES, CLUSTER_COUNTS, EDGE_PRF = 9, 7, 5
@@ -76,7 +76,7 @@
 
 LIB_PATH = os.environ.get("MTMC_MPN_LIB") or os.path.join(os.path.dirname(os.path.abspath(__file__)), "csrc", "libmtmc_mpn.so")
 EXPORTS = ["mtmc_mpn_abi_version", "mtmc_mpn_last_error", "mtmc_mpn_workspace_bytes", "mtmc_mpn_workspace_layout",
-           "mtmc_mpn_forward", "mtmc_mpn_run_phase", "mtmc_mpn_run_phases", "mtmc_mpn_plan_call", "mtmc_scatter_add", "mtmc_scatter_add_i64", "mtmc_scatter_mean", "mtmc_scatter_max",
+           "mtmc_mpn_forward", "mtmc_mpn_run_phase", "mtmc_mpn_run_phases", "mtmc_mpn_plan_call", "mtmc_mpn_proj_folded", "mtmc_scatter_add", "mtmc_scatter_add_i64", "mtmc_scatter_mean", "mtmc_scatter_max",
            "mtmc_mlp_layer_forward", "mtmc_mpn_train_workspace_bytes", "mtmc_mpn_backward", "mtmc_graph_workspace_bytes",
            "mtmc_build_graph", "mtmc_postprocess_workspace_bytes", "mtmc_postprocess",
            "mtmc_cross_entropy_forward", "mtmc_cross_entropy_backward",
@@ -193,6 +193,9 @@
                                      C.c_size_t, C.c_void_p]
     lib.mtmc_mpn_plan_call.restype = C.c_int32
     lib.mtmc_mpn_plan_call.argtypes = [C.POINTER(Model), C.POINTER(Call), C.POINTER(Plan)]
+    if hasattr(lib, "mtmc_mpn_proj_folded"):
+        lib.mtmc_mpn_proj_folded.restype = C.c_int32
+        lib.mtmc_mpn_proj_folded.argtypes = [C.POINTER(Model), C.POINTER(Call)]
     lib.mtmc_mpn_run_phase.restype = C.c_int32
     lib.mtmc_mpn_run_phase.argtypes = [C.POINTER(Model), C.POINTER(Call), C.c_int32, C.c_int32]
     lib.mtmc_mpn_run_phases.restype = C.c_int32
diff --git a/graph-convolutional-network-for-multi-camera-vehicle-tracking_amd/csrc/api.hip b/graph-convolutional-network-for-multi-camera-vehicle-tracking_amd/csrc/api.hip
--- a/graph-convolutional-network-for-multi-camera-vehicle-tracking_amd/csrc/api.hip
+++ b/graph-convolutional-network-for-multi-camera-vehicle-tracking_amd/csrc/api.hip
@@ -147,6 +147,18 @@
   out->layer0_panels = p.l0_panels;
   out->enc2_passenger = (p.enc2_may_ride && !(c->flags & MTMC_F_FORK)) ? 1 : 0;
   return MTMC_OK;
+}
+
+int32_t mtmc_mpn_proj_folded(const mtmc_mpn_model* model, const mtmc_mpn_call* call) {
+  mtmc_mpn_plan pub;
+  if (mtmc_mpn_plan_call(model, call, &pub) != MTMC_OK) return 0;
+  Layout lo;
+  CacheLayout cl;
+  CallPlan p;
+  make_layout(model, call->n_nodes, call->n_edges, &lo, call->training != 0);
+  make_cache_layout(model, &cl);
+  make_plan(model, call, lo, cl, &p);
+  return p.proj_fold ? 1 : 0;
 }
 
 int32_t mtmc_mpn_forward(const mtmc_mpn_model* model, const mtmc_mpn_call* call) {
@@ -175,8 +187,9 @@
   if (sd && hipStreamWaitEvent(x.stream, sd->join, 0) != hipSuccess) return fail(MTMC_E_HIP, "join failed");
   const bool fused_h0 = model->num_enc_steps > 0 && call->node_lo == 0 && call->node_hi == call->n_nodes;
   if (!fused_h0 && (rc = run_phase(x, MTMC_PH_NODE_H0, 0))) return rc;
+  x.fold = x.plan.proj_fold;
   for (int r = 0; r < model->num_enc_steps; ++r) {
-    if ((rc = run_phase(x, MTMC_PH_ROUND_PROJ, r, fused_h0))) return rc;
+    if (!(x.fold && r >= 1) && (rc = run_phase(x, MTMC_PH_ROUND_PROJ, r, fused_h0))) return rc;
     if ((rc = run_phase(x, MTMC_PH_ROUND_A, r))) return rc;
     if ((rc = run_phase(x, MTMC_PH_ROUND_B, r))) return rc;
     if ((rc = run_phase(x, MTMC_PH_ROUND_STAT, r))) return rc;
diff --git a/graph-convolutional-network-for-multi-camera-vehicle-tracking_amd/csrc/api_internal.h b/graph-convolutional-network-for-multi-camera-vehicle-tracking_amd/csrc/api_internal.h
--- a/graph-convolutional-network-for-multi-camera-vehicle-tracking_amd/csrc/api_internal.h
+++ b/graph-convolutional-network-for-multi-camera-vehicle-tracking_amd/csrc/api_internal.h
@@ -29,6 +29,7 @@
 struct Layout {
   mtmc_ws_layout pub;
   size_t row32, col32, e_buf[2], P, Q, slab, enc_aff, row_start, carry;
+  size_t P2, Q2;
   size_t col_sub; int col_blocks;
   size_t amax;
   size_t amax_w;
@@ -133,6 +134,8 @@
   lo->P = take((size_t)N * 8 * sizeof(float));
   lo->pub.P_off = lo->P;
   lo->Q = take((size_t)N * 32 * sizeof(float));
+  lo->P2 = training ? lo->P : take((size_t)N * 8 * sizeof(float));
+  lo->Q2 = training ? lo->Q : take((size_t)N * 32 * sizeof(float));
   lo->row32 = take((size_t)E * sizeof(int32_t));
   lo->col32 = take((size_t)E * sizeof(int32_t));
   lo->e_buf[0] = take((size_t)E * 4 * sizeof(float));
@@ -242,6 +245,7 @@
   double avg_degree;
   int col_blocks;
   mtmc::PassC pass_c;
+  bool proj_fold;
   int pass_c_pub() const {
     switch (pass_c) {
       case mtmc::kPassCSortedWalk: case mtmc::kPassCSortedDet: return MTMC_PASS_C_MFMA_SORTED;
@@ -295,6 +299,9 @@
                    mtmc::plan_col_blocks(N, E, p->avg_degree, lo.training) == lo.col_blocks) ? lo.col_blocks : 0;
   const bool drop_n = lo.training && m->dropout_upd_node > 0.f;
   p->pass_c = mtmc::plan_pass_c(m->agg, (c->flags & MTMC_F_DETERMINISTIC) != 0, drop_n, E, N, p->avg_degree);
+  p->proj_fold = !c->training && m->agg == MTMC_AGG_SUM && !m->reattach_nodes && m->num_enc_steps >= 2 &&
+                 !(c->flags & (MTMC_F_DETERMINISTIC | MTMC_F_NO_PROJ_FOLD)) && c->row_hi == 0 && E == c->n_edges_total &&
+                 p->fold_node_stat && p->pass_c == mtmc::kPassCAny;
 }
 
 struct Ctx {
@@ -308,6 +315,7 @@
   CallPlan plan;
   template <typename T> T* wc_at(size_t off) const { return reinterpret_cast<T*>(wc + off); }
   const SidePipe* pipe = nullptr;
+  bool fold = false;
   bool enc2_rides = false;
   template <typename T> T* at(size_t off) const { return reinterpret_cast<T*>(ws + off); }
 };
@@ -399,8 +407,8 @@
   if (r == 0) return x.at<float>(x.lo.pub.h0_off);
   return x.lo.training ? x.at<float>(x.lo.h_tr[r - 1]) : x.at<float>(x.lo.pub.h_acc_off[(r - 1) & 1]);
 }
-inline float* round_P(const Ctx& x, int r) { return x.at<float>(x.lo.training ? x.lo.P_tr[r] : x.lo.P); }
-inline float* round_Q(const Ctx& x, int r) { return x.at<float>(x.lo.training ? x.lo.Q_tr[r] : x.lo.Q); }
+inline float* round_P(const Ctx& x, int r) { return x.at<float>(x.lo.training ? x.lo.P_tr[r] : (x.fold && (r & 1)) ? x.lo.P2 : x.lo.P); }
+inline float* round_Q(const Ctx& x, int r) { return x.at<float>(x.lo.training ? x.lo.Q_tr[r] : (x.fold && (r & 1)) ? x.lo.Q2 : x.lo.Q); }
 inline float* round_z(const Ctx& x, int r) { return x.at<float>(x.lo.training ? x.lo.z_tr[r] : x.lo.e_buf[r & 1]); }
 inline float* round_e(const Ctx& x, int r) { return x.at<float>(x.lo.training ? x.lo.e_tr[r] : x.lo.e_buf[r & 1]); }
 
@@ -436,6 +444,14 @@
   p.col_blocks = x.plan.col_blocks;
   p.col_sub = x.at<int>(x.lo.col_sub); p.cb_row_lo = proj_lo(x.c); p.cb_row_hi = proj_hi(x.c);
   p.enc = enc_params(x);
+  if (x.fold) {
+    const bool last = r == m->num_enc_steps - 1;
+    if (!last) { p.Q_next = round_Q(x, r + 1); p.P_next = round_P(x, r + 1); }
+    if (r >= 1) {
+      p.node_sums = 1;
+      if (!last) { p.zero_q = p.Q_next; p.zero_p = p.P_next; }
+    }
+  }
   return p;
 }
 
@@ -673,6 +689,10 @@
       p.hn = node_in_width(m);
       p.P = round_P(x, arg); p.Q = round_Q(x, arg);
       p.zero_buf = agg_target(x, arg);
+      if (x.fold) {
+        p.zero_buf = agg_target(x, L - 1);
+        p.zero_q = round_Q(x, 1); p.zero_p = round_P(x, 1);
+      }
       p.n_nodes = c->n_nodes;
       p.node_begin = proj_lo(c); p.node_end = proj_hi(c);
       p.edge_deg = x.at<int>(x.lo.pub.deg_off); p.un_b = m->upd_node.bias;
diff --git a/graph-convolutional-network-for-multi-camera-vehicle-tracking_amd/csrc/edge_pass_b.hip b/graph-convolutional-network-for-multi-camera-vehicle-tracking_amd/csrc/edge_pass_b.hip
--- a/graph-convolutional-network-for-multi-camera-vehicle-tracking_amd/csrc/edge_pass_b.hip
+++ b/graph-convolutional-network-for-multi-camera-vehicle-tracking_amd/csrc/edge_pass_b.hip
@@ -6,12 +6,13 @@
 __global__ __launch_bounds__(256) void pass_b_kernel(RoundParams p) {
   drop_resolve(p.drop_e);
   __shared__ float s1[4], t1[4];
-  __shared__ double red[14 * 4 + 4 * 128 + 4];
+  __shared__ double red[14 * 4 + 4 * 128 + 4 + 4 * 64];
   const int lane = threadIdx.x & 63;
   constexpr bool kFold = kEPT == 1;
   const int k32 = lane & 31, hh = lane >> 5;
   const float ub = p.un_b[k32];
   double c0 = 0, c1 = 0;
+  double n1 = 0, n2 = 0;
   const int64_t stride = (int64_t)gridDim.x * blockDim.x * kEPT;
   const int64_t e_end = ((p.n_edges + 63) / 64) * 64;
   int64_t base = (int64_t)blockIdx.x * blockDim.x * kEPT + threadIdx.x;
@@ -62,6 +63,12 @@
   if (base < e_end) fetch(base);
   stat_gather(p.stats + kRoundZ1Off, 8, kZ1Stride, red);
   if (base < e_end) prefetch_q();
+  if (p.zero_q) {
+    const int64_t nq = p.n_nodes * (kH / 4), n4 = nq + p.n_nodes * 2;
+    for (int64_t i = (int64_t)blockIdx.x * blockDim.x + threadIdx.x; i < n4; i += (int64_t)gridDim.x * blockDim.x)
+      (i < nq ? reinterpret_cast<float4*>(p.zero_q) + i : reinterpret_cast<float4*>(p.zero_p) + (i - nq))[0] =
+          make_float4(0.f, 0.f, 0.f, 0.f);
+  }
   __syncthreads();
   EK_T(3, 1);
   if (threadIdx.x < 4) {
@@ -93,10 +100,15 @@
     if (!first_trip) prefetch_q();
     first_trip = false;
     auto rl_f32 = [](float x, int l) { return __int_as_float(__builtin_amdgcn_readlane(__float_as_int(x), l)); };
-    auto add_run = [&](float S0, float S1, float S2, float S3, float qrow) {
+    auto add_run = [&](float S0, float S1, float S2, float S3, float qrow, int len) {
       const double qb = (double)(qrow + ub);
       c0 = fma((double)(hh ? S2 : S0), qb, c0);
       c1 = fma((double)(hh ? S3 : S1), qb, c1);
+      if (p.node_sums) {
+        const double lq = (double)len * qb;
+        n1 += lq;
+        n2 = fma(lq, qb, n2);
+      }
     };
 #pragma unroll
     for (int i = 0; i < kEPT; ++i) {
@@ -115,7 +127,7 @@
       const unsigned long long in_first = __ballot(r == r0);
       if (in_first == ~0ull && r0 >= 0) {
         const float t = wave_sum4_f32(v[0], v[1], v[2], v[3]);
-        if (kFold) add_run(rl_f32(t, 15), rl_f32(t, 47), rl_f32(t, 31), rl_f32(t, 63), qf[i]);
+        if (kFold) add_run(rl_f32(t, 15), rl_f32(t, 47), rl_f32(t, 31), rl_f32(t, 63), qf[i], 64);
         else if ((lane & 15) == 15) unsafeAtomicAdd(p.seg + (int64_t)r0 * 4 + wave_sum4_slot(lane), (double)t);
         continue;
       }
@@ -127,8 +139,9 @@
         if (kFold) {
           const float f0 = rl_f32(fst, 15), f1 = rl_f32(fst, 47);
           const float f2 = rl_f32(fst, 31), f3 = rl_f32(fst, 63);
-          add_run(f0, f1, f2, f3, qf[i]);
-          add_run(rl_f32(tot, 15) - f0, rl_f32(tot, 47) - f1, rl_f32(tot, 31) - f2, rl_f32(tot, 63) - f3, ql[i]);
+          const int n_first = __builtin_popcountll(in_first);
+          add_run(f0, f1, f2, f3, qf[i], n_first);
+          add_run(rl_f32(tot, 15) - f0, rl_f32(tot, 47) - f1, rl_f32(tot, 31) - f2, rl_f32(tot, 63) - f3, ql[i], 64 - n_first);
         } else if ((lane & 15) == 15) {
           const int k = wave_sum4_slot(lane);
           unsafeAtomicAdd(p.seg + (int64_t)r0 * 4 + k, (double)fst);
@@ -138,6 +151,7 @@
       }
       const int prev = __shfl_up(r, 1, 64);
       int flag = (lane == 0 || prev != r) ? 1 : 0;
+      const unsigned long long heads = __ballot(flag != 0);
       const int next_head = __shfl_down(flag, 1, 64);
       const bool tail = active && (lane == 63 || next_head != 0 || e + 1 >= p.n_edges);
 #pragma unroll
@@ -164,8 +178,9 @@
         const int tl = __builtin_amdgcn_readfirstlane(__ffsll((long long)tails) - 1);
         tails &= tails - 1;
         const int rt = __builtin_amdgcn_readlane(r, tl);
+        const int head = 63 - __builtin_clzll(heads & ((2ull << tl) - 1ull));
         add_run(rl_f32(v[0], tl), rl_f32(v[1], tl), rl_f32(v[2], tl),
-                rl_f32(v[3], tl), p.Q[(int64_t)rt * kH + k32]);
+                rl_f32(v[3], tl), p.Q[(int64_t)rt * kH + k32], tl - head + 1);
       }
     }
     base += stride;
@@ -177,9 +192,11 @@
     double* sm_m = red;
     double* sm_c = red + 14 * 4;
     double* sm_m1 = sm_c + 4 * 128;
+    double* sm_n = sm_m1 + 4;
     wave_sums_f64<14>(acc, sm_m + wid * 14);
     sm_c[wid * 128 + (2 * hh) * 32 + k32] = c0;
     sm_c[wid * 128 + (2 * hh + 1) * 32 + k32] = c1;
+    sm_n[wid * 64 + hh * 32 + k32] = hh ? n2 : n1;
     __syncthreads();
     double* m_dst = p.stats + kRoundMOff + (blockIdx.x % kStatRep) * kMStride;
     if (threadIdx.x < 14) {
@@ -191,6 +208,10 @@
       const int i = threadIdx.x - 64;
       sm_c[i] = sm_c[i] + sm_c[128 + i] + sm_c[256 + i] + sm_c[384 + i];
     }
+    if (threadIdx.x >= 192) {
+      const int i = threadIdx.x - 192;
+      sm_n[i] = sm_n[i] + sm_n[64 + i] + sm_n[128 + i] + sm_n[192 + i];
+    }
     __syncthreads();
     if (kFold && threadIdx.x < 32) {
       const int k = threadIdx.x;
@@ -202,8 +223,8 @@
         cross += (double)a[j] * sm_c[j * 32 + k];
       }
       double* z_dst = p.stats + kRoundZ2Off + (blockIdx.x % kStatRep) * kZ2Stride;
-      unsafeAtomicAdd(z_dst + k, lin);
-      unsafeAtomicAdd(z_dst + 32 + k, 2.0 * cross);
+      unsafeAtomicAdd(z_dst + k, p.node_sums ? lin + sm_n[k] : lin);
+      unsafeAtomicAdd(z_dst + 32 + k, p.node_sums ? 2.0 * cross + sm_n[32 + k] : 2.0 * cross);
     }
   }
   EK_T(3, 4);
diff --git a/graph-convolutional-network-for-multi-camera-vehicle-tracking_amd/csrc/edge_pass_c.hip b/graph-convolutional-network-for-multi-camera-vehicle-tracking_amd/csrc/edge_pass_c.hip
--- a/graph-convolutional-network-for-multi-camera-vehicle-tracking_amd/csrc/edge_pass_c.hip
+++ b/graph-convolutional-network-for-multi-camera-vehicle-tracking_amd/csrc/edge_pass_c.hip
@@ -151,7 +151,7 @@
   }
 }
 
-template <bool DROP, bool DET, typename C0Of, typename Account>
+template <bool DROP, bool BY_ROW, typename C0Of, typename Account>
 __device__ __forceinline__ void several_rows_group(const RoundParams& p, const NodeUpdAffine& af, const f32x16c& acc, int rw,
                                                    int g, unsigned gm, int k, int hi, unsigned keep, float ikn, C0Of c0_of,
                                                    Account account) {
@@ -160,7 +160,7 @@
     return DROP ? t * (((keep >> i) & 1u) ? ikn : 0.f) : t;
   };
   int n_rows = 0;
-  if (!DET) {
+  if (!BY_ROW) {
     unsigned left = gm;
     while (left != 0 && n_rows <= 4) {
       const int r = __builtin_amdgcn_readfirstlane(__shfl(rw, 32 * g + __ffs(left) - 1, 64));
@@ -168,7 +168,7 @@
       ++n_rows;
     }
   }
-  if (!DET && n_rows > 4) {
+  if (!BY_ROW && n_rows > 4) {
 #pragma unroll
     for (int i = 0; i < 16; ++i) {
       const int off = (i & 3) + 8 * (i >> 2) + 4 * hi;
@@ -194,16 +194,26 @@
 }
 
 
-template <bool DROP>
-__global__ __launch_bounds__(256, (DROP ? 3 : 1)) void pass_c_mfma_kernel(RoundParams p, int span_c) {
+constexpr int kWcatRows = 40, kWcatLd = 41;
+template <bool DROP, bool FOLD = false>
+__global__ __launch_bounds__(256, (DROP || FOLD ? 3 : 1)) void pass_c_mfma_kernel(RoundParams p, int span_c) {
+  static_assert(!(DROP && FOLD), "the folded projection is an eval-mode form");
   if (DROP) drop_resolve(p.drop_n);
   __shared__ double st[10 + 64];
   __shared__ Z1AffineShared z1s;
+  __shared__ float wcat_s[FOLD ? kH * kWcatLd : 1];
   const int lane = threadIdx.x & 63;
   const int wid = __builtin_amdgcn_readfirstlane(threadIdx.x >> 6);
   const int k = lane & 31, hi = lane >> 5;
   if (p.pass_c == kPassCAnyWalk && p.flags[0] != 0) return;
   EK_T(4, 0);
+  if (FOLD) {
+    for (int i = threadIdx.x; i < kWcatRows * kH; i += 256) {
+      const int j = i >> 5, kk = i & 31;
+      wcat_s[kk * kWcatLd + j] = j < kH ? p.un_w[j * p.un_ld + kk]
+                                        : p.ue_w[((j - kH) & 3) * p.ue_ld + (j < kH + 4 ? 0 : kH) + kk];
+    }
+  }
   const NodeUpdAffine af = node_upd_affine(p, p.lazy_e, k, 4, st, z1s);
   const float sk = af.sk, cb = af.cb;
   const float b0 = sk * p.un_w[k * p.un_ld + p.un_eoff + hi];
@@ -212,6 +222,12 @@
   const Cls2 cls = cls2_load(p.cls_w, p.cls_b, want_logits && p.n_classes == 2);
 
   EK_T(4, 2);
+  float wrow[FOLD ? kH : 1];
+  if (FOLD) {
+    const int j = lane < kWcatRows ? lane : kWcatRows - 1;
+#pragma unroll
+    for (int kk = 0; kk < kH; ++kk) wrow[kk] = wcat_s[kk * kWcatLd + j];
+  }
   const int64_t n_chunks = (p.n_edges + 63) / 64;
   const int64_t n_spans = (n_chunks + span_c - 1) / span_c;
   const int64_t wave_stride = (int64_t)gridDim.x * 4;
@@ -221,7 +237,18 @@
     auto flush = [&]() {
       if (cur >= 0) {
         const float tot = run + __shfl_xor(run, 32, 64);
-        if (hi == 0) unsafeAtomicAdd(p.h_acc + (int64_t)cur * kH + k, tot);
+        if (!FOLD) {
+          if (hi == 0) unsafeAtomicAdd(p.h_acc + (int64_t)cur * kH + k, tot);
+        } else {
+          float o[4] = {0.f, 0.f, 0.f, 0.f};
+#pragma unroll
+          for (int kk = 0; kk < kH; ++kk)
+            o[kk & 3] = fmaf(wrow[kk], __int_as_float(__builtin_amdgcn_readlane(__float_as_int(tot), kk)), o[kk & 3]);
+          const float out = (o[0] + o[1]) + (o[2] + o[3]);
+          float* dst = lane < kH ? p.Q_next + (int64_t)cur * kH + lane
+                                 : p.P_next + ((lane < kH + 4 ? 0 : p.n_nodes) + cur) * 4 + (lane & 3);
+          if (lane < kWcatRows) unsafeAtomicAdd(dst, out);
+        }
       }
     };
     const int64_t c_end = min(n_chunks, (span + 1) * span_c);
@@ -380,7 +407,7 @@
           f32x16c acc = {};
           acc = __builtin_amdgcn_mfma_f32_32x32x2f32(__uint_as_float(xy[g]), b0, acc, 0, 0, 0);
           acc = __builtin_amdgcn_mfma_f32_32x32x2f32(__uint_as_float(zw[g]), b1, acc, 0, 0, 0);
-          several_rows_group<DROP, false>(p, af, acc, rw, g, gm, k, hi, keepbits[g], ikn, c0_of, account);
+          several_rows_group<DROP, FOLD>(p, af, acc, rw, g, gm, k, hi, keepbits[g], ikn, c0_of, account);
         }
       }
       ev_1 = ev_2; rw_1 = rw_2;
@@ -617,11 +644,16 @@
       else hipLaunchKernelGGL((pass_c_sorted_kernel<false, false>), grid, dim3(256), 0, s, p, sc);
     }
   } else if (p.pass_c != kPassCWalk) {
-    const int span_c = span_env > 0 ? span_env : (p.pass_c == kPassCAny ? 1 : 8);
-    const int64_t spans = ((p.n_edges + 63) / 64 + span_c - 1) / span_c, blocks = (spans + 3) / 4;
     const int cap = max_blocks < 256 * 3 ? max_blocks : 256 * 3;
-    if (p.drop_n.on) hipLaunchKernelGGL(pass_c_mfma_kernel<true>, dim3((int)(blocks > cap ? cap : blocks)), dim3(256), 0, s, p, span_c);
-    else hipLaunchKernelGGL(pass_c_mfma_kernel<false>, dim3((int)(blocks > cap ? cap : blocks)), dim3(256), 0, s, p, span_c);
+    const int64_t n_chunks = (p.n_edges + 63) / 64;
+    int span_c = span_env > 0 ? span_env : (p.pass_c == kPassCAny ? 1 : 8);
+    if (span_env <= 0 && p.Q_next && p.pass_c == kPassCAny && cap > 0 && n_chunks > (int64_t)cap * 4)
+      span_c = (int)((n_chunks + (int64_t)cap * 4 - 1) / ((int64_t)cap * 4));
+    const int64_t spans = (n_chunks + span_c - 1) / span_c, blocks = (spans + 3) / 4;
+    const dim3 grid((int)(blocks > cap ? cap : blocks));
+    if (p.drop_n.on) hipLaunchKernelGGL((pass_c_mfma_kernel<true>), grid, dim3(256), 0, s, p, span_c);
+    else if (p.Q_next) hipLaunchKernelGGL((pass_c_mfma_kernel<false, true>), grid, dim3(256), 0, s, p, span_c);
+    else hipLaunchKernelGGL((pass_c_mfma_kernel<false>), grid, dim3(256), 0, s, p, span_c);
   }
 #ifdef MTMC_WALK_TAIL_GRID
   if (p.pass_c == kPassCSortedWalk || p.pass_c == kPassCSortedDet) {
diff --git a/graph-convolutional-network-for-multi-camera-vehicle-tracking_amd/csrc/kernels.h b/graph-convolutional-network-for-multi-camera-vehicle-tracking_amd/csrc/kernels.h
--- a/graph-convolutional-network-for-multi-camera-vehicle-tracking_amd/csrc/kernels.h
+++ b/graph-convolutional-network-for-multi-camera-vehicle-tracking_amd/csrc/kernels.h
@@ -79,6 +79,9 @@
   int det; const int* flags; const int* deg; const int* row_start; float* carry; int64_t n_nodes;
   double avg_degree;
   int col_blocks = 0; const int* col_sub = nullptr; int64_t cb_row_lo = 0, cb_row_hi = 0;
+  float* Q_next = nullptr; float* P_next = nullptr;
+  float* zero_q = nullptr; float* zero_p = nullptr;
+  int node_sums = 0;
   EdgeEncParams enc;
 };
 
@@ -94,6 +97,7 @@
   int hn;
   float* P; float* Q;
   float* zero_buf;
+  float* zero_q = nullptr; float* zero_p = nullptr;
   int64_t n_nodes;
   int64_t node_begin, node_end;
   const int* edge_deg; const float* un_b; double* z2_stats;
diff --git a/graph-convolutional-network-for-multi-camera-vehicle-tracking_amd/csrc/node_kernels.hip b/graph-convolutional-network-for-multi-camera-vehicle-tracking_amd/csrc/node_kernels.hip
--- a/graph-convolutional-network-for-multi-camera-vehicle-tracking_amd/csrc/node_kernels.hip
+++ b/graph-convolutional-network-for-multi-camera-vehicle-tracking_amd/csrc/node_kernels.hip
@@ -66,6 +66,14 @@
       if (node < p.node_end)
         reinterpret_cast<float4*>(p.zero_buf + node * kH)[threadIdx.x & 7] = make_float4(0.f, 0.f, 0.f, 0.f);
     }
+    if (p.zero_q && threadIdx.x < kProjNodes * 8) {
+      const int64_t node = node0 + (threadIdx.x >> 3);
+      const int q = threadIdx.x & 7;
+      if (node < p.node_end) {
+        reinterpret_cast<float4*>(p.zero_q + node * kH)[q] = make_float4(0.f, 0.f, 0.f, 0.f);
+        if (q < 2) reinterpret_cast<float4*>(p.zero_p)[(q ? p.n_nodes : 0) + node] = make_float4(0.f, 0.f, 0.f, 0.f);
+      }
+    }
     __syncthreads();
     EK_T(0, 2);
     float acc[5] = {0.f, 0.f, 0.f, 0.f, 0.f};
@@ -209,6 +217,11 @@
     if (p.zero_buf && live) {
       *reinterpret_cast<float4*>(p.zero_buf + node * kH + 8 * g) = make_float4(0.f, 0.f, 0.f, 0.f);
       *reinterpret_cast<float4*>(p.zero_buf + node * kH + 8 * g + 4) = make_float4(0.f, 0.f, 0.f, 0.f);
+    }
+    if (p.zero_q && live) {
+      *reinterpret_cast<float4*>(p.zero_q + node * kH + 8 * g) = make_float4(0.f, 0.f, 0.f, 0.f);
+      *reinterpret_cast<float4*>(p.zero_q + node * kH + 8 * g + 4) = make_float4(0.f, 0.f, 0.f, 0.f);
+      if (g < 2) reinterpret_cast<float4*>(p.zero_p)[(g ? p.n_nodes : 0) + node] = make_float4(0.f, 0.f, 0.f, 0.f);
     }
     f32x4p acc[3];
 #pragma unroll
diff --git a/graph-convolutional-network-for-multi-camera-vehicle-tracking_amd/engine.py b/graph-convolutional-network-for-multi-camera-vehicle-tracking_amd/engine.py
--- a/graph-convolutional-network-for-multi-camera-vehicle-tracking_amd/engine.py
+++ b/graph-convolutional-network-for-multi-camera-vehicle-tracking_amd/engine.py
@@ -185,7 +185,8 @@
     def call_struct(self, n_nodes, n_edges, n_edges_total=None, node_lo=0, node_hi=None, row_range=None, training=False,
                     flags=None, weight_cache=None) -> _lib.Call:
         if flags is None:
-            flags = _lib.F_DETERMINISTIC if getattr(self.module, "deterministic", False) else 0
+            flags = (_lib.F_DETERMINISTIC if getattr(self.module, "deterministic", False) else 0) | \
+                (0 if getattr(self.module, "fold_projections", True) else _lib.F_NO_PROJ_FOLD)
         if weight_cache is None:
             weight_cache = getattr(self.module, "cache_weight_planes", True)
         call = _lib.Call()
@@ -265,6 +266,16 @@
                                      layer0_panels=out.layer0_panels, enc2_passenger=bool(out.enc2_passenger),
                                      node_stat_folded=bool(out.node_stat_folded))
 
+    def proj_folded(self, n_nodes, n_edges, n_edges_total=None, node_range=None, row_range=None, training=False, flags=0,
+                    weight_cache=True) -> bool:
+        fn = getattr(self.lib, "mtmc_mpn_proj_folded", None)
+        if fn is None:
+            return False
+        model = self.shape_model(dropout=True)
+        node_lo, node_hi = (0, None) if node_range is None else node_range[:2]
+        call = self.call_struct(n_nodes, n_edges, n_edges_total, node_lo, node_hi, row_range, training, flags, weight_cache)
+        return bool(fn(C.byref(model), C.byref(call)))
+
     def phase_list(self):
         s = self.spec
         seq = [(_lib.PH_BEGIN, 0), (_lib.PH_EDGE_ENC, 0)]
diff --git a/graph-convolutional-network-for-multi-camera-vehicle-tracking_amd/modules.py b/graph-convolutional-network-for-multi-camera-vehicle-tracking_amd/modules.py
--- a/graph-convolutional-network-for-multi-camera-vehicle-tracking_amd/modules.py
+++ b/graph-convolutional-network-for-multi-camera-vehicle-tracking_amd/modules.py
@@ -102,6 +102,7 @@
         self.num_class_steps = s.num_class_steps
         self.check_indices = False
         self.deterministic = False
+        self.fold_projections = True
         self.cache_weight_planes = True
         self.device_seed = None
         self._engine = None
@@ -193,6 +194,7 @@
             x.requires_grad or edge_attr.requires_grad or any(p.requires_grad for p in params))
         tape = bool(needs_grad or self.training)
         flags = (_lib_flags.F_DETERMINISTIC if self.deterministic else 0) | \
+            (0 if self.fold_projections else _lib_flags.F_NO_PROJ_FOLD) | \
             (torch_ops.CHECK_INDICES if self.check_indices else 0) | \
             (0 if self.cache_weight_planes else torch_ops.NO_WEIGHT_CACHE)
         if self.training and self.device_seed is not None:
diff --git a/include/mtmc_mpn.h b/include/mtmc_mpn.h
--- a/include/mtmc_mpn.h
+++ b/include/mtmc_mpn.h
@@ -82,6 +82,8 @@
 #define MTMC_F_FORK 2
 #define MTMC_F_SEED_ON_DEVICE 16
 
+#define MTMC_F_NO_PROJ_FOLD 32
+
 #define MTMC_STAT_REPLICAS 16
 #define MTMC_ATTR_STRIDE 16
 #define MTMC_ENC2_STRIDE 16
@@ -156,6 +158,7 @@
   int32_t node_stat_folded;
 } mtmc_mpn_plan;
 int32_t mtmc_mpn_plan_call(const mtmc_mpn_model* model, const mtmc_mpn_call* call, mtmc_mpn_plan* out);
+int32_t mtmc_mpn_proj_folded(const mtmc_mpn_model* model, const mtmc_mpn_call* call);
 
 int32_t mtmc_scatter_add(const float* src, const int64_t* index, int64_t n_src, int64_t n_cols,
                          int64_t dim_size, float* out, void* stream);
```

Measured after the change: 1.220 billion edges/s. 0.966x the previous value.
